# HorizonRobotics/GeoFlowSlam

Measured on AMD Instinct MI355X. Metric: front-end frames/sec (ORB+match+GICP) on 640x480 RGBD, higher is better.
Workload: dtype u8/int32 (ORB, match) + f64 (GICP); 1 GPU; BASELINE.json configs[1]: 640x480 RGBD frame pair, ORB extract (1000 feats, 8 levels) + BF Hamming match + GMS filter + GICP on ~19k-pt clouds (stride-4 depth grid); batch_pairs_per_gpu=512, lanes_per_gpu=4, passes=K passes per lane chain, joined once, distinct_scenes_per_gpu=512, scene_seeds=1000..1511 (rank 0), global_batch_pairs=512, parallelism=frames sharded x1, no collective

## Files before the change

### geoflowslam_amd/api.py

```python
import ctypes as C
import os

import numpy as np

_HERE = os.path.dirname(os.path.abspath(__file__))
_LIB_PATH = os.path.join(_HERE, "libgfs_hip.so")
_lib = None

KP_DTYPE = np.dtype(
    [("x", "<f4"), ("y", "<f4"), ("size", "<f4"), ("angle", "<f4"), ("response", "<f4"), ("octave", "<i4"),
     ("class_id", "<i4")]
)


class GfsError(RuntimeError):
    pass


class OrbConfig(C.Structure):
    _fields_ = [("nfeatures", C.c_int32), ("scale_factor", C.c_float), ("nlevels", C.c_int32),
                ("ini_th_fast", C.c_int32), ("min_th_fast", C.c_int32), ("max_rows", C.c_int32),
                ("max_cols", C.c_int32), ("max_batch", C.c_int32), ("device", C.c_int32),
                ("blur_taps_variant", C.c_int32)]


def _i32_fields(names):
    return [(n, C.c_int32) for n in names.split()]


class OrbGeometryInfo(C.Structure):
    _fields_ = _i32_fields("supported pyr_strips pyr_strips_fine pyr_in_lds xtab_in_lds xtab_in_lds_fine kp_cap octree_on_device "
                           "oct_node_cap n_cells n_blur_tiles fast_lds_wave")


class OrbLevelInfo(C.Structure):
    _fields_ = _i32_fields("rows cols n_cell_cols n_cell_rows w_cell h_cell n_cells max_cell_w max_cell_h quota n_ini kp_cap "
                           "octree_on_device")


class OrbPaths(C.Structure):
    _fields_ = _i32_fields("octree_on_device pyr_kernel pyr_fine_cut geometry_builds last_batch rows cols")


ORB_PYR_NONE, ORB_PYR_LDS, ORB_PYR_HBM = 0, 1, 2


class GicpConfig(C.Structure):
    _fields_ = [("num_threads", C.c_int32), ("downsampling_resolution", C.c_double),
                ("max_correspondence_distance", C.c_double), ("rotation_eps", C.c_double),
                ("translation_eps", C.c_double), ("max_iterations", C.c_int32), ("num_neighbors", C.c_int32)]


class GicpResult(C.Structure):
    _fields_ = [("T", C.c_double * 16), ("converged", C.c_int32), ("iterations", C.c_uint64),
                ("num_inliers", C.c_uint64), ("H", C.c_double * 36), ("b", C.c_double * 6), ("error", C.c_double),
                ("n_target_ds", C.c_int32), ("n_source_ds", C.c_int32), ("n_linearize", C.c_int32),
                ("n_error_evals", C.c_int32)]


class LbaProblem(C.Structure):
    _fields_ = [("n_poses", C.c_int32), ("n_points", C.c_int32), ("n_edges", C.c_int32), ("pose_q", C.c_void_p),
                ("pose_t", C.c_void_p), ("pose_fixed", C.c_void_p), ("points", C.c_void_p), ("edge_pose", C.c_void_p),
                ("edge_point", C.c_void_p), ("edge_obs", C.c_void_p), ("edge_inv_sigma2", C.c_void_p),
                ("edge_stereo", C.c_void_p), ("fx", C.c_double), ("fy", C.c_double), ("cx", C.c_double),
                ("cy", C.c_double), ("bf", C.c_double), ("huber_mono", C.c_double), ("huber_stereo", C.c_double),
                ("iterations", C.c_int32)]


class LbaSolution(C.Structure):
    _fields_ = [("pose_q", C.c_void_p), ("pose_t", C.c_void_p), ("points", C.c_void_p), ("edge_chi2", C.c_void_p),
                ("edge_depth_positive", C.c_void_p), ("iterations_run", C.c_int32), ("final_chi2", C.c_double),
                ("final_lambda", C.c_double)]


class LbaTrial(C.Structure):
    _fields_ = [("Dinv", C.c_void_p), ("Hs", C.c_void_p), ("bs", C.c_void_p), ("xp", C.c_void_p), ("xl", C.c_void_p),
                ("lambda_", C.c_double), ("scale", C.c_double), ("solve_ok", C.c_int32)]


class GbaInfo(C.Structure):
    _fields_ = [("n_free", C.c_int32), ("panel_rows", C.c_int32), ("panels", C.c_int32), ("block_pairs", C.c_int64),
                ("contributions", C.c_int64), ("system_bytes", C.c_int64), ("trials", C.c_int32), ("launches", C.c_int32)]


class EssentialGraphProblem(C.Structure):
    _fields_ = [("n_vertices", C.c_int32), ("n_edges", C.c_int32), ("n_points", C.c_int32), ("vertex_q", C.c_void_p),
                ("vertex_t", C.c_void_p), ("vertex_s", C.c_void_p), ("vertex_fixed", C.c_void_p), ("edge_i", C.c_void_p),
                ("edge_j", C.c_void_p), ("edge_q", C.c_void_p), ("edge_t", C.c_void_p), ("edge_s", C.c_void_p), ("edge_w", C.c_void_p),
                ("fix_scale", C.c_int32), ("iterations", C.c_int32), ("lambda_init", C.c_double), ("points", C.c_void_p),
                ("point_ref", C.c_void_p)]


class EssentialGraphSolution(C.Structure):
    _fields_ = [("vertex_q", C.c_void_p), ("vertex_t", C.c_void_p), ("vertex_s", C.c_void_p), ("points", C.c_void_p),
                ("edge_chi2", C.c_void_p), ("iterations_run", C.c_int32), ("final_chi2", C.c_double), ("final_lambda", C.c_double)]


class EssentialGraphInfo(C.Structure):
    _fields_ = [("n_free", C.c_int32), ("dimension", C.c_int32), ("panels", C.c_int32), ("blocks", C.c_int64), ("trials", C.c_int32),
                ("launches", C.c_int32), ("system_bytes", C.c_int64)]


class EssentialGraphTrial(C.Structure):
    _fields_ = [("H", C.c_void_p), ("b", C.c_void_p), ("x", C.c_void_p), ("chi2", C.c_double), ("trial_chi2", C.c_double),
                ("scale", C.c_double), ("n_free", C.c_int32), ("dimension", C.c_int32), ("solve_ok", C.c_int32)]


class LbaLidar(C.Structure):
    _fields_ = [("map", C.c_void_p), ("pose_local", C.c_void_p), ("matches_inliers", C.c_void_p), ("cloud_begin", C.c_void_p),
                ("cloud", C.c_void_p), ("two_camera", C.c_int32)]


def lba_lidar_struct(prob, map_handle=None):
    L = LbaLidar()
    keep = dict(pose_local=np.ascontiguousarray(prob["pose_local"], np.uint8),
                matches_inliers=np.ascontiguousarray(prob["matches_inliers"], np.int32),
                cloud_begin=np.ascontiguousarray(prob["cloud_begin"], np.int32),
                cloud=np.ascontiguousarray(prob["cloud"], np.float32).reshape(-1, 3))
    for k, v in keep.items():
        setattr(L, k, v.ctypes.data)
    L.map = map_handle
    L.two_camera = int(prob.get("two_camera", 0))
    return L, keep


class PoseProblem(C.Structure):
    _fields_ = [("q", C.c_double * 4), ("t", C.c_double * 3), ("n_obs", C.c_int32), ("xw", C.c_void_p), ("obs", C.c_void_p),
                ("inv_sigma2", C.c_void_p), ("stereo", C.c_void_p), ("fx", C.c_double), ("fy", C.c_double),
                ("cx", C.c_double), ("cy", C.c_double), ("bf", C.c_double), ("n_rounds", C.c_int32), ("its", C.c_int32)]


class PoseSolution(C.Structure):
    _fields_ = [("outlier", C.c_void_p), ("chi2", C.c_void_p), ("q", C.c_double * 4), ("t", C.c_double * 3),
                ("avg_reproj_error", C.c_float), ("n_inliers", C.c_int32), ("rounds_run", C.c_int32),
                ("iterations_run", C.c_int32)]


def pose_structs(prob):
    P, S = PoseProblem(), PoseSolution()
    n = int(prob["n_obs"]) if "n_obs" in prob else len(prob["xw"])
    keep = dict(xw=np.ascontiguousarray(prob["xw"], np.float64).reshape(-1, 3), obs=np.ascontiguousarray(prob["obs"], np.float64).reshape(-1, 3),
                inv_sigma2=np.ascontiguousarray(prob["inv_sigma2"], np.float32), stereo=np.ascontiguousarray(prob["stereo"], np.uint8),
                outlier=np.zeros(max(n, 1), np.uint8), chi2=np.zeros(max(n, 1), np.float64))
    P.q[:] = [float(v) for v in prob["q"]]
    P.t[:] = [float(v) for v in prob["t"]]
    P.n_obs = n
    for name in ("xw", "obs", "inv_sigma2", "stereo"):
        setattr(P, name, keep[name].ctypes.data)
    for name in ("fx", "fy", "cx", "cy", "bf"):
        setattr(P, name, float(prob[name]))
    P.n_rounds = int(prob.get("n_rounds", 4))
    P.its = int(prob.get("its", 10))
    S.outlier = keep["outlier"].ctypes.data
    S.chi2 = keep["chi2"].ctypes.data
    return P, S, keep, n


def pose_result(S, keep, n):
    return dict(outlier=keep["outlier"][:n].astype(bool), chi2=keep["chi2"][:n].copy(), q=np.array(S.q[:]), t=np.array(S.t[:]),
                avg_reproj_error=float(S.avg_reproj_error), n_inliers=int(S.n_inliers), rounds_run=int(S.rounds_run),
                iterations_run=int(S.iterations_run))


class Sim3OptProblem(C.Structure):
    _fields_ = [("s12", C.c_double * 8), ("cam1", C.c_double * 4), ("cam2", C.c_double * 4), ("th2", C.c_float),
                ("fix_scale", C.c_int32), ("n_pairs", C.c_int32), ("x1c", C.c_void_p), ("x2c", C.c_void_p), ("obs1", C.c_void_p),
                ("obs2", C.c_void_p), ("inv_sigma2_1", C.c_void_p), ("inv_sigma2_2", C.c_void_p)]


class Sim3OptSolution(C.Structure):
    _fields_ = [("s12", C.c_double * 8), ("n_in", C.c_int32), ("n_bad", C.c_int32), ("status", C.c_int32),
                ("iterations_run", C.c_int32 * 2), ("pair_state", C.c_void_p), ("chi2", C.c_void_p)]


SIM3_OPT_EARLY_RETURN, SIM3_OPT_BOTH_PHASES = 0, 1
SIM3_PAIR_INLIER, SIM3_PAIR_REMOVED_FIRST, SIM3_PAIR_REMOVED_FINAL = 0, 1, 2


def sim3_opt_structs(prob):
    P, S = Sim3OptProblem(), Sim3OptSolution()
    n = int(prob["n_pairs"]) if "n_pairs" in prob else len(prob["x1c"])
    keep = dict(x1c=np.ascontiguousarray(prob["x1c"], np.float64).reshape(-1, 3), x2c=np.ascontiguousarray(prob["x2c"], np.float64).reshape(-1, 3),
                obs1=np.ascontiguousarray(prob["obs1"], np.float64).reshape(-1, 2), obs2=np.ascontiguousarray(prob["obs2"], np.float64).reshape(-1, 2),
                inv_sigma2_1=np.ascontiguousarray(prob["inv_sigma2_1"], np.float32), inv_sigma2_2=np.ascontiguousarray(prob["inv_sigma2_2"], np.float32),
                pair_state=np.zeros(max(n, 1), np.uint8), chi2=np.zeros((max(n, 1), 2), np.float64))
    P.s12[:] = [float(v) for v in prob["s12"]]
    P.cam1[:] = [float(v) for v in prob["cam1"]]
    P.cam2[:] = [float(v) for v in prob["cam2"]]
    P.th2 = float(prob["th2"])
    P.fix_scale = int(bool(prob["fix_scale"]))
    P.n_pairs = n
    for name in ("x1c", "x2c", "obs1", "obs2", "inv_sigma2_1", "inv_sigma2_2"):
        setattr(P, name, keep[name].ctypes.data)
    S.pair_state = keep["pair_state"].ctypes.data
    S.chi2 = keep["chi2"].ctypes.data
    return P, S, keep, n

# ... 483 lines not shown
                 node_start=np.full(cap + 1, -7, np.int32), feat_idx=np.full(cap, -7, np.int32),
                 word_of_feature=np.full(cap, -7, np.int32) if with_words else None)
        for name, a in k.items():
            setattr(VV[b], name, a.ctypes.data if a is not None else None)
        keep.append(k)
    return VV, keep


def bow_vectors_results(VV, keep, counts):
    out = []
    for b, k in enumerate(keep):
        nw, nn = VV[b].n_words, VV[b].n_nodes
        m = int(k["node_start"][nn])
        out.append(dict(word_id=k["word_id"][:nw].copy(), word_value=k["word_value"][:nw].copy(), node_id=k["node_id"][:nn].copy(),
                        node_start=k["node_start"][:nn + 1].copy(), feat_idx=k["feat_idx"][:m].copy(),
                        word_of_feature=None if k["word_of_feature"] is None or counts is None else k["word_of_feature"][:counts[b]].copy()))
    return out


def sbp_map_struct(prob):
    P = SbpMapProblem()
    keep = dict(mp_proj=np.ascontiguousarray(prob["mp_proj"], np.float32).reshape(-1, 3),
                mp_level=np.ascontiguousarray(prob["mp_level"], np.int32),
                mp_view_cos=np.ascontiguousarray(prob["mp_view_cos"], np.float32),
                mp_desc=np.ascontiguousarray(prob["mp_desc"], np.uint8).reshape(-1, 32),
                mp_has_obs=np.ascontiguousarray(prob["mp_has_obs"], np.uint8),
                cur_kps_un=np.ascontiguousarray(prob["cur_kps_un"], KP_DTYPE),
                cur_u_right=np.ascontiguousarray(prob["cur_u_right"], np.float32),
                cur_desc=np.ascontiguousarray(prob["cur_desc"], np.uint8).reshape(-1, 32),
                cur_has_mp_obs=np.ascontiguousarray(prob["cur_has_mp_obs"], np.uint8),
                scale_factors=np.ascontiguousarray(prob["scale_factors"], np.float32))
    P.n_mp, P.n_cur = len(keep["mp_proj"]), len(keep["cur_kps_un"])
    for name, a in keep.items():
        setattr(P, name, a.ctypes.data)
    for name in ("min_x", "min_y", "grid_w_inv", "grid_h_inv", "th", "nn_ratio"):
        setattr(P, name, float(np.float32(prob[name])))
    P.n_levels = len(keep["scale_factors"])
    return P, keep


def sbp_struct(prob):
    P = SbpProblem()
    keep = dict(last_xw=np.ascontiguousarray(prob["last_xw"], np.float32).reshape(-1, 3),
                last_desc=np.ascontiguousarray(prob["last_desc"], np.uint8).reshape(-1, 32),
                last_octave=np.ascontiguousarray(prob["last_octave"], np.int32),
                last_angle=np.ascontiguousarray(prob["last_angle"], np.float32),
                last_mp_has_obs=np.ascontiguousarray(prob["last_mp_has_obs"], np.uint8),
                cur_kps_un=np.ascontiguousarray(prob["cur_kps_un"], KP_DTYPE),
                cur_u_right=np.ascontiguousarray(prob["cur_u_right"], np.float32),
                cur_desc=np.ascontiguousarray(prob["cur_desc"], np.uint8).reshape(-1, 32),
                cur_has_mp_obs=np.ascontiguousarray(prob["cur_has_mp_obs"], np.uint8),
                scale_factors=np.ascontiguousarray(prob["scale_factors"], np.float32))
    P.n_last, P.n_cur = len(keep["last_xw"]), len(keep["cur_kps_un"])
    for name, a in keep.items():
        setattr(P, name, a.ctypes.data)
    for name in ("Tcw_q", "Tcw_t", "Tlw_q", "Tlw_t"):
        getattr(P, name)[:] = [float(np.float32(v)) for v in prob[name]]
    for name in ("fx", "fy", "cx", "cy", "bf", "b", "min_x", "max_x", "min_y", "max_y", "grid_w_inv", "grid_h_inv", "th"):
        setattr(P, name, float(np.float32(prob[name])))
    P.n_levels = len(keep["scale_factors"])
    P.mono = int(prob.get("mono", 0))
    P.check_orientation = int(prob.get("check_orientation", 1))
    return P, keep


class PoseLidarProblem(C.Structure):
    _fields_ = [("q", C.c_float * 4), ("t", C.c_float * 3), ("n_obs", C.c_int32), ("xw", C.c_void_p), ("obs", C.c_void_p),
                ("inv_sigma2", C.c_void_p), ("stereo", C.c_void_p), ("fx", C.c_double), ("fy", C.c_double), ("cx", C.c_double),
                ("cy", C.c_double), ("bf", C.c_double), ("n_cloud", C.c_int32), ("cloud", C.c_void_p), ("map", C.c_void_p),
                ("n_iterations", C.c_int32), ("two_camera", C.c_int32)]


class PoseLidarSolution(C.Structure):
    _fields_ = [("outlier", C.c_void_p), ("chi2", C.c_void_p), ("q", C.c_double * 4), ("t", C.c_double * 3), ("qf", C.c_float * 4),
                ("tf", C.c_float * 3), ("avg_reproj_error", C.c_float), ("n_inliers", C.c_int32), ("n_lidar_inliers", C.c_int32),
                ("residual", C.c_float), ("lidar_rounds", C.c_int32), ("rounds_run", C.c_int32), ("iterations_run", C.c_int32),
                ("round_edges", C.c_int32 * 4), ("round_chi2", C.c_float * 4), ("round_valid", C.c_int32 * 4)]


class LidarMapInput(C.Structure):
    _fields_ = [("n_keyframes", C.c_int32), ("q", C.c_void_p), ("t", C.c_void_p), ("cloud_begin", C.c_void_p), ("cloud", C.c_void_p),
                ("leaf", C.c_float)]


class LidarMapInfo(C.Structure):
    _fields_ = [("n_in", C.c_int32), ("n_out", C.c_int32), ("passthrough", C.c_int32), ("div", C.c_int32 * 3)]


class FrameCloudConfig(C.Structure):
    _fields_ = [("horizontal_angle", C.c_double), ("max_distance", C.c_double), ("local_map_resolution", C.c_double),
                ("downsize_resolution", C.c_float), ("angle_guard_deg", C.c_double)]


class FrameCloudInfo(C.Structure):
    _fields_ = [(k, C.c_int32) for k in ("n_in", "n_scans", "n_edge_raw", "n_surf_raw", "n_edge_voxel", "n_surf_voxel", "n_edge", "n_surf",
                                         "n_down", "host_scan_split")] + [("passthrough", C.c_int32 * 3)]


class FrameCloudStageBuffers(C.Structure):
    _fields_ = [("scans", C.c_void_p), ("cap_scans", C.c_int32)] + \
               [(k, C.c_void_p) for k in ("edge_raw", "surf_raw", "edge_voxel", "surf_voxel", "edge", "surf")] + [("cap_points", C.c_int32)]


def frame_cloud_info(I):
    d = {k: int(getattr(I, k)) for k, _ in FrameCloudInfo._fields_[:10]}
    d["passthrough"] = tuple(int(v) for v in I.passthrough)
    return d


def lidar_map_info(I):
    return dict(n_in=int(I.n_in), n_out=int(I.n_out), passthrough=int(I.passthrough), div=tuple(int(v) for v in I.div))


def pose_lidar_structs(prob, map_handle=None):
    P, S = PoseLidarProblem(), PoseLidarSolution()
    xw = np.ascontiguousarray(prob["xw"], np.float64).reshape(-1, 3)
    n = len(xw)
    cloud = np.ascontiguousarray(prob["cloud"], np.float32).reshape(-1, 3)
    keep = dict(xw=xw, obs=np.ascontiguousarray(prob["obs"], np.float64).reshape(-1, 3),
                inv_sigma2=np.ascontiguousarray(prob["inv_sigma2"], np.float32), stereo=np.ascontiguousarray(prob["stereo"], np.uint8),
                cloud=cloud, outlier=np.zeros(max(n, 1), np.uint8), chi2=np.zeros(max(n, 1), np.float64))
    P.q[:] = [float(v) for v in np.asarray(prob["q"], np.float32)]
    P.t[:] = [float(v) for v in np.asarray(prob["t"], np.float32)]
    P.n_obs = n
    for name in ("xw", "obs", "inv_sigma2", "stereo", "cloud"):
        setattr(P, name, keep[name].ctypes.data)
    for name in ("fx", "fy", "cx", "cy", "bf"):
        setattr(P, name, float(prob[name]))
    P.n_cloud = len(cloud)
    P.map = map_handle
    P.n_iterations = int(prob.get("n_iterations", 3))
    P.two_camera = int(prob.get("two_camera", 0))
    S.outlier = keep["outlier"].ctypes.data
    S.chi2 = keep["chi2"].ctypes.data
    S.n_lidar_inliers = int(prob.get("n_lidar_inliers", 0))
    S.residual = float(prob.get("residual", 0.0))
    return P, S, keep, n


def pose_lidar_result(S, keep, n):
    return dict(outlier=keep["outlier"][:n].astype(bool), chi2=keep["chi2"][:n].copy(), q=np.array(S.q[:]), t=np.array(S.t[:]),
                qf=np.array(S.qf[:], np.float32), tf=np.array(S.tf[:], np.float32), avg_reproj_error=np.float32(S.avg_reproj_error),
                n_inliers=int(S.n_inliers), n_lidar_inliers=int(S.n_lidar_inliers), residual=np.float32(S.residual),
                lidar_rounds=int(S.lidar_rounds), rounds_run=int(S.rounds_run), iterations_run=int(S.iterations_run),
                round_edges=list(S.round_edges), round_chi2=np.array(S.round_chi2[:], np.float32), round_valid=list(S.round_valid))


ABI_SYMBOLS = [
    "gfs_abi_version", "gfs_last_error", "gfs_device_count",
    "gfs_orb_default_config", "gfs_orb_create", "gfs_orb_destroy", "gfs_orb_get_tables", "gfs_orb_max_keypoints",
    "gfs_orb_extract", "gfs_orb_extract_batch", "gfs_orb_extract_batch_device", "gfs_orb_device_results",
    "gfs_orb_fetch", "gfs_orb_level_size", "gfs_orb_fetch_level", "gfs_orb_fetch_candidates", "gfs_orb_octree_host",
    "gfs_orb_octree_device", "gfs_test_sort_replica", "gfs_test_heap_sort_replica", "gfs_test_glibc_math", "gfs_test_traffic",
    "gfs_test_orb_blur_tiles", "gfs_test_orb_geometry", "gfs_test_orb_last_paths",
    "gfs_hamming256", "gfs_matcher_create", "gfs_matcher_destroy", "gfs_bf_match_hamming",
    "gfs_bf_match_hamming_batch_device",
    "gfs_gicp_default_config", "gfs_gicp_create", "gfs_gicp_destroy", "gfs_gicp_align", "gfs_gicp_align_batch_device",
    "gfs_gicp_fetch_preprocessed", "gfs_gicp_tile_stats", "gfs_gicp_knn_stats", "gfs_gicp_coop_stats", "gfs_test_gicp_coop_hold", "gfs_test_gicp_coop_release", "gfs_test_gicp_coop_in_use", "gfs_frame_rgbd", "gfs_gicp_align_next", "gfs_gicp_align_next_batch_device", "gfs_test_voxel_sort", "gfs_test_voxel_sort_paths", "gfs_test_wave_std_sort",
    "gfs_lba_create", "gfs_lba_destroy", "gfs_lba_solve", "gfs_lba_solve_bool", "gfs_lba_linearize", "gfs_lba_batch_create", "gfs_lba_batch_destroy",
    "gfs_lba_solve_batch", "gfs_lba_lidar_reserve", "gfs_lba_solve_lidar", "gfs_lba_solve_lidar_bool", "gfs_lba_linearize_lidar",
    "gfs_lba_fetch_lidar_edges", "gfs_test_lba_stop_at_look", "gfs_test_lba_last_looks", "gfs_test_lba_first_trial",
    "gfs_gba_create", "gfs_gba_destroy", "gfs_gba_solve", "gfs_gba_solve_bool", "gfs_gba_last_info", "gfs_test_gba_first_trial",
    "gfs_test_gba_panel_rows", "gfs_test_gba_lists", "gfs_test_gba_tile_layout",
    "gfs_essential_graph_create", "gfs_essential_graph_destroy", "gfs_essential_graph_optimize", "gfs_essential_graph_correct_points",
    "gfs_essential_graph_last_info", "gfs_test_essential_graph_first_trial", "gfs_test_essential_graph_lists",
    "gfs_sim3_opt_create", "gfs_sim3_opt_destroy", "gfs_sim3_optimize", "gfs_test_glibc_exp",
    "gfs_sim3_ransac_iterations", "gfs_sim3_ransac_create", "gfs_sim3_ransac_solve", "gfs_sim3_ransac_destroy",
    "gfs_frame_create", "gfs_frame_destroy", "gfs_depth_to_cloud", "gfs_depth_to_cloud_batch_device", "gfs_depth_convert_u16_batch_device", "gfs_stereo_from_rgbd",
    "gfs_stereo_from_rgbd_batch_device",
    "gfs_pose_create", "gfs_pose_destroy", "gfs_pose_optimize", "gfs_pose_set_sum_order",
    "gfs_lidar_mapper_create", "gfs_lidar_mapper_destroy", "gfs_lidar_map_build", "gfs_lidar_map_fetch", "gfs_voxel_grid_filter",
    "gfs_test_lidar_map_grid",
    "gfs_frame_cloud_default_config", "gfs_frame_cloud_create", "gfs_frame_cloud_destroy", "gfs_frame_cloud_extract",
    "gfs_frame_cloud_extract_device", "gfs_test_frame_cloud_stages", "gfs_test_frame_cloud_radius",
    "gfs_lidar_map_create", "gfs_lidar_map_set", "gfs_lidar_map_destroy", "gfs_pose_lidar_create", "gfs_pose_lidar_destroy",
    "gfs_pose_lidar_set_sum_order", "gfs_pose_lidar_optimize", "gfs_pose_lidar_fetch_edges",
    "gfs_gms_create", "gfs_gms_destroy", "gfs_gms_inlier_mask", "gfs_gms_inlier_mask_batch_device",
    "gfs_sbp_create", "gfs_sbp_destroy", "gfs_search_by_projection", "gfs_search_by_projection_map",
    "gfs_sbp_reserve_local", "gfs_search_local_points", "gfs_sbp_reserve_fuse", "gfs_fuse_search", "gfs_test_glibc_logf",
    "gfs_sbp_reserve_sim3_search", "gfs_sim3_search", "gfs_test_sim3_search_groups",
    "gfs_sbp_reserve_triangulation", "gfs_create_new_map_points", "gfs_sbp_reserve_bow", "gfs_search_by_bow",
    "gfs_map_points_create", "gfs_map_points_destroy", "gfs_map_points_update",
    "gfs_bow_create", "gfs_bow_destroy", "gfs_bow_transform", "gfs_bow_transform_device",
    "gfs_bow_db_create", "gfs_bow_db_destroy", "gfs_bow_db_add", "gfs_bow_db_erase", "gfs_bow_db_query",
    "gfs_klt_create", "gfs_klt_destroy", "gfs_klt_layout", "gfs_klt_pyramid_create", "gfs_klt_pyramid_destroy",
    "gfs_klt_build_pyramid", "gfs_klt_build_pyramid_device", "gfs_klt_pyramid_download", "gfs_klt_track", "gfs_klt_fb_track",
    "gfs_klt_fb_track_device",
    "gfs_fmat_create", "gfs_fmat_destroy", "gfs_find_fundamental_ransac", "gfs_find_fundamental_ransac_device",
    "gfs_klt_compact_tracks_device", "gfs_klt_apply_mask_device",
    "gfs_clahe_default_config", "gfs_clahe_create", "gfs_clahe_destroy", "gfs_clahe_apply", "gfs_clahe_apply_device",
    "gfs_clahe_download_luts", "gfs_klt_build_pyramid_clahe", "gfs_klt_build_pyramid_clahe_device",
    "gfs_timer_create", "gfs_timer_destroy", "gfs_timer_start", "gfs_timer_stop", "gfs_timer_elapsed_ms",
    "gfs_profile_enable", "gfs_profile_report", "gfs_profile_reset",
]


def lib():
    global _lib
    if _lib is None:
        if not os.path.exists(_LIB_PATH):
            raise GfsError(f"{_LIB_PATH} not built: run `python -c 'import __graft_entry__ as g; g.build()'` "
                           "(there is no CPU fallback)")
        L = C.CDLL(_LIB_PATH)
        L.gfs_last_error.restype = C.c_char_p
        vp, ip, i = C.c_void_p, C.POINTER(C.c_int), C.c_int
        L.gfs_orb_default_config.argtypes = [C.POINTER(OrbConfig)]
        L.gfs_orb_create.argtypes = [C.POINTER(OrbConfig), C.POINTER(vp)]
        L.gfs_orb_destroy.argtypes = [vp]
        L.gfs_orb_get_tables.argtypes = [vp] * 7
        L.gfs_orb_max_keypoints.argtypes = [vp]
        L.gfs_orb_extract.argtypes = [vp, vp, i, i, i, i, i, vp, vp, i, ip]
        L.gfs_orb_extract_batch.argtypes = [vp, vp, i, i, i, i, i, i, vp, vp, i, vp, vp]
        L.gfs_orb_extract_batch_device.argtypes = [vp, vp, i, i, i, i, i, vp]
        L.gfs_orb_device_results.argtypes = [vp, C.POINTER(vp), C.POINTER(vp), C.POINTER(vp), C.POINTER(vp), ip]
        L.gfs_orb_fetch.argtypes = [vp, i, vp, vp, i, ip, ip]
        L.gfs_orb_level_size.argtypes = [vp, i, ip, ip]
        L.gfs_orb_fetch_level.argtypes = [vp, i, i, i, vp]
        L.gfs_orb_fetch_candidates.argtypes = [vp, i, i, vp, vp, vp, i]
        L.gfs_test_orb_geometry.argtypes = [i, i, i, i, C.c_float, C.POINTER(OrbGeometryInfo), vp, i]
        L.gfs_test_orb_last_paths.argtypes = [vp, C.POINTER(OrbPaths)]
        L.gfs_orb_octree_host.argtypes = [vp, vp, vp, i, i, i, i, i, i, vp, i]
        L.gfs_orb_octree_device.argtypes = [i, vp, vp, vp, i, i, i, i, i, i, vp, vp, vp, i]
        L.gfs_test_glibc_math.argtypes = [i, vp, i, vp, vp, vp]
        L.gfs_test_glibc_logf.argtypes = [i, vp, i, vp]
        L.gfs_sbp_reserve_local.argtypes = [vp, i]
        L.gfs_search_local_points.argtypes = [vp, C.POINTER(LocalPointsProblem), i, C.POINTER(LocalPointsResult)]
        L.gfs_sbp_reserve_fuse.argtypes = [vp, i, i, i]
        L.gfs_fuse_search.argtypes = [vp, C.POINTER(FusePoints), i, C.POINTER(FuseKeyframe), i, C.POINTER(FuseResult)]
        L.gfs_sbp_reserve_sim3_search.argtypes = [vp, i, i, i]
        L.gfs_sim3_search.argtypes = [vp, C.POINTER(FusePoints), i, C.POINTER(Sim3SearchProblem), i, C.POINTER(Sim3SearchResult)]
        L.gfs_test_sim3_search_groups.argtypes = [vp, i]
        L.gfs_sbp_reserve_triangulation.argtypes = [vp, i, C.c_int64]
        L.gfs_create_new_map_points.argtypes = [vp, C.POINTER(TriProblem), i, C.POINTER(C.POINTER(TriResult))]
        L.gfs_sbp_reserve_bow.argtypes = [vp, i, i]
        L.gfs_search_by_bow.argtypes = [vp, C.POINTER(BowProblem), i, C.POINTER(C.POINTER(BowResult))]
        L.gfs_map_points_create.argtypes = [i, i, i, C.POINTER(vp)]
        L.gfs_map_points_destroy.argtypes = [vp]
        L.gfs_map_points_update.argtypes = [vp, C.POINTER(MapPointsProblem), C.POINTER(MapPointsResult)]
        L.gfs_test_traffic.argtypes = [i, i, C.c_longlong, C.c_longlong, i, C.POINTER(C.c_longlong)]
        L.gfs_hamming256.argtypes = [vp, vp]
        L.gfs_matcher_create.argtypes = [i, i, i, i, C.POINTER(vp)]
        L.gfs_matcher_destroy.argtypes = [vp]
        L.gfs_bf_match_hamming.argtypes = [vp, vp, i, vp, i, vp, vp]
        L.gfs_bf_match_hamming_batch_device.argtypes = [vp, vp, vp, vp, vp, i, i, vp, vp, vp]
        if hasattr(L, "gfs_gicp_create"):
            L.gfs_gicp_default_config.argtypes = [C.POINTER(GicpConfig)]
            L.gfs_gicp_create.argtypes = [i, i, i, C.POINTER(vp)]
            L.gfs_gicp_destroy.argtypes = [vp]
            L.gfs_gicp_align.argtypes = [vp, vp, i, vp, i, vp, C.POINTER(GicpConfig), C.POINTER(GicpResult)]
            L.gfs_gicp_align_batch_device.argtypes = [vp, vp, vp, vp, vp, i, i, vp, C.POINTER(GicpConfig), vp, vp]
            L.gfs_gicp_fetch_preprocessed.argtypes = [vp, i, i, vp, vp, i, ip]
            L.gfs_gicp_tile_stats.argtypes = [vp, vp, i]
            L.gfs_gicp_knn_stats.argtypes = [vp, i, i, vp, vp, i]
            L.gfs_gicp_coop_stats.argtypes = [vp, vp]
            L.gfs_test_gicp_coop_hold.argtypes = [vp, i]
            L.gfs_test_gicp_coop_release.argtypes = [vp, i]
            L.gfs_test_gicp_coop_in_use.argtypes = [i]
            L.gfs_test_voxel_sort.argtypes = [vp, vp, i, vp]
            L.gfs_test_voxel_sort_paths.argtypes = [vp, vp]
            L.gfs_test_wave_std_sort.argtypes = [i, vp, i, vp]
            L.gfs_gicp_align_next.argtypes = [vp, vp, i, vp, C.POINTER(GicpConfig), C.POINTER(GicpResult)]
            L.gfs_gicp_align_next_batch_device.argtypes = [vp, vp, vp, i, i, vp, C.POINTER(GicpConfig), vp, vp]
        if hasattr(L, "gfs_lba_create"):
            L.gfs_lba_create.argtypes = [i, i, i, i, C.POINTER(vp)]
            L.gfs_lba_destroy.argtypes = [vp]
            L.gfs_lba_solve.argtypes = [vp, C.POINTER(LbaProblem), C.POINTER(LbaSolution), vp]
            L.gfs_lba_solve_bool.argtypes = [vp, C.POINTER(LbaProblem), C.POINTER(LbaSolution), vp]
            L.gfs_lba_linearize.argtypes = [vp, C.POINTER(LbaProblem), vp, vp, vp, vp, vp, vp, C.POINTER(C.c_double)]
            L.gfs_lba_batch_create.argtypes = [i, i, i, i, i, C.POINTER(vp)]
            L.gfs_lba_batch_destroy.argtypes = [vp]
            L.gfs_lba_solve_batch.argtypes = [vp, vp, vp, i, vp]
            L.gfs_test_lba_stop_at_look.argtypes = [i]
            L.gfs_test_lba_last_looks.argtypes = [C.POINTER(C.c_int32)] * 4
            L.gfs_test_lba_first_trial.argtypes = [vp, C.POINTER(LbaProblem), C.POINTER(LbaTrial)]
        if hasattr(L, "gfs_gba_create"):
            L.gfs_gba_create.argtypes = [i, i, i, i, C.POINTER(vp)]
            L.gfs_gba_destroy.argtypes = [vp]
            L.gfs_gba_solve.argtypes = [vp, C.POINTER(LbaProblem), C.POINTER(LbaSolution), vp]
            L.gfs_gba_solve_bool.argtypes = [vp, C.POINTER(LbaProblem), C.POINTER(LbaSolution), vp]
            L.gfs_gba_last_info.argtypes = [vp, C.POINTER(GbaInfo)]
            L.gfs_test_gba_first_trial.argtypes = [vp, C.POINTER(LbaProblem), C.POINTER(LbaTrial)]
            L.gfs_test_gba_panel_rows.argtypes = []
            L.gfs_test_gba_lists.argtypes = [i, i, i, vp, vp, vp, vp, vp, vp, vp, C.c_int64, vp, C.c_int64, vp, vp]
            L.gfs_test_gba_tile_layout.argtypes = [C.c_int64, C.c_int64, C.c_int64, vp]
        if hasattr(L, "gfs_essential_graph_create"):
            L.gfs_essential_graph_create.argtypes = [i, i, i, i, C.POINTER(vp)]
            L.gfs_essential_graph_destroy.argtypes = [vp]
            L.gfs_essential_graph_optimize.argtypes = [vp, C.POINTER(EssentialGraphProblem), C.POINTER(EssentialGraphSolution)]
            L.gfs_essential_graph_correct_points.argtypes = [vp, i, vp, vp, i, vp, vp, vp]
            L.gfs_essential_graph_last_info.argtypes = [vp, C.POINTER(EssentialGraphInfo)]
            L.gfs_test_essential_graph_first_trial.argtypes = [vp, C.POINTER(EssentialGraphProblem), C.POINTER(EssentialGraphTrial)]
            L.gfs_test_essential_graph_lists.argtypes = [i, i, vp, vp, vp, vp, vp, vp, vp, C.c_int64, vp, C.c_int64]
        if hasattr(L, "gfs_sim3_opt_create"):
            L.gfs_sim3_opt_create.argtypes = [i, i, i, C.POINTER(vp)]
            L.gfs_sim3_opt_destroy.argtypes = [vp]
            L.gfs_sim3_optimize.argtypes = [vp, vp, i, vp]
            L.gfs_test_glibc_exp.argtypes = [i, vp, i, vp]
        if hasattr(L, "gfs_sim3_ransac_create"):
            L.gfs_sim3_ransac_iterations.argtypes = [i, C.c_double, i, i]
            L.gfs_sim3_ransac_create.argtypes = [i, i, i, i, C.POINTER(vp)]
            L.gfs_sim3_ransac_destroy.argtypes = [vp]
            L.gfs_sim3_ransac_solve.argtypes = [vp, vp, i, vp]
        L.gfs_bow_create.argtypes = [i, C.POINTER(BowVocabularyStruct), i, i, C.POINTER(vp)]
        L.gfs_bow_destroy.argtypes = [vp]
        L.gfs_bow_destroy.restype = None
        L.gfs_bow_transform.argtypes = [vp, C.POINTER(vp), vp, i, i, C.POINTER(BowVectors)]
        L.gfs_bow_transform_device.argtypes = [vp, vp, vp, i, i, i, C.POINTER(BowVectors)]
        L.gfs_bow_db_create.argtypes = [i, i, i, C.POINTER(vp)]
        L.gfs_bow_db_destroy.argtypes = [vp]
        L.gfs_bow_db_destroy.restype = None
        L.gfs_bow_db_add.argtypes = [vp, i, i, vp, vp]
        L.gfs_bow_db_erase.argtypes = [vp, i]
        L.gfs_bow_db_query.argtypes = [vp, i, vp, vp, vp, vp, vp]
        if hasattr(L, "gfs_lba_solve_lidar"):
            L.gfs_lba_lidar_reserve.argtypes = [vp, i]
            L.gfs_lba_solve_lidar.argtypes = [vp, C.POINTER(LbaProblem), C.POINTER(LbaLidar), C.POINTER(LbaSolution), vp, vp]
            L.gfs_lba_solve_lidar_bool.argtypes = [vp, C.POINTER(LbaProblem), C.POINTER(LbaLidar), C.POINTER(LbaSolution), vp, vp]
            L.gfs_lba_linearize_lidar.argtypes = [vp, C.POINTER(LbaProblem), C.POINTER(LbaLidar), vp, vp, vp, vp, vp, vp,
                                                  C.POINTER(C.c_double), vp, i, vp]
            L.gfs_lba_fetch_lidar_edges.argtypes = [vp, i, vp, vp, vp, i, vp]
        if hasattr(L, "gfs_lidar_map_build"):
            L.gfs_lidar_mapper_create.argtypes = [i, i, i, C.POINTER(vp)]
            L.gfs_lidar_mapper_destroy.argtypes = [vp]
            L.gfs_lidar_map_build.argtypes = [vp, C.POINTER(LidarMapInput), vp, C.POINTER(LidarMapInfo)]
            L.gfs_lidar_map_fetch.argtypes = [vp, vp, i, C.POINTER(C.c_int32)]
            L.gfs_voxel_grid_filter.argtypes = [vp, vp, i, C.c_float, vp, i, C.POINTER(LidarMapInfo)]
            L.gfs_test_lidar_map_grid.argtypes = [vp, vp, i, vp, vp, i, C.POINTER(C.c_int32), C.POINTER(C.c_int32)]
        L.gfs_frame_cloud_default_config.argtypes = [C.POINTER(FrameCloudConfig)]
        L.gfs_frame_cloud_default_config.restype = None
        L.gfs_frame_cloud_create.argtypes = [i, i, C.POINTER(FrameCloudConfig), C.POINTER(vp)]
        L.gfs_frame_cloud_destroy.argtypes = [vp]
        L.gfs_frame_cloud_extract.argtypes = [vp, vp, i, vp, i, vp, i, C.POINTER(FrameCloudInfo)]
        L.gfs_frame_cloud_extract_device.argtypes = [vp, vp, vp, vp, i, vp, i, C.POINTER(FrameCloudInfo)]
        L.gfs_test_frame_cloud_stages.argtypes = [vp, C.POINTER(FrameCloudStageBuffers)]
        L.gfs_test_frame_cloud_radius.argtypes = [vp, vp, i, i, vp, i, C.POINTER(C.c_int32)]
        if hasattr(L, "gfs_frame_create"):
            f = C.c_float
            L.gfs_frame_create.argtypes = [i, i, i, i, C.POINTER(vp)]
            L.gfs_frame_destroy.argtypes = [vp]
            L.gfs_depth_to_cloud.argtypes = [vp, vp, i, i, i, i, f, f, f, f, vp, i, ip]
            L.gfs_depth_to_cloud_batch_device.argtypes = [vp, vp, i, i, i, i, f, f, f, f, vp, i, vp, vp]
            L.gfs_depth_convert_u16_batch_device.argtypes = [vp, vp, i, i, i, f, vp, vp]
            L.gfs_stereo_from_rgbd.argtypes = [vp, vp, vp, i, vp, i, i, i, f, vp, vp]
            L.gfs_frame_rgbd.argtypes = [vp, vp, vp, i, vp, i, i, i, f, i, f, f, f, f, vp, vp, vp, i, ip, vp, vp, ip]
            L.gfs_stereo_from_rgbd_batch_device.argtypes = [vp, vp, vp, vp, i, i, vp, i, i, f, vp, vp, vp]
        if hasattr(L, "gfs_klt_create"):
            f, d = C.c_float, C.c_double
            L.gfs_klt_create.argtypes = [i, i, i, i, i, i, i, C.POINTER(vp)]
            L.gfs_klt_destroy.argtypes = [vp]
            L.gfs_klt_layout.argtypes = [vp, vp, vp, vp]
            L.gfs_klt_pyramid_create.argtypes = [vp, C.POINTER(vp)]
            L.gfs_klt_pyramid_destroy.argtypes = [vp]
            L.gfs_klt_build_pyramid.argtypes = [vp, vp, vp, i, i]
            L.gfs_klt_build_pyramid_device.argtypes = [vp, vp, vp, i, i, vp]
            L.gfs_klt_pyramid_download.argtypes = [vp, vp, i, vp, vp]
            L.gfs_klt_track.argtypes = [vp, vp, vp, i, vp, vp, vp, vp, vp, i, i, d, i, d]
            L.gfs_klt_fb_track.argtypes = [vp, vp, vp, i, vp, vp, vp, vp, vp, i, f, f]
            L.gfs_klt_fb_track_device.argtypes = [vp, vp, vp, i, i, vp, vp, vp, vp, vp, i, f, f, vp]
            L.gfs_klt_compact_tracks_device.argtypes = [vp, i, i, vp, vp, vp, vp, vp, vp, vp, vp, vp]
            L.gfs_klt_apply_mask_device.argtypes = [vp, i, i, vp, vp, vp, vp, vp]
        L.gfs_clahe_default_config.argtypes = [C.POINTER(ClaheConfig)]
        L.gfs_clahe_default_config.restype = None
        L.gfs_clahe_create.argtypes = [i, i, i, i, C.POINTER(ClaheConfig), C.POINTER(vp)]
        L.gfs_clahe_destroy.argtypes = [vp]
        L.gfs_clahe_apply.argtypes = [vp, vp, i, i, i, i, vp, i]
        L.gfs_clahe_apply_device.argtypes = [vp, vp, i, i, i, i, vp, i, vp]
        L.gfs_clahe_download_luts.argtypes = [vp, i, vp]
        L.gfs_klt_build_pyramid_clahe.argtypes = [vp, vp, vp, vp, i, i, vp, i]
        L.gfs_klt_build_pyramid_clahe_device.argtypes = [vp, vp, vp, vp, i, i, vp, i, vp]
        if hasattr(L, "gfs_fmat_create"):
            L.gfs_fmat_create.argtypes = [i, i, i, C.POINTER(vp)]
            L.gfs_fmat_destroy.argtypes = [vp]
            L.gfs_find_fundamental_ransac.argtypes = [vp, i, vp, vp, vp, C.c_double, C.c_double, i, vp, vp, vp]
            L.gfs_find_fundamental_ransac_device.argtypes = [vp, i, i, vp, vp, vp, C.c_double, C.c_double, i, vp, vp, vp]
        L.gfs_timer_create.argtypes = [i, C.POINTER(vp)]
        L.gfs_timer_destroy.argtypes = [vp]
        L.gfs_timer_start.argtypes = [vp, vp]
        L.gfs_timer_stop.argtypes = [vp, vp]
        L.gfs_timer_elapsed_ms.argtypes = [vp, C.POINTER(C.c_float)]
        L.gfs_profile_report.argtypes = [vp, vp, vp, i]
        _lib = L
    return _lib


def _p(a):
    return a.ctypes.data_as(C.c_void_p) if a is not None else None


def _check(rc, what):
    if rc < 0:
        err = GfsError(f"{what} failed ({rc}): {lib().gfs_last_error().decode()}")
        err.code = rc
        raise err
    return rc


def device_count():
    return lib().gfs_device_count()


class ORBextractor:

    def __init__(self, nfeatures=1000, scaleFactor=1.2, nlevels=8, iniThFAST=20, minThFAST=7, max_rows=480,
                 max_cols=640, max_batch=1, device=0, blur_taps_variant=0):
        L = lib()
        cfg = OrbConfig()
        L.gfs_orb_default_config(C.byref(cfg))
        cfg.nfeatures, cfg.scale_factor, cfg.nlevels = nfeatures, scaleFactor, nlevels
        cfg.ini_th_fast, cfg.min_th_fast = iniThFAST, minThFAST
        cfg.max_rows, cfg.max_cols, cfg.max_batch, cfg.device = max_rows, max_cols, max_batch, device
        cfg.blur_taps_variant = blur_taps_variant
        self.nlevels = nlevels
        self.h = C.c_void_p()
        _check(L.gfs_orb_create(C.byref(cfg), C.byref(self.h)), "gfs_orb_create")
        self.cap = L.gfs_orb_max_keypoints(self.h)

    def close(self):
        if getattr(self, "h", None) and _lib is not None:
            _lib.gfs_orb_destroy(self.h)
        self.h = None

    __del__ = close

    def GetLevels(self):
        return self.nlevels

    def tables(self):
        n = self.nlevels
        sc, inv, s2, is2 = (np.zeros(n, np.float32) for _ in range(4))
        feats = np.zeros(n, np.int32)
        umax = np.zeros(16, np.int32)
        _check(lib().gfs_orb_get_tables(self.h, _p(sc), _p(inv), _p(s2), _p(is2), _p(feats), _p(umax)), "get_tables")
        return dict(scale=sc, inv_scale=inv, sigma2=s2, inv_sigma2=is2, feats=feats, umax=umax)

    def GetScaleFactors(self):
        return self.tables()["scale"]

    def GetInverseScaleFactors(self):
        return self.tables()["inv_scale"]

    def GetScaleSigmaSquares(self):
        return self.tables()["sigma2"]

    def GetInverseScaleSigmaSquares(self):
        return self.tables()["inv_sigma2"]

    def __call__(self, image, vLappingArea=(0, 0)):
        if image is None or image.size == 0:
            return -1, np.zeros(0, KP_DTYPE), np.zeros((0, 32), np.uint8)
        assert image.dtype == np.uint8 and image.ndim == 2, "CV_8UC1 expected (src/ORBextractor.cc:1153)"
        stride = image.strides[0]
        assert image.strides[1] == 1
        kps = np.zeros(self.cap, KP_DTYPE)
        desc = np.zeros((self.cap, 32), np.uint8)
        n = C.c_int(0)
        r = lib().gfs_orb_extract(self.h, C.c_void_p(image.ctypes.data), image.shape[0], image.shape[1], stride,
                                  vLappingArea[0], vLappingArea[1], _p(kps), _p(desc), self.cap, C.byref(n))
        if r < -1:
            err = GfsError(f"gfs_orb_extract failed ({r + 100}): {lib().gfs_last_error().decode()}")
            err.code = r + 100
            raise err
        return r, kps[:n.value].copy(), desc[:n.value].copy()

    def extract_batch(self, images, vLappingArea=(0, 0)):
        imgs = [np.ascontiguousarray(im, np.uint8) for im in images]
        B = len(imgs)
        rows, cols = imgs[0].shape
        ptrs = (C.c_void_p * B)(*[im.ctypes.data for im in imgs])
        kps = np.zeros((B, self.cap), KP_DTYPE)
        desc = np.zeros((B, self.cap, 32), np.uint8)
        n = np.zeros(B, np.int32)
        mono = np.zeros(B, np.int32)
        _check(lib().gfs_orb_extract_batch(self.h, ptrs, B, rows, cols, cols, vLappingArea[0], vLappingArea[1], _p(kps),
                                           _p(desc), self.cap, _p(n), _p(mono)), "gfs_orb_extract_batch")
        return [(int(mono[b]), kps[b, :n[b]].copy(), desc[b, :n[b]].copy()) for b in range(B)]

    def extract_batch_device(self, dev_ptr, B, rows, cols, vLappingArea=(0, 0), stream=None):
        _check(lib().gfs_orb_extract_batch_device(self.h, C.c_void_p(dev_ptr), B, rows, cols, vLappingArea[0],
                                                  vLappingArea[1], C.c_void_p(stream) if stream else None),
               "gfs_orb_extract_batch_device")

    def device_results(self):
        k, d, c, m = C.c_void_p(), C.c_void_p(), C.c_void_p(), C.c_void_p()
        cap = C.c_int()
        _check(lib().gfs_orb_device_results(self.h, C.byref(k), C.byref(d), C.byref(c), C.byref(m), C.byref(cap)),
               "gfs_orb_device_results")
        return dict(kps=k.value, desc=d.value, counts=c.value, mono=m.value, cap=cap.value)

    def fetch(self, b):
        kps = np.zeros(self.cap, KP_DTYPE)
        desc = np.zeros((self.cap, 32), np.uint8)
        n, mono = C.c_int(), C.c_int()
        _check(lib().gfs_orb_fetch(self.h, b, _p(kps), _p(desc), self.cap, C.byref(n), C.byref(mono)), "gfs_orb_fetch")
        return mono.value, kps[:n.value].copy(), desc[:n.value].copy()

    def level_size(self, l):
        r, c = C.c_int(), C.c_int()
        _check(lib().gfs_orb_level_size(self.h, l, C.byref(r), C.byref(c)), "gfs_orb_level_size")
        return r.value, c.value

    def level(self, l, b=0, blurred=False):
        r, c = self.level_size(l)
        a = np.zeros((r, c), np.uint8)
        _check(lib().gfs_orb_fetch_level(self.h, b, l, int(blurred), _p(a)), "gfs_orb_fetch_level")
        return a

    def candidates(self, l, b=0):
        n = _check(lib().gfs_orb_fetch_candidates(self.h, b, l, None, None, None, 0), "gfs_orb_fetch_candidates")
        x, y, s = (np.zeros(max(n, 1), np.int32) for _ in range(3))
        lib().gfs_orb_fetch_candidates(self.h, b, l, _p(x), _p(y), _p(s), n)
        return x[:n], y[:n], s[:n]


    def last_paths(self):
        P = OrbPaths()
        _check(lib().gfs_test_orb_last_paths(self.h, C.byref(P)), "gfs_test_orb_last_paths")
        return {n: int(getattr(P, n)) for n, _ in OrbPaths._fields_}


def orb_geometry(rows, cols, nfeatures=1000, nlevels=8, scale_factor=1.2):
    I = OrbGeometryInfo()
    Lv = (OrbLevelInfo * nlevels)()
    rc = lib().gfs_test_orb_geometry(rows, cols, nfeatures, nlevels, scale_factor, C.byref(I), C.cast(Lv, C.c_void_p), nlevels)
    out = {n: int(getattr(I, n)) for n, _ in OrbGeometryInfo._fields_}
    out["supported"] = bool(out["supported"])
    if rc == -5:
        return dict(out, levels=[])
    _check(rc, "gfs_test_orb_geometry")
    return dict(out, levels=[{n: int(getattr(Lv[l], n)) for n, _ in OrbLevelInfo._fields_} for l in range(nlevels)])


def wave_std_sort_perm(keys, device=0):
    k = np.ascontiguousarray(keys, np.uint32)
    perm = np.zeros(max(len(k), 1), np.uint16)
    _check(lib().gfs_test_wave_std_sort(device, _p(k), len(k), _p(perm)), "gfs_test_wave_std_sort")
    return perm[:len(k)].astype(np.int64)


def octree_host(x, y, score, min_x, max_x, min_y, max_y, n_features):
    x = np.ascontiguousarray(x, np.int32)
    y = np.ascontiguousarray(y, np.int32)
    score = np.ascontiguousarray(score, np.int32)
    out = np.zeros(max(len(x), 1), np.int32)
    n = lib().gfs_orb_octree_host(_p(x), _p(y), _p(score), len(x), min_x, max_x, min_y, max_y, n_features, _p(out),
                                  len(out))
    return out[:n]


def octree_device(x, y, score, min_x, max_x, min_y, max_y, n_features, device=0):
    x = np.ascontiguousarray(x, np.int32)
    y = np.ascontiguousarray(y, np.int32)
    score = np.ascontiguousarray(score, np.int32)
    cap = n_features + 64
    ox, oy, os_ = (np.zeros(cap, np.int32) for _ in range(3))
    n = _check(lib().gfs_orb_octree_device(device, _p(x), _p(y), _p(score), len(x), min_x, max_x, min_y, max_y, n_features,
                                           _p(ox), _p(oy), _p(os_), cap), "gfs_orb_octree_device")
    return ox[:n], oy[:n], os_[:n]


class ORBmatcher:

    def __init__(self, max_query=4096, max_train=4096, max_batch=1, device=0):
        self.h = C.c_void_p()
        _check(lib().gfs_matcher_create(device, max_query, max_train, max_batch, C.byref(self.h)), "gfs_matcher_create")

    def close(self):
        if getattr(self, "h", None) and _lib is not None:
            _lib.gfs_matcher_destroy(self.h)
        self.h = None

    __del__ = close

    @staticmethod
    def DescriptorDistance(a, b):
        a = np.ascontiguousarray(a, np.uint8)
        b = np.ascontiguousarray(b, np.uint8)
        return int(lib().gfs_hamming256(_p(a), _p(b)))

    def match(self, query, train):
        q = np.ascontiguousarray(query, np.uint8).reshape(-1, 32)
        t = np.ascontiguousarray(train, np.uint8).reshape(-1, 32)
        ti = np.zeros(len(q), np.int32)
        di = np.zeros(len(q), np.int32)
        n = _check(lib().gfs_bf_match_hamming(self.h, _p(q), len(q), _p(t), len(t), _p(ti), _p(di)),
                   "gfs_bf_match_hamming")
        return ti[:n], di[:n]

    def match_batch_device(self, d_query, d_nq, d_train, d_nt, B, stride_rows, d_idx, d_dist, stream=None):
        _check(lib().gfs_bf_match_hamming_batch_device(self.h, C.c_void_p(d_query), C.c_void_p(d_nq), C.c_void_p(d_train),
                                                       C.c_void_p(d_nt), B, stride_rows, C.c_void_p(d_idx),
                                                       C.c_void_p(d_dist), C.c_void_p(stream) if stream else None),
               "gfs_bf_match_hamming_batch_device")


def gicp_default_config():
    c = GicpConfig()
    lib().gfs_gicp_default_config(C.byref(c))
    return c


def _result_dict(res):
    return dict(
        T=np.array(res.T).reshape(4, 4).T.copy(), converged=bool(res.converged), iterations=int(res.iterations),
        num_inliers=int(res.num_inliers), H=np.array(res.H).reshape(6, 6).T.copy(), b=np.array(res.b),
        error=float(res.error), n_target_ds=res.n_target_ds, n_source_ds=res.n_source_ds,
        n_linearize=res.n_linearize, n_error_evals=res.n_error_evals)


class RegistrationGICP:

    def __init__(self, max_points=40960, max_batch=1, device=0):
        self.h = C.c_void_p()
        self.max_points = max_points
        _check(lib().gfs_gicp_create(device, max_points, max_batch, C.byref(self.h)), "gfs_gicp_create")

    def close(self):
        if getattr(self, "h", None) and _lib is not None:
            _lib.gfs_gicp_destroy(self.h)
        self.h = None

    __del__ = close

    def RegisterPointClouds(self, target_points, source_points, init_T_target_source=None, cfg=None):
        t = np.ascontiguousarray(target_points, np.float32).reshape(-1, 4)
        s = np.ascontiguousarray(source_points, np.float32).reshape(-1, 4)
        T0 = np.eye(4) if init_T_target_source is None else np.asarray(init_T_target_source, np.float64)
        T0c = np.ascontiguousarray(T0.T.reshape(-1))
        cfg = cfg or gicp_default_config()
        res = GicpResult()
        _check(lib().gfs_gicp_align(self.h, _p(t), len(t), _p(s), len(s), _p(T0c), C.byref(cfg), C.byref(res)),
               "gfs_gicp_align")
        return _result_dict(res)

    def voxel_sort_perm(self, keys):
        k = np.ascontiguousarray(keys, np.uint64)
        perm = np.zeros(max(len(k), 1), np.uint32)
        _check(lib().gfs_test_voxel_sort(self.h, _p(k), len(k), _p(perm)), "gfs_test_voxel_sort")
        return perm[:len(k)].astype(np.int64)

    def voxel_sort_paths(self):
        out = np.zeros(3, np.int32)
        _check(lib().gfs_test_voxel_sort_paths(self.h, _p(out)), "gfs_test_voxel_sort_paths")
        return dict(tie_free=int(out[0]), harmless=int(out[1]), replica=int(out[2]))

    def RegisterNext(self, source_points, init_T_target_source=None, cfg=None):
        s = np.ascontiguousarray(source_points, np.float32).reshape(-1, 4)
        T0 = np.eye(4) if init_T_target_source is None else np.asarray(init_T_target_source, np.float64)
        T0c = np.ascontiguousarray(T0.T.reshape(-1))
        cfg = cfg or gicp_default_config()
        res = GicpResult()
        _check(lib().gfs_gicp_align_next(self.h, _p(s), len(s), _p(T0c), C.byref(cfg), C.byref(res)), "gfs_gicp_align_next")
        return _result_dict(res)

    def align_next_batch_device(self, d_source, d_ns, B, stride_pts, init_T=None, cfg=None, stream=None, raw=False):
        cfg = cfg or gicp_default_config()
        out = (GicpResult * B)()
        T0 = None
        if init_T is not None:
            T0 = np.ascontiguousarray(np.asarray(init_T, np.float64).transpose(0, 2, 1).reshape(B, 16))
        _check(lib().gfs_gicp_align_next_batch_device(self.h, C.c_void_p(d_source), C.c_void_p(d_ns), B, stride_pts, _p(T0),
                                                      C.byref(cfg), out, C.c_void_p(stream) if stream else None),
               "gfs_gicp_align_next_batch_device")
        return out if raw else [_result_dict(r) for r in out]

    def align_batch_device(self, d_target, d_nt, d_source, d_ns, B, stride_pts, init_T=None, cfg=None, stream=None,
                           raw=False):
        cfg = cfg or gicp_default_config()
        out = (GicpResult * B)()
        T0 = None
        if init_T is not None:
            T0 = np.ascontiguousarray(np.asarray(init_T, np.float64).transpose(0, 2, 1).reshape(B, 16))
# ... 1229 lines not shown
```

### geoflowslam_amd/csrc/orb.hip

```cpp
#include <algorithm>
#include <atomic>
#include <cmath>
#include <condition_variable>
#include <functional>
#include <memory>
#include <thread>

#include "gfs_common.hpp"
#include "orb_host.hpp"
#include "std_sort_replica.hpp"
#include "wave_std_sort.hpp"

using gfs::BlurTileDev;
using gfs::CellDev;
using gfs::LevelDev;

namespace {

struct KpIn {
  float x, y;
  int level;
  float response;
  int slot;
};

struct Lvl0 {
  const uint8_t* base;
  size_t frame_stride;
  int pitch;
};

__device__ __forceinline__ const uint8_t* level_ptr(const LevelDev& L, int level, int b, Lvl0 l0, const uint8_t* pyr,
                                                    size_t pyr_frame, int* pitch) {
  if (level == 0) {
    *pitch = l0.pitch;
    return l0.base + (size_t)b * l0.frame_stride;
  }
  *pitch = L.pitch;
  return pyr + (size_t)b * pyr_frame + L.plane_off;
}

constexpr int kPyrThreads = 1024, kPyrWaves = kPyrThreads / 64;
constexpr int kPyrTabRows = gfs::OrbGeometry::kPyrTabRows, kPyrProgRows = gfs::OrbGeometry::kPyrProgRows;
typedef float pyr_f2 __attribute__((ext_vector_type(2)));

__global__ __launch_bounds__(kPyrThreads) void k_pyr_area_lds(const LevelDev* __restrict__ levels, int nlevels, Lvl0 l0,
                                                              uint8_t* __restrict__ pyr, size_t pyr_frame,
                                                              const int* __restrict__ strip_rows, unsigned lds_a,
                                                              unsigned lds_x, int xt_total,
                                                              const int* __restrict__ xt_start, const int* __restrict__ xt_n,
                                                              const float* __restrict__ xt_alpha, const int* __restrict__ yt_start,
                                                              const int* __restrict__ yt_n, const float* __restrict__ yt_alpha) {
  extern __shared__ __align__(16) uint8_t smem[];
  __shared__ float4 s_prog[kPyrProgRows + 1];
  __shared__ int s_first[kPyrTabRows];
  const int k = blockIdx.x, b = blockIdx.y, tid = threadIdx.x;
  const int wave = __builtin_amdgcn_readfirstlane(tid >> 6), lane = tid & 63;
  const int* rng = strip_rows + 2 * k * nlevels;
#ifdef GFS_PYR_TIMING
  __shared__ long long pyr_t[12];
  { const long long _n = clock64(); if (tid == 0) pyr_t[0] = _n; }
#endif
  for (int i = tid; i < kPyrProgRows + 1; i += kPyrThreads) s_prog[i] = make_float4(0.f, 0.f, 0.f, 0.f);
  bool my_row = false;
  int my_first = 0, my_ny = 0, my_prev_last = -1, my_slot = 0, my_prog = 0;
  float4 my_ay = make_float4(0.f, 0.f, 0.f, 0.f);
  {
    int off = 0, pb = 0;
    for (int level = 1; level < nlevels; level++) {
      const int r0 = rng[2 * level], n = rng[2 * level + 1] - r0, yo = levels[level].ytab_off;
      const int srow0 = rng[2 * (level - 1)];
      const int i = tid - off;
      if (i >= 0 && i < n) {
        const int d = r0 + i;
        my_row = true;
        my_first = yt_start[yo + d];
        my_ny = yt_n[yo + d];
        my_ay = *reinterpret_cast<const float4*>(yt_alpha + 4 * (size_t)(yo + d));
        if (d > 0) my_prev_last = yt_start[yo + d - 1] + yt_n[yo + d - 1] - 1;
        my_slot = off + i;
        my_prog = pb - srow0;
      }
      off += n;
      pb += rng[2 * (level - 1) + 1] - srow0;
    }
  }
  float4* s_xt = reinterpret_cast<float4*>(smem + lds_x);
  if (lds_x)
    for (int i0 = tid; i0 < xt_total; i0 += 4 * kPyrThreads) {
      float4 a[4];
      int st[4];
#pragma unroll
      for (int q = 0; q < 4; q++) {
        const int i = i0 + q * kPyrThreads;
        if (i < xt_total) {
          a[q] = *reinterpret_cast<const float4*>(xt_alpha + 4 * (size_t)i);
          st[q] = xt_start[i];
        }
      }
#pragma unroll
      for (int q = 0; q < 4; q++) {
        const int i = i0 + q * kPyrThreads;
        if (i < xt_total) s_xt[i] = make_float4(a[q].x, a[q].y, a[q].z, __int_as_float(st[q]));
      }
    }
  {
    const LevelDev S0 = levels[0];
    int gp;
    const uint8_t* src = level_ptr(S0, 0, b, l0, pyr, pyr_frame, &gp);
    const int s0 = rng[0], s1 = rng[1], cols = S0.cols, sp = gfs::OrbGeometry::kPyrLdsPitch(cols);
    if (((cols | gp) & 15) == 0 && ((uintptr_t)src & 15) == 0) {
      const int qpr = cols >> 4, total = (s1 - s0) * qpr;
      for (int i0 = tid; i0 < total; i0 += 4 * kPyrThreads) {
        uint4 v[4];
#pragma unroll
        for (int q = 0; q < 4; q++) {
          const int i = i0 + q * kPyrThreads;
          if (i < total) {
            const int y = i / qpr, x = i - y * qpr;
            v[q] = *reinterpret_cast<const uint4*>(src + (size_t)(s0 + y) * gp + 16 * x);
          }
        }
#pragma unroll
        for (int q = 0; q < 4; q++) {
          const int i = i0 + q * kPyrThreads;
          if (i < total) reinterpret_cast<uint4*>(smem)[i] = v[q];
        }
      }
    } else if (((cols | gp) & 3) == 0 && ((uintptr_t)src & 3) == 0) {
      const int wpr = cols >> 2, total = (s1 - s0) * wpr;
      for (int i0 = tid; i0 < total; i0 += 4 * kPyrThreads) {
        uint32_t v[4];
#pragma unroll
        for (int q = 0; q < 4; q++) {
          const int i = i0 + q * kPyrThreads;
          if (i < total) {
            const int y = i / wpr, x = i - y * wpr;
            v[q] = *reinterpret_cast<const uint32_t*>(src + (size_t)(s0 + y) * gp + 4 * x);
          }
        }
#pragma unroll
        for (int q = 0; q < 4; q++) {
          const int i = i0 + q * kPyrThreads;
          if (i < total) reinterpret_cast<uint32_t*>(smem)[i] = v[q];
        }
      }
    } else {
      const int total = (s1 - s0) * cols;
      for (int i = tid; i < total; i += kPyrThreads) {
        const int y = i / cols, x = i - y * cols;
        smem[y * sp + x] = src[(size_t)(s0 + y) * gp + x];
      }
    }
  }
  __syncthreads();
  if (my_row) {
    const float ays[4] = {my_ay.x, my_ay.y, my_ay.z, my_ay.w};
    s_first[my_slot] = my_first;
    float* pr = reinterpret_cast<float*>(s_prog + my_prog + my_first);
#pragma unroll
    for (int j = 0; j < 4; j++)
      if (j < my_ny) {
        if (j == 0 && my_first == my_prev_last) {
          pr[1] = ays[0];
          pr[3] = __int_as_float(1);
        } else {
          pr[4 * j] = ays[j];
        }
        if (j == my_ny - 1) pr[4 * j + 2] = __int_as_float(1);
      }
  }
  __syncthreads();
#ifdef GFS_PYR_TIMING
  { const long long _n = clock64(); if (tid == 0) pyr_t[8] = _n; }
#endif
  int tab0 = 0, pb = 0;
  for (int level = 1; level < nlevels; level++) {
    const LevelDev L = levels[level];
    const int scols = levels[level - 1].cols;
    const int r0 = rng[2 * level], nrow = rng[2 * level + 1] - r0, srow0 = rng[2 * (level - 1)], nsrc = rng[2 * (level - 1) + 1] - srow0;
    const int sp = gfs::OrbGeometry::kPyrLdsPitch(scols), kp = gfs::OrbGeometry::kPyrLdsPitch(L.cols);
    const unsigned src_off = (level - 1) & 1 ? lds_a : 0u, keep_off = level & 1 ? lds_a : 0u;
    const bool has_keep = level + 1 < nlevels;
    uint8_t* dst = pyr + (size_t)b * pyr_frame + L.plane_off;
    const bool dst_even = (((uintptr_t)dst | (unsigned)L.pitch) & 1) == 0;
    const int nchunk = (L.cols + 127) >> 7, cw = (((L.cols + nchunk - 1) / nchunk) + 1) & ~1;
    const int units = nchunk * nrow;
    const int u1 = (int)((long long)(wave + 1) * units / kPyrWaves);
    int u = (int)((long long)wave * units / kPyrWaves);
    while (u < u1) {
      const int chunk = u / nrow, row_a = u - chunk * nrow, row_b = min(nrow, row_a + (u1 - u));
      const int dx0 = chunk * cw + 2 * lane;
      const bool on0 = 2 * lane < cw && dx0 < L.cols, on1 = on0 && dx0 + 1 < L.cols;
      const int xa = L.xtab_off + min(dx0, L.cols - 1), xb = L.xtab_off + min(dx0 + 1, L.cols - 1);
      int sxa, sxb;
      float4 axa, axb;
      bool x4 = false;
      if (lds_x) {
        axa = s_xt[xa];
        axb = s_xt[xb];
        sxa = __float_as_int(axa.w);
        sxb = __float_as_int(axb.w);
      } else {
        sxa = xt_start[xa];
        sxb = xt_start[xb];
        x4 = __ballot(xt_n[xa] > 3 || xt_n[xb] > 3) != 0ull;
        axa = *reinterpret_cast<const float4*>(xt_alpha + 4 * (size_t)xa);
        axb = *reinterpret_cast<const float4*>(xt_alpha + 4 * (size_t)xb);
      }
      const pyr_f2 a0 = {axa.x, axb.x}, a1 = {axa.y, axb.y}, a2 = {axa.z, axb.z}, a3 = {axa.w, axb.w};
      const uint32_t* wa = reinterpret_cast<const uint32_t*>(smem + src_off + (sxa & ~3));
      const uint32_t* wb = reinterpret_cast<const uint32_t*>(smem + src_off + (sxb & ~3));
      const int sha = (sxa & 3) * 8, shb = (sxb & 3) * 8, spw = sp >> 2;
      uint8_t* drow = dst + (size_t)(r0 + row_a) * L.pitch + dx0;
      uint8_t* krow = smem + keep_off + (size_t)row_a * kp + dx0;
      auto walk = [&](auto X4) {
        constexpr bool kX4 = decltype(X4)::value;
        auto words = [&](int si, uint32_t(&w)[4]) {
          const int o = si * spw;
          w[0] = wa[o];
          w[1] = wa[o + 1];
          w[2] = wb[o];
          w[3] = wb[o + 1];
        };
        auto hsum = [&](const uint32_t(&w)[4]) {
          const uint32_t va = __builtin_amdgcn_alignbit(w[1], w[0], sha), vb = __builtin_amdgcn_alignbit(w[3], w[2], shb);
          const pyr_f2 c0 = {(float)(va & 0xffu), (float)(vb & 0xffu)}, c1 = {(float)((va >> 8) & 0xffu), (float)((vb >> 8) & 0xffu)},
                       c2 = {(float)((va >> 16) & 0xffu), (float)((vb >> 16) & 0xffu)};
          pyr_f2 buf = c0 * a0;
          buf = buf + c1 * a1;
          buf = buf + c2 * a2;
          if constexpr (kX4) {
            const pyr_f2 c3 = {(float)(va >> 24), (float)(vb >> 24)};
            buf = buf + c3 * a3;
          }
          return buf;
        };
        auto emit = [&](pyr_f2 sum) {
          const unsigned v = __builtin_amdgcn_cvt_pk_u8_f32(sum.y, 1u, __builtin_amdgcn_cvt_pk_u8_f32(sum.x, 0u, 0u));
          if (on0) {
            if (on1 && dst_even) {
              *reinterpret_cast<uint16_t*>(drow) = (uint16_t)v;
            } else {
              drow[0] = (uint8_t)v;
              if (on1) drow[1] = (uint8_t)(v >> 8);
            }
            if (has_keep) *reinterpret_cast<uint16_t*>(krow) = (uint16_t)v;
          }
          drow += L.pitch;
          krow += kp;
        };
        int si = __builtin_amdgcn_readfirstlane(s_first[tab0 + row_a]) - srow0, left = row_b - row_a;
        uint32_t w[4];
        words(si, w);
        float4 P = s_prog[pb + si];
        pyr_f2 sum;
        {
          const pyr_f2 h = hsum(w);
          words(min(si + 1, nsrc - 1), w);
          const float4 Pn = s_prog[pb + si + 1];
          const bool opens = __builtin_amdgcn_readfirstlane(__float_as_int(P.w)) != 0;
          sum = h * (opens ? P.y : P.x);
          if (!opens && __builtin_amdgcn_readfirstlane(__float_as_int(P.z)) != 0) {
            emit(sum);
            sum = h * P.y;
            left--;
          }
          P = Pn;
          si++;
        }
        while (left > 0) {
          const pyr_f2 h = hsum(w);
          words(min(si + 1, nsrc - 1), w);
          const float4 Pn = s_prog[pb + si + 1];
          sum = sum + h * P.x;
          if (__builtin_amdgcn_readfirstlane(__float_as_int(P.z)) != 0) {
            emit(sum);
            sum = h * P.y;
            left--;
          }
          P = Pn;
          si++;
        }
      };
      if (x4) walk(std::true_type{});
      else walk(std::false_type{});
      u += row_b - row_a;
    }
    pb += nsrc;
    tab0 += nrow;
    __syncthreads();
#ifdef GFS_PYR_TIMING
    { const long long _n = clock64(); if (tid == 0) pyr_t[level] = _n; }
#endif
  }
#ifdef GFS_PYR_TIMING
  if (tid == 0 && b == 7 && (k == 0 || k == 3))
    printf("PYRT k=%d stage=%lld l1=%lld l2=%lld l3=%lld l4=%lld l5=%lld l6=%lld l7=%lld total=%lld\n", k, pyr_t[8] - pyr_t[0],
           pyr_t[1] - pyr_t[8], pyr_t[2] - pyr_t[1], pyr_t[3] - pyr_t[2], pyr_t[4] - pyr_t[3], pyr_t[5] - pyr_t[4], pyr_t[6] - pyr_t[5],
           pyr_t[7] - pyr_t[6], pyr_t[7] - pyr_t[0]);
#endif
}

__global__ __launch_bounds__(kPyrThreads) void k_pyr_area_hbm(const LevelDev* __restrict__ levels, int nlevels, Lvl0 l0,
                                                              uint8_t* __restrict__ pyr, size_t pyr_frame,
                                                              const int* __restrict__ strip_rows,
                                                              const int* __restrict__ xt_start, const int* __restrict__ xt_n,
                                                              const float* __restrict__ xt_alpha, const int* __restrict__ yt_start,
                                                              const int* __restrict__ yt_n, const float* __restrict__ yt_alpha) {
  const int k = blockIdx.x, b = blockIdx.y, tid = threadIdx.x;
  const int* rng = strip_rows + 2 * k * nlevels;
  for (int level = 1; level < nlevels; level++) {
    const LevelDev L = levels[level];
    const LevelDev S = levels[level - 1];
    const int r0 = rng[2 * level], r1 = rng[2 * level + 1];
    int sp;
    const uint8_t* src = level_ptr(S, level - 1, b, l0, pyr, pyr_frame, &sp);
    uint8_t* dst = pyr + (size_t)b * pyr_frame + L.plane_off;
    int ncolt = min(L.cols, kPyrThreads), rows_par = kPyrThreads / ncolt;
    {
      int best = rows_par * L.cols;
      for (int q = 2; q <= 8; q++) {
        const int c = (L.cols + q - 1) / q, r = kPyrThreads / c;
        if (c >= 64 && r * L.cols > best * q) {
          best = r * L.cols / q;
          ncolt = c;
          rows_par = r;
        }
      }
    }
    const int cxi = tid % ncolt, ry = tid / ncolt;
    if (ry < rows_par) {
      for (int dx = cxi; dx < L.cols; dx += ncolt) {
        const int xi = L.xtab_off + dx;
        const int sx0 = xt_start[xi], nx = xt_n[xi];
        const float4 ax = *reinterpret_cast<const float4*>(xt_alpha + 4 * (size_t)xi);
        for (int dy = r0 + ry; dy < r1; dy += rows_par) {
          const int yi = L.ytab_off + dy;
          const int sy0 = yt_start[yi], ny = yt_n[yi];
          const float4 ay = *reinterpret_cast<const float4*>(yt_alpha + 4 * (size_t)yi);
          const float ays[4] = {ay.x, ay.y, ay.z, ay.w};
          float sum = 0.f;
#pragma unroll
          for (int j = 0; j < 4; j++) {
            if (j < ny) {
              const uint8_t* row = src + (size_t)(sy0 + j) * sp + sx0;
              float buf = __fadd_rn(0.f, __fmul_rn((float)row[0], ax.x));
              if (nx > 1) buf = __fadd_rn(buf, __fmul_rn((float)row[1], ax.y));
              if (nx > 2) buf = __fadd_rn(buf, __fmul_rn((float)row[2], ax.z));
              if (nx > 3) buf = __fadd_rn(buf, __fmul_rn((float)row[3], ax.w));
              const float t = __fmul_rn(ays[j], buf);
              sum = (j == 0) ? t : __fadd_rn(sum, t);
            }
          }
          const int r = __float2int_rn(sum);
          dst[(size_t)dy * L.pitch + dx] = (uint8_t)min(max(r, 0), 255);
        }
      }
    }
    __threadfence_block();
    __syncthreads();
  }
}

__device__ __forceinline__ unsigned has9(unsigned m) {
  const unsigned m32 = m | (m << 16);
  unsigned r = m32 & (m32 >> 1);
  r &= r >> 2;
  r &= r >> 4;
  r &= m32 >> 8;
  return r & 0xffffu;
}

#define GFS_RING16_(F)                                                                                                     \
  F(rp3[0]) F(rp3[1]) F(rp2[2]) F(rp1[3]) F(c[3]) F(rm1[3]) F(rm2[2]) F(rm3[1]) F(rm3[0]) F(rm3[-1]) F(rm2[-2]) F(rm1[-3]) \
  F(c[-3]) F(rp1[-3]) F(rp2[-2]) F(rp3[-1])
__device__ __forceinline__ bool arc_is_corner_pol(const uint8_t* __restrict__ c, int p, int th, int pol) {
  const int v = c[0];
  const int sgn = pol ? -1 : 1, off = pol ? v + th : th - v;
  const uint8_t *rm3 = c - 3 * p, *rm2 = c - 2 * p, *rm1 = c - p, *rp1 = c + p, *rp2 = c + 2 * p, *rp3 = c + 3 * p;
  unsigned m = 0;
#define GFS_RING_(px) m = __builtin_amdgcn_alignbit(m, (unsigned)((int)(px) * sgn + off), 31);
  GFS_RING16_(GFS_RING_)
#undef GFS_RING_
  return has9(m & 0xffffu) != 0;
}
__device__ __forceinline__ int arc_score_pol(const uint8_t* __restrict__ c, int p, int pol) {
  const int v = c[0];
  const int sgn = pol ? 1 : -1, off = pol ? -v : v;
  const uint8_t *rm3 = c - 3 * p, *rm2 = c - 2 * p, *rm1 = c - p, *rp1 = c + p, *rp2 = c + 2 * p, *rp3 = c + 3 * p;
  int d[16];
  {
    int k = 0;
#define GFS_RING_(px) d[k++] = (int)(px) * sgn + off;
    GFS_RING16_(GFS_RING_)
#undef GFS_RING_
  }
  int lo[16], lo4[16];
#pragma unroll
  for (int k = 0; k < 16; k++) lo[k] = min(d[k], d[(k + 1) & 15]);
#pragma unroll
  for (int k = 0; k < 16; k++) lo4[k] = min(lo[k], lo[(k + 2) & 15]);
  int A = -256;
#pragma unroll
  for (int k = 0; k < 16; k++) A = max(A, min(min(lo4[k], lo4[(k + 4) & 15]), d[(k + 8) & 15]));
  return A;
}
#undef GFS_RING16_

#ifndef GFS_FC_WAVES
#define GFS_FC_WAVES 4
#endif
constexpr int kFcWaves = GFS_FC_WAVES;
#ifdef GFS_FAST_TIMING
#define FC_T_INIT long long fc_acc[8] = {0, 0, 0, 0, 0, 0, 0, 0}, fc_last = clock64();
#define FC_T(k) { const long long _n = clock64(); fc_acc[k] += _n - fc_last; fc_last = _n; }
#define FC_T_END(nq_, nc_, nk_) if (lane == 0 && (blockIdx.x % 257) == 0 && wave == 0) printf("FASTT lvl=%d stage=%lld p0=%lld compact=%lld arc=%lld score=%lld nms=%lld emit=%lld nq=%d nc=%d nk=%d\n", (int)C.level, fc_acc[0], fc_acc[1], fc_acc[2], fc_acc[3], fc_acc[4], fc_acc[5], fc_acc[6], nq_, nc_, nk_);
#else
#define FC_T_INIT
#define FC_T(k)
#define FC_T_END(a, b, c)
#endif

typedef unsigned short fc_us2 __attribute__((ext_vector_type(2)));
typedef short fc_s2 __attribute__((ext_vector_type(2)));
__device__ __forceinline__ unsigned fc_min(unsigned a, unsigned b) {
  return __builtin_bit_cast(unsigned, __builtin_elementwise_min(__builtin_bit_cast(fc_us2, a), __builtin_bit_cast(fc_us2, b)));
}
__device__ __forceinline__ unsigned fc_max(unsigned a, unsigned b) {
  return __builtin_bit_cast(unsigned, __builtin_elementwise_max(__builtin_bit_cast(fc_us2, a), __builtin_bit_cast(fc_us2, b)));
}
__device__ __forceinline__ unsigned fc_add(unsigned a, unsigned b) {
  return __builtin_bit_cast(unsigned, (fc_s2)(__builtin_bit_cast(fc_s2, a) + __builtin_bit_cast(fc_s2, b)));
}
__device__ __forceinline__ unsigned fc_sub(unsigned a, unsigned b) {
  return __builtin_bit_cast(unsigned, (fc_s2)(__builtin_bit_cast(fc_s2, a) - __builtin_bit_cast(fc_s2, b)));
}
__device__ __forceinline__ void fc_pair_test(unsigned T, unsigned Bt, unsigned L, unsigned R, unsigned v, unsigned t2, unsigned* dark,
                                             unsigned* bright) {
  const unsigned md = fc_max(fc_min(T, Bt), fc_min(L, R));
  const unsigned mb = fc_min(fc_max(T, Bt), fc_max(L, R));
  *dark = fc_sub(fc_add(md, t2), v);
  *bright = fc_sub(fc_add(v, t2), mb);
}
__device__ __forceinline__ unsigned fc_nibble(unsigned fe, unsigned fo) {
  const unsigned tt = ((fe >> 15) & 0x00010001u) | ((fo >> 14) & 0x00020002u);
  return (tt | (tt >> 14)) & 0xfu;
}
// ... 841 lines not shown
          const int j = V - 1 - k;
          const int ni = vs[j].node;
          const ONode nd = nodes[ni];
          s_proc[ni] = 1;
          const unsigned long long v = s_npre[k];
          const int A = (int)(pbase & 0xfffff), Mx = (int)((pbase >> 20) & 0xfffff);
          pbase += v;
          const int ci = (int)(v & 0xfffff);
          uint32_t* pa = perm(pc);
          uint32_t* pb = perm(pc ^ 1);
          unsigned long long pk = 0;
          if (have) {
#pragma unroll
            for (int u = 0; u < kOctChunk; u++)
              if (nd.kb + u < nd.ke) pk += 1ull << (16 * oct_quadrant(nd, nkey[u]));
          } else {
            for_keys(pa, nd.kb, nd.ke, [&](int, uint32_t key) { pk += 1ull << (16 * oct_quadrant(nd, key)); });
          }
          const int cnt[4] = {(int)(pk & 0xffff), (int)((pk >> 16) & 0xffff), (int)((pk >> 32) & 0xffff), (int)(pk >> 48)};
          unsigned long long pos = (unsigned long long)cnt[0] << 16 | (unsigned long long)(cnt[0] + cnt[1]) << 32 |
                                   (unsigned long long)(cnt[0] + cnt[1] + cnt[2]) << 48;
          if (have) {
#pragma unroll
            for (int u = 0; u < kOctChunk; u++)
              if (nd.kb + u < nd.ke) {
                const int sh = 16 * oct_quadrant(nd, nkey[u]);
                pa[nd.kb + (int)((pos >> sh) & 0xffff)] = nkey[u];
                pos += 1ull << sh;
              }
          } else {
            for_keys(pa, nd.kb, nd.ke, [&](int, uint32_t key) {
              const int sh = 16 * oct_quadrant(nd, key);
              pb[nd.kb + (int)((pos >> sh) & 0xffff)] = key;
              pos += 1ull << sh;
            });
            for_keys(pb, nd.kb, nd.ke, [&](int p, uint32_t key) { pa[p] = key; });
          }
          int kb = nd.kb, before = 0, mrank = 0;
          for (int q = 0; q < 4; q++) {
            if (cnt[q] == 0) continue;
            const int posn = T - A - ci + (ci - 1 - before);
            ONode ch = oct_child(nd, q);
            ch.kb = kb;
            ch.ke = kb + cnt[q];
            nxt[posn] = ch;
            if (cnt[q] > 1) {
              vnew[Mx + mrank] = OVs{cnt[q], ch.x0, (short)posn};
              mrank++;
            }
            kb += cnt[q];
            before++;
          }
        }
        __syncthreads();
        const int nchunk = (nn + kOctThreads - 1) / kOctThreads;
        const int i0 = min(tid * nchunk, nn), i1 = min(i0 + nchunk, nn);
        unsigned long long ls = 0;
        for (int i = i0; i < i1; i++) ls += s_proc[i] ? 0 : 1;
        unsigned long long stot;
        unsigned long long sbase = oct_scan_u64(ls, s_w64, &stot);
        for (int i = i0; i < i1; i++) {
          if (s_proc[i]) continue;
          nxt[T + (int)sbase] = nodes[i];
          sbase++;
        }
        __syncthreads();
        cur ^= 1;
        vcur ^= 1;
        nn = T + (int)stot;
        nvs = Mtot;
        OCT_T(4)
        if (nn >= N || nn == prev2) finish = true;
      }
    }
  }
  const ONode* nodes = s_nodes(cur);
  uint32_t* out = kept + (size_t)b * kp_cap + kept_off[l];
  for (int i = tid; i < nn; i += kOctThreads) {
    const ONode nd = nodes[i];
    uint32_t best = perm(pc)[nd.kb];
    for (int pb_ = nd.kb + 1; pb_ < nd.ke; pb_ += 8) {
      uint32_t t[8];
#pragma unroll
      for (int u = 0; u < 8; u++) t[u] = pb_ + u < nd.ke ? perm(pc)[pb_ + u] : 0u;
#pragma unroll
      for (int u = 0; u < 8; u++)
        if (pb_ + u < nd.ke && (t[u] >> 24) > (best >> 24)) best = t[u];
    }
    out[i] = best;
  }
  OCT_T(5)
  OCT_T_END
  if (tid == 0) kept_cnt[(size_t)b * nlevels + l] = nn;
}

__global__ __launch_bounds__(256) void k_kp_finalize(const LevelDev* __restrict__ levels, int nlevels,
                                                     const uint32_t* __restrict__ kept, const int* __restrict__ kept_cnt,
                                                     const int* __restrict__ kept_off, int kp_cap, int lap0, int lap1,
                                                     KpIn* __restrict__ kpin, int* __restrict__ kp_count,
                                                     int* __restrict__ mono_out) {
  __shared__ unsigned long long s_w64[4];
  __shared__ int s_base[2];
  const int b = blockIdx.x, tid = threadIdx.x;
  const uint32_t* kp = kept + (size_t)b * kp_cap;
  const int* cnt = kept_cnt + (size_t)b * nlevels;
  int total = 0;
  for (int l = 0; l < nlevels; l++) total += cnt[l];
  KpIn* out = kpin + (size_t)b * kp_cap;
  if (tid == 0) {
    s_base[0] = 0;
    s_base[1] = 0;
  }
  __syncthreads();
  int rec = 0;
  for (int l = 0; l < nlevels; l++) {
    const float scale = levels[l].scale;
    const int nl_ = cnt[l];
    for (int i0 = 0; i0 < nl_; i0 += 256) {
      const int i = i0 + tid;
      const bool valid = i < nl_;
      KpIn k;
      bool stereo = false;
      if (valid) {
        const uint32_t v = kp[kept_off[l] + i];
        k.x = (float)((int)(v & 0xfff) + 16);
        k.y = (float)((int)((v >> 12) & 0xfff) + 16);
        k.level = l;
        k.response = (float)(v >> 24);
        const float sx = l ? __fmul_rn(k.x, scale) : k.x;
        stereo = sx >= (float)lap0 && sx <= (float)lap1;
      }
      unsigned long long tot;
      const unsigned long long pre = oct_scan_u64(valid ? (stereo ? (1ull << 32) : 1ull) : 0ull, s_w64, &tot);
      if (valid) {
        const int mono_rank = s_base[0] + (int)(pre & 0xffffffffull), st_rank = s_base[1] + (int)(pre >> 32);
        k.slot = stereo ? (total - 1 - st_rank) : mono_rank;
        out[rec + i] = k;
      }
      __syncthreads();
      if (tid == 0) {
        s_base[0] += (int)(tot & 0xffffffffull);
        s_base[1] += (int)(tot >> 32);
      }
      __syncthreads();
    }
    rec += nl_;
  }
  if (tid == 0) {
    kp_count[b] = total;
    mono_out[b] = s_base[0];
  }
}

__device__ __forceinline__ int reflect101(int p, int n) {
  if (p < 0) p = -p;
  if (p >= n) p = 2 * (n - 1) - p;
  return p;
}

constexpr int kBlurTW = 64, kBlurTH = 32;
__global__ __launch_bounds__(256) void k_blur7(const LevelDev* __restrict__ levels,
                                               const BlurTileDev* __restrict__ tiles, Lvl0 l0,
                                               const uint8_t* __restrict__ pyr, size_t pyr_frame,
                                               uint8_t* __restrict__ blur, size_t blur_frame, int t0, int t1, int t2,
                                               int t3) {
  __shared__ __align__(16) uint32_t raw[kBlurTH + 6][18];
  __shared__ __align__(16) uint16_t hb[kBlurTH + 6][kBlurTW];
  const BlurTileDev T = tiles[blockIdx.x];
  const int b = blockIdx.y;
  struct {
    int rows, cols, pitch;
    unsigned blur_off;
  } L = {T.rows, T.cols, T.pitch, T.blur_off};
  const int sp = T.level == 0 ? l0.pitch : T.pitch;
  const uint8_t* src = T.level == 0 ? l0.base + (size_t)b * l0.frame_stride : pyr + (size_t)b * pyr_frame + T.plane_off;
  const int x0 = T.tx * kBlurTW, y0 = T.ty * kBlurTH;
  const int tid = threadIdx.x;
  const bool word_ok = ((sp & 3) == 0) && ((reinterpret_cast<size_t>(src) & 3) == 0);
  constexpr int kWords = (kBlurTH + 6) * 18, kIt = (kWords + 255) / 256;
  uint32_t v[kIt];
#pragma unroll
  for (int it = 0; it < kIt; it++) {
    const int i = tid + it * 256;
    v[it] = 0;
    if (i < kWords) {
      const int r = i / 18, w = i - r * 18;
      const int sy = reflect101(y0 + r - 3, L.rows);
      const int xb = x0 - 4 + 4 * w;
      if (word_ok && xb >= 0 && xb + 3 < L.cols) {
        v[it] = *reinterpret_cast<const uint32_t*>(src + (size_t)sy * sp + xb);
      } else {
#pragma unroll
        for (int k = 0; k < 4; k++) {
          const int sx = reflect101(xb + k, L.cols);
          const int sxc = min(max(sx, 0), L.cols - 1);
          v[it] |= (uint32_t)src[(size_t)sy * sp + sxc] << (8 * k);
        }
      }
    }
  }
#pragma unroll
  for (int it = 0; it < kIt; it++) {
    const int i = tid + it * 256;
    if (i < kWords) (&raw[0][0])[i] = v[it];
  }
  __syncthreads();
  for (int i = tid; i < (kBlurTH + 6) * (kBlurTW / 4); i += 256) {
    const int r = i >> 4, g = i & 15;
    const uint32_t w0 = raw[r][g], w1 = raw[r][g + 1], w2 = raw[r][g + 2];
    typedef unsigned short us2 __attribute__((ext_vector_type(2)));
    auto pair = [&](int i) -> us2 {
      const uint32_t hi = i + 1 <= 7 ? w1 : w2, lo = i + 1 <= 7 ? w0 : w1;
      const uint32_t j = i + 1 <= 7 ? i : i - 4;
      const uint32_t v = __builtin_amdgcn_perm(hi, lo, j | (0x0cu << 8) | ((j + 1) << 16) | (0x0cu << 24));
      return __builtin_bit_cast(us2, v);
    };
    const us2 T0 = {(unsigned short)t0, (unsigned short)t0}, T1 = {(unsigned short)t1, (unsigned short)t1},
              T2 = {(unsigned short)t2, (unsigned short)t2}, T3 = {(unsigned short)t3, (unsigned short)t3};
    uint32_t o2[2];
#pragma unroll
    for (int h2 = 0; h2 < 2; h2++) {
      const int b0 = 1 + 2 * h2;
      const us2 v = (pair(b0) + pair(b0 + 6)) * T0 + (pair(b0 + 1) + pair(b0 + 5)) * T1 + (pair(b0 + 2) + pair(b0 + 4)) * T2 + pair(b0 + 3) * T3;
      o2[h2] = __builtin_bit_cast(uint32_t, v);
    }
    *reinterpret_cast<uint2*>(&hb[r][4 * g]) = make_uint2(o2[0], o2[1]);
  }
  __syncthreads();
  uint8_t* dst = blur + (size_t)b * blur_frame + L.blur_off;
  for (int i = tid; i < kBlurTH * (kBlurTW / 4); i += 256) {
    const int r = i >> 4, g = i & 15;
    const int y = y0 + r, x = x0 + 4 * g;
    if (y >= L.rows || x >= L.cols) continue;
    unsigned acc[4] = {0, 0, 0, 0};
    const int taps[7] = {t0, t1, t2, t3, t2, t1, t0};
#pragma unroll
    for (int j = 0; j < 7; j++) {
      const uint2 h = *reinterpret_cast<const uint2*>(&hb[r + j][4 * g]);
      typedef unsigned short us2 __attribute__((ext_vector_type(2)));
      const us2 hx = __builtin_bit_cast(us2, h.x), hy = __builtin_bit_cast(us2, h.y);
      const unsigned short tj = (unsigned short)taps[j];
      acc[0] += (unsigned)hx.x * (unsigned)tj;
      acc[1] += (unsigned)hx.y * (unsigned)tj;
      acc[2] += (unsigned)hy.x * (unsigned)tj;
      acc[3] += (unsigned)hy.y * (unsigned)tj;
    }
    uint32_t pk = 0;
#pragma unroll
    for (int k = 0; k < 4; k++) pk |= min((acc[k] + 32768u) >> 16, 255u) << (8 * k);
    uint8_t* d = dst + (size_t)y * L.pitch + x;
    if (x + 3 < L.cols) {
      *reinterpret_cast<uint32_t*>(d) = pk;
    } else {
      for (int k = 0; k < 4 && x + k < L.cols; k++) d[k] = (uint8_t)(pk >> (8 * k));
    }
  }
}

__device__ __forceinline__ float fast_atan2_deg(float y, float x) {
  const float p1 = 0.9997878412794807f * (float)(180 / 3.14159265358979323846);
  const float p3 = -0.3258083974640975f * (float)(180 / 3.14159265358979323846);
  const float p5 = 0.1555786518463281f * (float)(180 / 3.14159265358979323846);
  const float p7 = -0.04432655554792128f * (float)(180 / 3.14159265358979323846);
  const float eps = (float)2.2204460492503131e-16;
  const float ax = fabsf(x), ay = fabsf(y);
  float a, c, c2;
  if (ax >= ay) {
    c = __fdiv_rn(ay, __fadd_rn(ax, eps));
    c2 = __fmul_rn(c, c);
    a = __fmul_rn(__fadd_rn(__fmul_rn(__fadd_rn(__fmul_rn(__fadd_rn(__fmul_rn(p7, c2), p5), c2), p3), c2), p1), c);
  } else {
    c = __fdiv_rn(ax, __fadd_rn(ay, eps));
    c2 = __fmul_rn(c, c);
    a = __fsub_rn(90.f, __fmul_rn(__fadd_rn(__fmul_rn(__fadd_rn(__fmul_rn(__fadd_rn(__fmul_rn(p7, c2), p5), c2), p3), c2), p1), c));
  }
  if (x < 0) a = __fsub_rn(180.f, a);
  if (y < 0) a = __fsub_rn(360.f, a);
  return a;
}

__device__ __forceinline__ float sincos_poly(double x, double x2, int n, bool flip) {
  const double C0 = 0x1p0, C1 = -0x1.ffffffd0c621cp-2, C2 = 0x1.55553e1068f19p-5, C3 = -0x1.6c087e89a359dp-10,
               C4 = 0x1.99343027bf8c3p-16;
  const double S1 = -0x1.555545995a603p-3, S2 = 0x1.1107605230bc4p-7, S3 = -0x1.994eb3774cf24p-13;
  if ((n & 1) == 0) {
    const double x3 = __dmul_rn(x, x2);
    const double s1 = __fma_rn(x2, S3, S2);
    const double x7 = __dmul_rn(x3, x2);
    const double s = __fma_rn(x3, S1, x);
    return (float)__fma_rn(x7, s1, s);
  }
  const double sg = flip ? -1.0 : 1.0;
  const double x4 = __dmul_rn(x2, x2);
  const double c2 = __fma_rn(x2, sg * C4, sg * C3);
  const double c1 = __fma_rn(x2, sg * C1, sg * C0);
  const double x6 = __dmul_rn(x4, x2);
  const double c = __fma_rn(x4, sg * C2, c1);
  return (float)__fma_rn(x6, c2, c);
}
__device__ __forceinline__ unsigned abstop12(float x) { return (__float_as_uint(x) >> 20) & 0x7ff; }
__device__ __forceinline__ void glibc_sincosf(float y, float* sn, float* cs) {
  double x = (double)y;
  if (abstop12(y) < abstop12(0x1.921FB6p-1f)) {
    if (abstop12(y) < abstop12(0x1p-12f)) {
      *sn = y;
      *cs = 1.0f;
      return;
    }
    const double x2 = __dmul_rn(x, x);
    *sn = sincos_poly(x, x2, 0, false);
    *cs = sincos_poly(x, x2, 1, false);
    return;
  }
  const double r = __dmul_rn(x, 0x1.45F306DC9C883p+23);
  const int n = ((int)r + 0x800000) >> 24;
  x = __fma_rn(-(double)n, 0x1.921FB54442D18p0, x);
  const double sgn = ((n & 3) == 1 || (n & 3) == 2) ? -1.0 : 1.0;
  const bool flip = (n & 2) != 0;
  const double x2 = __dmul_rn(x, x);
  const double xs = __dmul_rn(x, sgn);
  *sn = sincos_poly(xs, x2, n, flip);
  *cs = sincos_poly(xs, x2, n ^ 1, flip);
}

__device__ __forceinline__ int round_half_away(float x) {
  float r = truncf(x);
  const float diff = __fsub_rn(x, r);
  if (fabsf(diff) >= 0.5f) r = __fadd_rn(r, copysignf(1.f, x));
  return (int)r;
}

constexpr int kObGroup = 16;
constexpr int kObPerWg = 256 / kObGroup;
constexpr int kObHalf = 18, kObRows = 2 * kObHalf + 1, kObRowWords = 10;
__global__ __launch_bounds__(256) void k_orient_brief(const LevelDev* __restrict__ levels, Lvl0 l0,
                                                      const uint8_t* __restrict__ pyr, size_t pyr_frame,
                                                      const uint8_t* __restrict__ blur, size_t blur_frame,
                                                      const KpIn* __restrict__ kpin, const int* __restrict__ kp_count,
                                                      int kp_cap, const int* __restrict__ umax,
                                                      const int8_t* __restrict__ pattern, gfs_keypoint* __restrict__ kps,
                                                      uint8_t* __restrict__ desc, int xcd_frames, int nchunks) {
  int wg_chunk = blockIdx.x, wg_frame = blockIdx.y;
  if (xcd_frames > 0) {
    const int id = blockIdx.x, slot = id >> 3;
    wg_frame = (slot / nchunks) * 8 + (id & 7);
    wg_chunk = slot % nchunks;
    if (wg_frame >= xcd_frames) return;
  }
  __shared__ uint2 s_w[31 * 8];
  __shared__ uint32_t s_patch[kObPerWg][kObRows * kObRowWords];
  if (threadIdx.x < 31 * 8) {
    const int r = threadIdx.x >> 3, j = threadIdx.x & 7, v = r - 15, um = umax[v < 0 ? -v : v];
    unsigned W = 0, M = 0;
#pragma unroll
    for (int q = 0; q < 4; q++) {
      const int u = -16 + 4 * j + q;
      if (u >= -um && u <= um) {
        W |= (unsigned)(u + 16) << (8 * q);
        M |= 1u << (8 * q);
      }
    }
    s_w[threadIdx.x] = make_uint2(W, M);
  }
  __syncthreads();
  const int sl = threadIdx.x & (kObGroup - 1);
  const int b = wg_frame, n_kp = kp_count[b];
  const int k_raw = wg_chunk * kObPerWg + (threadIdx.x / kObGroup);
  if ((int)(wg_chunk * kObPerWg + (threadIdx.x >> 6) * (64 / kObGroup)) >= n_kp) return;
  const bool live = k_raw < n_kp;
  const int k = live ? k_raw : n_kp - 1;
  const KpIn in = kpin[(size_t)b * kp_cap + k];
  const LevelDev L = levels[in.level];
  int sp;
  const uint8_t* src = level_ptr(L, in.level, b, l0, pyr, pyr_frame, &sp);
  const int cx = __float2int_rn(in.x), cy = __float2int_rn(in.y);
  const uint8_t* bl = blur + (size_t)b * blur_frame + L.blur_off;
  const int bx = round_half_away(in.x), by = round_half_away(in.y);
  const uint8_t* bc = bl + (size_t)by * L.pitch + bx;
  const uint8_t* wcorner = bc - (size_t)kObHalf * L.pitch - kObHalf;
// ... 30 lines not shown
        sW = __builtin_amdgcn_udot4(w, wm.x, sW, false);
        sM += dm;
        m01 += (r - 15) * dm;
      }
    }
    m10 = (int)sW - 16 * sM;
  }
#pragma unroll
  for (int ofs = kObGroup / 2; ofs > 0; ofs >>= 1) {
    m10 += __shfl_xor(m10, ofs, kObGroup);
    m01 += __shfl_xor(m01, ofs, kObGroup);
  }
  const float angle = fast_atan2_deg((float)m01, (float)m10);
  const float factorPI = (float)(3.14159265358979323846 / 180.f);
  float a, bb;
  glibc_sincosf(__fmul_rn(angle, factorPI), &bb, &a);
  __builtin_amdgcn_fence(__ATOMIC_RELEASE, "wavefront");
  __builtin_amdgcn_wave_barrier();
  __builtin_amdgcn_fence(__ATOMIC_ACQUIRE, "wavefront");
  const uint8_t* win = reinterpret_cast<const uint8_t*>(mp) + kObHalf * (4 * kObRowWords) + kObHalf + ax;
  unsigned bits = 0;
#pragma unroll
  for (int q = 0; q < 4; q++) {
    const int4 pw = *reinterpret_cast<const int4*>(pattern + 64 * sl + 16 * q);
    const int words[4] = {pw.x, pw.y, pw.z, pw.w};
#pragma unroll
    for (int t = 0; t < 4; t++) {
      const int wv = words[t];
      const float x0 = (float)(int8_t)(wv & 0xff), y0 = (float)(int8_t)((wv >> 8) & 0xff);
      const float x1 = (float)(int8_t)((wv >> 16) & 0xff), y1 = (float)(int8_t)((wv >> 24) & 0xff);
      const int r0 = round_half_away(__fadd_rn(__fmul_rn(x0, bb), __fmul_rn(y0, a)));
      const int c0 = round_half_away(__fsub_rn(__fmul_rn(x0, a), __fmul_rn(y0, bb)));
      const int r1 = round_half_away(__fadd_rn(__fmul_rn(x1, bb), __fmul_rn(y1, a)));
      const int c1 = round_half_away(__fsub_rn(__fmul_rn(x1, a), __fmul_rn(y1, bb)));
      const int v0 = win[r0 * (4 * kObRowWords) + c0], v1 = win[r1 * (4 * kObRowWords) + c1];
      bits |= (unsigned)(v0 < v1) << (4 * q + t);
    }
  }
  if (!live) return;
  const size_t o = (size_t)b * kp_cap + in.slot;
  *reinterpret_cast<unsigned short*>(desc + o * 32 + 2 * sl) = (unsigned short)bits;
  if (sl == 0) {
    gfs_keypoint kp;
    kp.x = in.level ? __fmul_rn(in.x, L.scale) : in.x;
    kp.y = in.level ? __fmul_rn(in.y, L.scale) : in.y;
    kp.size = L.patch_size;
    kp.angle = angle;
    kp.response = in.response;
    kp.octave = in.level;
    kp.class_id = -1;
    kps[o] = kp;
  }
}

const int8_t kPattern[256 * 4] = {
#include "brief_pattern.inc"
};
const int kBlurTaps[2][4] = {{18, 34, 48, 56}, {18, 34, 49, 55}};

class WorkerPool {
 public:
  explicit WorkerPool(int n) : n_(std::max(1, n)) {
    for (int t = 1; t < n_; t++) th_.emplace_back([this, t]() { loop(t); });
  }
  ~WorkerPool() {
    {
      std::lock_guard<std::mutex> lk(mu_);
      quit_ = true;
      gen_++;
    }
    cv_.notify_all();
    for (auto& x : th_) x.join();
  }
  int size() const { return n_; }
  void run(int n, const std::function<void(int, int)>& f) {
    if (n <= 0) return;
    {
      std::lock_guard<std::mutex> lk(mu_);
      fn_ = &f;
      total_ = n;
      next_.store(0);
      pending_ = n_ - 1;
      gen_++;
    }
    cv_.notify_all();
    work(0);
    std::unique_lock<std::mutex> lk(mu_);
    done_cv_.wait(lk, [this]() { return pending_ == 0; });
    fn_ = nullptr;
  }

 private:
  void work(int t) {
    for (;;) {
      const int i = next_.fetch_add(1);
      if (i >= total_) break;
      (*fn_)(i, t);
    }
  }
  void loop(int t) {
    unsigned long seen = 0;
    for (;;) {
      {
        std::unique_lock<std::mutex> lk(mu_);
        cv_.wait(lk, [&]() { return gen_ != seen; });
        seen = gen_;
        if (quit_) return;
      }
      work(t);
      {
        std::lock_guard<std::mutex> lk(mu_);
        if (--pending_ == 0) done_cv_.notify_one();
      }
    }
  }
  int n_;
  std::vector<std::thread> th_;
  std::mutex mu_;
  std::condition_variable cv_, done_cv_;
  const std::function<void(int, int)>* fn_ = nullptr;
  std::atomic<int> next_{0};
  int total_ = 0, pending_ = 0;
  unsigned long gen_ = 0;
  bool quit_ = false;
};

}

struct gfs_orb {
  gfs_orb_config cfg;
  gfs::OrbParams P;
  gfs::OrbGeometry G;
  int geom_rows = 0, geom_cols = 0;
  size_t cap_pyr = 0, cap_blur = 0, cap_slab = 0, cap_cells = 0;
  int cap_kp = 0;
  hipStream_t stream = nullptr;
  hipEvent_t ev_copy = nullptr;
  std::mutex mu;
  int host_threads = 1;
  std::unique_ptr<WorkerPool> pool;
  gfs::DevBuf<uint8_t> d_stage, d_pyr, d_blur;
  gfs::DevBuf<LevelDev> d_levels;
  gfs::DevBuf<CellDev> d_cells;
  gfs::DevBuf<BlurTileDev> d_tiles;
  gfs::DevBuf<int> d_strip_rows, d_strip_rows_fine, d_xt_start, d_xt_n, d_yt_start, d_yt_n, d_cell_cnt, d_cand_off, d_kp_count, d_mono;
  gfs::DevBuf<float> d_xt_alpha, d_yt_alpha;
  gfs::DevBuf<uint32_t> d_slab, d_cand, d_perm0, d_perm1, d_kept;
  gfs::DevBuf<unsigned short> d_seg0, d_seg1;
  gfs::DevBuf<int> d_kept_cnt, d_kept_off;
  int oct_node_cap = kOctMaxNodes;
  bool cands_packed = false;
  bool device_octree = true;
  bool pyr_in_hbm = false;
  bool octree_supported = true;
  bool host_counts_valid = false, host_cands_valid = false;
  gfs::DevBuf<KpIn> d_kpin;
  gfs::DevBuf<gfs_keypoint> d_kps;
  gfs::DevBuf<uint8_t> d_desc;
  gfs::DevBuf<int8_t> d_pattern;
  gfs::DevBuf<int> d_umax;
  gfs::PinBuf<int> h_cand_off, h_kp_count, h_mono;
  gfs::PinBuf<uint32_t> h_cand;
  gfs::PinBuf<KpIn> h_kpin;
  int geometry_builds = 0;
  int last_B = 0;
  Lvl0 last_l0{};
  std::vector<gfs::OctreeScratch> scratch;
  std::vector<std::vector<int>> kept;
};

namespace {

enum PyrKernel { kPyrNone = 0, kPyrLds = 1, kPyrHbm = 2 };
struct PyrPath {
  PyrKernel kernel;
  bool fine;
};
inline PyrPath pyr_path(const gfs_orb* h, int B) {
  const gfs::OrbGeometry& G = h->G;
  if (G.pyr_strips <= 0) return {kPyrNone, false};
  if (G.pyr_lds_a + G.pyr_lds_b > 0 && !h->pyr_in_hbm) return {kPyrLds, G.pyr_strips_fine > 0 && B * G.pyr_strips < 128};
  return {kPyrHbm, false};
}
inline bool octree_on_device(const gfs_orb* h) { return h->device_octree && h->octree_supported; }

int ensure_geometry(gfs_orb* h, int rows, int cols) {
  if (h->geom_rows == rows && h->geom_cols == cols) return GFS_OK;
  GFS_REQUIRE(rows <= h->cfg.max_rows && cols <= h->cfg.max_cols, GFS_ERR_CAPACITY,
              "image %dx%d exceeds the handle's max %dx%d", cols, rows, h->cfg.max_cols, h->cfg.max_rows);
  gfs::OrbGeometry G;
  G.build(h->P, rows, cols);
  GFS_REQUIRE(G.supported, GFS_ERR_UNSUPPORTED, "ORB geometry for %dx%d unsupported: %s", cols, rows, G.why);
  GFS_REQUIRE(kFcWaves * G.fast_lds_wave <= 160 * 1024 && G.max_tile_w + 6 <= 256 && (G.max_tile_w + 6) * G.max_tile_h < 16384,
              GFS_ERR_UNSUPPORTED, "FAST cell tile of %dx%d too large for LDS", cols, rows);
  GFS_REQUIRE(G.pyr_bytes <= h->cap_pyr && G.blur_bytes <= h->cap_blur && G.slab_entries <= h->cap_slab &&
                  G.cells.size() <= h->cap_cells && G.kp_cap <= h->cap_kp,
              GFS_ERR_CAPACITY, "image %dx%d needs more workspace than the handle reserved", cols, rows);
  hipStream_t s = h->stream;
  if (h->geom_rows != 0) GFS_HIP(hipDeviceSynchronize());
  GFS_HIP(hipMemcpyAsync(h->d_levels.p, G.levels.data(), G.levels.size() * sizeof(LevelDev), hipMemcpyHostToDevice, s));
  GFS_HIP(hipMemcpyAsync(h->d_cells.p, G.cells.data(), G.cells.size() * sizeof(CellDev), hipMemcpyHostToDevice, s));
  GFS_HIP(hipMemcpyAsync(h->d_tiles.p, G.blur_tiles.data(), G.blur_tiles.size() * sizeof(BlurTileDev), hipMemcpyHostToDevice, s));
  if (G.pyr_strips > 0) {
    GFS_HIP(hipMemcpyAsync(h->d_strip_rows.p, G.strip_rows.data(), G.strip_rows.size() * 4, hipMemcpyHostToDevice, s));
    if (G.pyr_strips_fine > 0)
      GFS_HIP(hipMemcpyAsync(h->d_strip_rows_fine.p, G.strip_rows_fine.data(), G.strip_rows_fine.size() * 4, hipMemcpyHostToDevice, s));
    GFS_HIP(hipMemcpyAsync(h->d_xt_start.p, G.xt_start.data(), G.xt_start.size() * 4, hipMemcpyHostToDevice, s));
    GFS_HIP(hipMemcpyAsync(h->d_xt_n.p, G.xt_n.data(), G.xt_n.size() * 4, hipMemcpyHostToDevice, s));
    GFS_HIP(hipMemcpyAsync(h->d_xt_alpha.p, G.xt_alpha.data(), G.xt_alpha.size() * 4, hipMemcpyHostToDevice, s));
    GFS_HIP(hipMemcpyAsync(h->d_yt_start.p, G.yt_start.data(), G.yt_start.size() * 4, hipMemcpyHostToDevice, s));
    GFS_HIP(hipMemcpyAsync(h->d_yt_n.p, G.yt_n.data(), G.yt_n.size() * 4, hipMemcpyHostToDevice, s));
    GFS_HIP(hipMemcpyAsync(h->d_yt_alpha.p, G.yt_alpha.data(), G.yt_alpha.size() * 4, hipMemcpyHostToDevice, s));
  }
  std::vector<int> kept_off(G.levels.size());
  {
    int o = 0;
    for (size_t l = 0; l < G.levels.size(); l++) {
      kept_off[l] = o;
      o += G.levels[l].kp_cap;
    }
  }
  GFS_HIP(hipMemcpyAsync(h->d_kept_off.p, kept_off.data(), kept_off.size() * sizeof(int), hipMemcpyHostToDevice, s));
  GFS_HIP(hipStreamSynchronize(s));
  h->octree_supported = G.oct_on_device;
  h->oct_node_cap = G.oct_node_cap;
  h->G = std::move(G);
  h->geom_rows = rows;
  h->geom_cols = cols;
  h->geometry_builds++;
  return GFS_OK;
}

int run_batch(gfs_orb* h, Lvl0 l0, int B, int rows, int cols, int lap0, int lap1, hipStream_t s) {
  const gfs::OrbGeometry& G = h->G;
  const int nl = h->P.nlevels;
  const int n_cells = (int)G.cells.size();
  const size_t cap_pyr = h->cap_pyr, cap_blur = h->cap_blur, cap_slab = h->cap_slab;
  const PyrPath pp = pyr_path(h, B);
  if (pp.kernel == kPyrLds) {
    const bool fine = pp.fine;
    const int S = fine ? G.pyr_strips_fine : G.pyr_strips;
    const size_t la = fine ? G.pyr_lds_a_fine : G.pyr_lds_a, lb = fine ? G.pyr_lds_b_fine : G.pyr_lds_b;
    const size_t lx = fine ? G.pyr_lds_x_fine : G.pyr_lds_x;
    GFS_LAUNCH("k_pyr_area_lds", k_pyr_area_lds, dim3(S, B), dim3(kPyrThreads), la + lb + lx, s, h->d_levels.p, nl, l0, h->d_pyr.p, cap_pyr,
               fine ? h->d_strip_rows_fine.p : h->d_strip_rows.p, (unsigned)la, lx ? (unsigned)(la + lb) : 0u, (int)G.xt_start.size(),
               h->d_xt_start.p, h->d_xt_n.p, h->d_xt_alpha.p,
               h->d_yt_start.p, h->d_yt_n.p, h->d_yt_alpha.p);
  } else if (pp.kernel == kPyrHbm) {
    GFS_LAUNCH("k_pyr_area_hbm", k_pyr_area_hbm, dim3(G.pyr_strips, B), dim3(kPyrThreads), 0, s, h->d_levels.p, nl, l0, h->d_pyr.p,
               cap_pyr, h->d_strip_rows.p, h->d_xt_start.p, h->d_xt_n.p, h->d_xt_alpha.p, h->d_yt_start.p, h->d_yt_n.p,
               h->d_yt_alpha.p);
  }
  const FastMap fm = fast_map(B, n_cells);
  GFS_LAUNCH("k_fast_cells", k_fast_cells, dim3(fm.grid), dim3(64 * kFcWaves), (size_t)kFcWaves * G.fast_lds_wave, s, h->d_cells.p, l0,
             h->d_pyr.p, cap_pyr, h->P.ini_th, h->P.min_th, n_cells, fm, (int)G.fast_lds_wave, cap_slab, h->d_slab.p, h->d_cell_cnt.p);
  const int* tp = kBlurTaps[h->P.blur_variant ? 1 : 0];
  if (octree_on_device(h)) {
    GFS_LAUNCH("k_octree", k_octree, dim3(B * nl), dim3(kOctThreads), oct_lds_bytes(h->oct_node_cap), s, h->d_levels.p, nl, nullptr,
               nullptr, cap_slab, h->d_perm0.p, h->d_perm1.p, h->d_seg0.p, h->d_seg1.p, h->d_kept_off.p, h->cap_kp, h->d_kept.p,
               h->d_kept_cnt.p, h->oct_node_cap, h->d_cells.p, h->d_cell_cnt.p, n_cells, h->d_slab.p);
    h->cands_packed = false;
    GFS_LAUNCH("k_kp_finalize", k_kp_finalize, dim3(B), dim3(256), 0, s, h->d_levels.p, nl, h->d_kept.p, h->d_kept_cnt.p,
               h->d_kept_off.p, h->cap_kp, lap0, lap1, h->d_kpin.p, h->d_kp_count.p, h->d_mono.p);
    GFS_LAUNCH("k_blur7", k_blur7, dim3((unsigned)G.blur_tiles.size(), B), dim3(256), 0, s, h->d_levels.p, h->d_tiles.p, l0,
               h->d_pyr.p, cap_pyr, h->d_blur.p, cap_blur, tp[0], tp[1], tp[2], tp[3]);
    {
      static const bool ob_xcd = !(getenv("GFS_ORB_OB_XCD") && atoi(getenv("GFS_ORB_OB_XCD")) == 0);
      const int nch = gfs::div_up(h->cap_kp, kObPerWg);
      const bool by_xcd = ob_xcd && B >= 8;
      GFS_LAUNCH("k_orient_brief", k_orient_brief, by_xcd ? dim3((unsigned)(gfs::div_up(B, 8) * 8 * nch)) : dim3(nch, B), dim3(256), 0, s,
                 h->d_levels.p, l0, h->d_pyr.p, cap_pyr, h->d_blur.p, cap_blur, h->d_kpin.p, h->d_kp_count.p, h->cap_kp, h->d_umax.p,
                 h->d_pattern.p, h->d_kps.p, h->d_desc.p, by_xcd ? B : 0, nch);
    }
    h->last_B = B;
    h->last_l0 = l0;
    h->host_counts_valid = false;
    h->host_cands_valid = false;
    return GFS_OK;
  }
  GFS_LAUNCH("k_cand_pack", k_cand_pack, dim3(B), dim3(256), 0, s, h->d_levels.p, h->d_cells.p, nl, n_cells, cap_slab, h->d_slab.p,
             h->d_cell_cnt.p, cap_slab, h->d_cand.p, h->d_cand_off.p);
  GFS_HIP(hipMemcpyAsync(h->h_cand_off.p, h->d_cand_off.p, (size_t)B * (nl + 1) * sizeof(int), hipMemcpyDeviceToHost, s));
  GFS_HIP(hipStreamSynchronize(s));
  int max_total = 0;
  for (int b = 0; b < B; b++) max_total = std::max(max_total, h->h_cand_off.p[(size_t)b * (nl + 1) + nl]);
  if (max_total > 0)
    GFS_HIP(hipMemcpy2DAsync(h->h_cand.p, cap_slab * 4, h->d_cand.p, cap_slab * 4, (size_t)max_total * 4, B,
                             hipMemcpyDeviceToHost, s));
  GFS_HIP(hipEventRecord(h->ev_copy, s));
  GFS_LAUNCH("k_blur7", k_blur7, dim3((unsigned)G.blur_tiles.size(), B), dim3(256), 0, s, h->d_levels.p, h->d_tiles.p, l0,
             h->d_pyr.p, cap_pyr, h->d_blur.p, cap_blur, tp[0], tp[1], tp[2], tp[3]);
  GFS_HIP(hipEventSynchronize(h->ev_copy));
  const int ntask = B * nl;
  if ((int)h->kept.size() < ntask) h->kept.resize(ntask);
  if ((int)h->scratch.size() < h->host_threads) h->scratch.resize(h->host_threads);
  h->pool->run(ntask, [&](int t, int tid) {
    const int b = t / nl, l = t % nl;
    const int* off = h->h_cand_off.p + (size_t)b * (nl + 1);
    const LevelDev& L = G.levels[l];
    std::vector<int>& out = h->kept[t];
    out.clear();
    gfs::distribute_octree(h->h_cand.p + (size_t)b * cap_slab + off[l], off[l + 1] - off[l], 16, L.max_bx, 16, L.max_by,
                           L.quota, h->scratch[tid], out);
  });
  int max_n = 0;
  for (int b = 0; b < B; b++) {
    int n = 0;
    for (int l = 0; l < nl; l++) n += (int)h->kept[(size_t)b * nl + l].size();
    GFS_REQUIRE(n <= h->cap_kp, GFS_ERR_CAPACITY, "internal: %d keypoints exceed capacity %d", n, h->cap_kp);
    h->h_kp_count.p[b] = n;
    max_n = std::max(max_n, n);
    int mono = 0, stereo = n - 1, i = 0;
    const int* off = h->h_cand_off.p + (size_t)b * (nl + 1);
    KpIn* rec = h->h_kpin.p + (size_t)b * h->cap_kp;
    for (int l = 0; l < nl; l++) {
      const uint32_t* c = h->h_cand.p + (size_t)b * cap_slab + off[l];
      const float scale = h->P.scale[l];
      for (int idx : h->kept[(size_t)b * nl + l]) {
        KpIn k;
        k.x = (float)(gfs::cand_x(c[idx]) + 16);
        k.y = (float)(gfs::cand_y(c[idx]) + 16);
        k.level = l;
        k.response = (float)gfs::cand_score(c[idx]);
        const float sx = l ? k.x * scale : k.x;
        if (sx >= lap0 && sx <= lap1)
          k.slot = stereo--;
        else
          k.slot = mono++;
        rec[i++] = k;
      }
    }
    h->h_mono.p[b] = mono;
  }
  GFS_HIP(hipMemcpyAsync(h->d_kp_count.p, h->h_kp_count.p, (size_t)B * sizeof(int), hipMemcpyHostToDevice, s));
  GFS_HIP(hipMemcpyAsync(h->d_mono.p, h->h_mono.p, (size_t)B * sizeof(int), hipMemcpyHostToDevice, s));
  if (max_n > 0) {
    GFS_HIP(hipMemcpy2DAsync(h->d_kpin.p, (size_t)h->cap_kp * sizeof(KpIn), h->h_kpin.p, (size_t)h->cap_kp * sizeof(KpIn),
                             (size_t)max_n * sizeof(KpIn), B, hipMemcpyHostToDevice, s));
    GFS_LAUNCH("k_orient_brief", k_orient_brief, dim3(gfs::div_up(max_n, kObPerWg), B), dim3(256), 0, s, h->d_levels.p, l0,
               h->d_pyr.p, cap_pyr, h->d_blur.p, cap_blur, h->d_kpin.p, h->d_kp_count.p, h->cap_kp, h->d_umax.p,
               h->d_pattern.p, h->d_kps.p, h->d_desc.p, 0, 0);
  }
  h->last_B = B;
  h->last_l0 = l0;
  h->host_counts_valid = true;
  h->host_cands_valid = true;
  h->cands_packed = true;
  return GFS_OK;
}

int sync_host_view(gfs_orb* h, bool want_candidates) {
  if (h->host_counts_valid && (!want_candidates || h->host_cands_valid)) return GFS_OK;
  const int B = h->last_B, nl = h->P.nlevels;
  GFS_HIP(hipDeviceSynchronize());
  GFS_HIP(hipMemcpy(h->h_kp_count.p, h->d_kp_count.p, (size_t)B * sizeof(int), hipMemcpyDeviceToHost));
  GFS_HIP(hipMemcpy(h->h_mono.p, h->d_mono.p, (size_t)B * sizeof(int), hipMemcpyDeviceToHost));
  h->host_counts_valid = true;
  if (want_candidates) {
    if (!h->cands_packed) {
      const int n_cells = (int)h->G.cells.size();
      GFS_LAUNCH("k_cand_pack", k_cand_pack, dim3(B), dim3(256), 0, h->stream, h->d_levels.p, h->d_cells.p, nl, n_cells, h->cap_slab,
                 h->d_slab.p, h->d_cell_cnt.p, h->cap_slab, h->d_cand.p, h->d_cand_off.p);
      GFS_HIP(hipDeviceSynchronize());
      h->cands_packed = true;
    }
    GFS_HIP(hipMemcpy(h->h_cand_off.p, h->d_cand_off.p, (size_t)B * (nl + 1) * sizeof(int), hipMemcpyDeviceToHost));
    GFS_HIP(hipMemcpy(h->h_cand.p, h->d_cand.p, (size_t)B * h->cap_slab * sizeof(uint32_t), hipMemcpyDeviceToHost));
    h->host_cands_valid = true;
  }
  return GFS_OK;
}

}

extern "C" {

void gfs_orb_default_config(gfs_orb_config* c) {
  if (!c) return;
  c->nfeatures = 1000;
  c->scale_factor = 1.2f;
  c->nlevels = 8;
  c->ini_th_fast = 20;
  c->min_th_fast = 7;
  c->max_rows = 480;
  c->max_cols = 640;
  c->max_batch = 1;
  c->device = 0;
  c->blur_taps_variant = 0;
}

int gfs_orb_create(const gfs_orb_config* cfg, gfs_orb** out) {
  GFS_REQUIRE(cfg && out, GFS_ERR_INVALID_ARG, "gfs_orb_create: NULL argument");
  GFS_REQUIRE(cfg->nfeatures > 0 && cfg->nlevels > 0 && cfg->nlevels <= 16 && cfg->scale_factor > 1.f &&
                  cfg->max_rows > 0 && cfg->max_cols > 0 && cfg->max_batch > 0,
              GFS_ERR_INVALID_ARG, "gfs_orb_create: invalid configuration");
  if (!gfs::device_ok(cfg->device)) return GFS_ERR_NO_DEVICE;
  GFS_HIP(hipSetDevice(cfg->device));
  std::unique_ptr<gfs_orb> h(new gfs_orb);
  h->cfg = *cfg;
  h->P.init(cfg->nfeatures, cfg->scale_factor, cfg->nlevels, cfg->ini_th_fast, cfg->min_th_fast, cfg->blur_taps_variant);
  gfs::OrbGeometry G;
  G.build(h->P, cfg->max_rows, cfg->max_cols);
  GFS_REQUIRE(G.supported, GFS_ERR_UNSUPPORTED, "ORB geometry for max size %dx%d unsupported: %s", cfg->max_cols,
              cfg->max_rows, G.why);
  GFS_REQUIRE(kFcWaves * G.fast_lds_wave <= 160 * 1024 && G.max_tile_w + 6 <= 256 && (G.max_tile_w + 6) * G.max_tile_h < 16384, GFS_ERR_UNSUPPORTED,
              "FAST cell tile too large for LDS");
  const size_t B = cfg->max_batch;
  h->cap_pyr = G.pyr_bytes + 4096;
  h->cap_blur = G.blur_bytes + 4096;
  h->cap_slab = G.slab_entries + 1024;
  h->cap_cells = G.cells.size() + 64;
  h->cap_kp = G.kp_cap + 8;
  const int nl = cfg->nlevels;
  GFS_HIP(hipStreamCreateWithFlags(&h->stream, hipStreamNonBlocking));
  GFS_HIP(hipEventCreateWithFlags(&h->ev_copy, hipEventDisableTiming));
  int rc = 0;
  const size_t tab_x = (size_t)cfg->max_cols * nl + 64, tab_y = (size_t)cfg->max_rows * nl + 64;
#define A(x) if (!rc) rc = (x)
  A(h->d_stage.alloc(B * (size_t)cfg->max_rows * cfg->max_cols));
  A(h->d_pyr.alloc(B * h->cap_pyr));
  A(h->d_blur.alloc(B * h->cap_blur));
  A(h->d_levels.alloc(nl));
  A(h->d_cells.alloc(h->cap_cells));
  A(h->d_tiles.alloc(G.blur_tiles.size() + 64));
  A(h->d_strip_rows.alloc((size_t)2 * gfs::OrbGeometry::kPyrMaxStrips * 16));
  A(h->d_strip_rows_fine.alloc((size_t)2 * gfs::OrbGeometry::kPyrMaxStrips * 16));
  GFS_HIP(hipFuncSetAttribute(reinterpret_cast<const void*>(&k_pyr_area_lds), hipFuncAttributeMaxDynamicSharedMemorySize,
                              (int)gfs::OrbGeometry::kPyrLdsBudget));
  GFS_HIP(hipFuncSetAttribute((const void*)k_octree, hipFuncAttributeMaxDynamicSharedMemorySize, (int)oct_lds_bytes(kOctMaxNodes)));
  GFS_HIP(hipFuncSetAttribute((const void*)k_fast_cells, hipFuncAttributeMaxDynamicSharedMemorySize, 160 * 1024));
  A(h->d_xt_start.alloc(tab_x));
  A(h->d_xt_n.alloc(tab_x));
  A(h->d_xt_alpha.alloc(tab_x * 4));
  A(h->d_yt_start.alloc(tab_y));
  A(h->d_yt_n.alloc(tab_y));
  A(h->d_yt_alpha.alloc(tab_y * 4));
  A(h->d_cell_cnt.alloc(B * h->cap_cells));
  A(h->d_cand_off.alloc(B * (nl + 1)));
  A(h->d_kp_count.alloc(B));
  A(h->d_mono.alloc(B));
  A(h->d_slab.alloc(B * h->cap_slab));
  A(h->d_cand.alloc(B * h->cap_slab));
  A(h->d_kpin.alloc(B * h->cap_kp));
  A(h->d_perm0.alloc(B * h->cap_slab + 64));
  A(h->d_perm1.alloc(B * h->cap_slab + 64));
  A(h->d_seg0.alloc(B * h->cap_slab + 64));
  A(h->d_seg1.alloc(B * h->cap_slab + 64));
  A(h->d_kept.alloc(B * h->cap_kp));
  A(h->d_kept_cnt.alloc(B * nl));
  A(h->d_kept_off.alloc(nl));
  A(h->d_kps.alloc(B * h->cap_kp));
  A(h->d_desc.alloc(B * h->cap_kp * 32));
  A(h->h_cand_off.alloc(B * (nl + 1)));
  A(h->h_kp_count.alloc(B));
  A(h->h_mono.alloc(B));
  A(h->h_cand.alloc(B * h->cap_slab));
  A(h->h_kpin.alloc(B * h->cap_kp));
  A(h->d_umax.alloc(16));
  A(h->d_pattern.alloc(1024));
#undef A
  if (rc) return rc;
  for (int i = 0; i < 512; i++) {
    const double x = (double)(int8_t)kPattern[2 * i], y = (double)(int8_t)kPattern[2 * i + 1];
    GFS_REQUIRE(std::sqrt(x * x + y * y) + 0.5 < (double)(kObHalf + 1), GFS_ERR_UNSUPPORTED,
                "a BRIEF test point lies outside the %d x %d window of k_orient_brief", kObRows, kObRows);
  }
  GFS_HIP(hipMemcpy(h->d_umax.p, h->P.umax, 16 * sizeof(int), hipMemcpyHostToDevice));
  GFS_HIP(hipMemcpy(h->d_pattern.p, kPattern, 1024, hipMemcpyHostToDevice));
  GFS_HIP(hipMemset(h->d_kp_count.p, 0, B * sizeof(int)));
  GFS_HIP(hipStreamSynchronize(nullptr));
  h->host_threads = (int)std::max(1u, std::min(16u, std::thread::hardware_concurrency()));
  if (const char* e = getenv("GFS_ORB_HOST_THREADS")) h->host_threads = std::max(1, atoi(e));
  h->pool.reset(new WorkerPool(h->host_threads));
  if (const char* e = getenv("GFS_ORB_OCTREE")) h->device_octree = strcmp(e, "host") != 0;
  h->pyr_in_hbm = getenv("GFS_ORB_PYR_HBM") != nullptr;
  *out = h.release();
  return GFS_OK;
}

void gfs_orb_destroy(gfs_orb* h) {
  if (!h) return;
  (void)hipSetDevice(h->cfg.device);
  if (h->stream) (void)hipStreamSynchronize(h->stream);
  if (h->ev_copy) (void)hipEventDestroy(h->ev_copy);
  if (h->stream) (void)hipStreamDestroy(h->stream);
  delete h;
}

int gfs_orb_get_tables(const gfs_orb* h, float* scale, float* inv_scale, float* sigma2, float* inv_sigma2,
                       int32_t* feats, int32_t* umax16) {
  GFS_REQUIRE(h, GFS_ERR_INVALID_ARG, "gfs_orb_get_tables: NULL handle");
  for (int i = 0; i < h->P.nlevels; i++) {
    if (scale) scale[i] = h->P.scale[i];
    if (inv_scale) inv_scale[i] = h->P.inv_scale[i];
    if (sigma2) sigma2[i] = h->P.sigma2[i];
    if (inv_sigma2) inv_sigma2[i] = h->P.inv_sigma2[i];
    if (feats) feats[i] = h->P.quota[i];
  }
  if (umax16)
    for (int i = 0; i < 16; i++) umax16[i] = h->P.umax[i];
  return GFS_OK;
}

int gfs_orb_max_keypoints(const gfs_orb* h) { return h ? h->cap_kp : GFS_ERR_INVALID_ARG; }

int gfs_orb_extract_batch_device(gfs_orb* h, const void* dev_imgs, int B, int rows, int cols, int lap0, int lap1,
                                 void* stream) {
  GFS_REQUIRE(h && dev_imgs && B > 0 && rows > 0 && cols > 0, GFS_ERR_INVALID_ARG,
              "gfs_orb_extract_batch_device: invalid argument");
  GFS_REQUIRE(B <= h->cfg.max_batch, GFS_ERR_CAPACITY, "batch %d exceeds handle max_batch %d", B, h->cfg.max_batch);
  std::lock_guard<std::mutex> lk(h->mu);
  GFS_HIP(hipSetDevice(h->cfg.device));
  int rc = ensure_geometry(h, rows, cols);
  if (rc) return rc;
  Lvl0 l0{(const uint8_t*)dev_imgs, (size_t)rows * cols, cols};
  return run_batch(h, l0, B, rows, cols, lap0, lap1, stream ? (hipStream_t)stream : h->stream);
}

int gfs_orb_extract_batch(gfs_orb* h, const uint8_t* const* imgs, int B, int rows, int cols, int stride, int lap0,
                          int lap1, gfs_keypoint* kps, uint8_t* desc, int cap, int* n, int* mono_index) {
  GFS_REQUIRE(h && imgs && B > 0 && rows > 0 && cols > 0 && stride >= cols && n, GFS_ERR_INVALID_ARG,
              "gfs_orb_extract_batch: invalid argument");
  GFS_REQUIRE(B <= h->cfg.max_batch, GFS_ERR_CAPACITY, "batch %d exceeds handle max_batch %d", B, h->cfg.max_batch);
  std::lock_guard<std::mutex> lk(h->mu);
  GFS_HIP(hipSetDevice(h->cfg.device));
  int rc = ensure_geometry(h, rows, cols);
  if (rc) return rc;
  hipStream_t s = h->stream;
  for (int b = 0; b < B; b++)
    GFS_HIP(hipMemcpy2DAsync(h->d_stage.p + (size_t)b * rows * cols, cols, imgs[b], stride, cols, rows,
                             hipMemcpyHostToDevice, s));
  Lvl0 l0{h->d_stage.p, (size_t)rows * cols, cols};
  rc = run_batch(h, l0, B, rows, cols, lap0, lap1, s);
  if (rc) return rc;
  GFS_HIP(hipStreamSynchronize(s));
  if ((rc = sync_host_view(h, false))) return rc;
  for (int b = 0; b < B; b++) {
    const int nb = h->h_kp_count.p[b];
    n[b] = nb;
    if (mono_index) mono_index[b] = h->h_mono.p[b];
    if (nb > cap) {
      gfs::set_error("gfs_orb_extract_batch: %d keypoints exceed caller capacity %d", nb, cap);
      return GFS_ERR_CAPACITY;
    }
    if (nb && kps)
      GFS_HIP(hipMemcpyAsync(kps + (size_t)b * cap, h->d_kps.p + (size_t)b * h->cap_kp, (size_t)nb * sizeof(gfs_keypoint),
                             hipMemcpyDeviceToHost, s));
    if (nb && desc)
      GFS_HIP(hipMemcpyAsync(desc + (size_t)b * cap * 32, h->d_desc.p + (size_t)b * h->cap_kp * 32, (size_t)nb * 32,
                             hipMemcpyDeviceToHost, s));
  }
  GFS_HIP(hipStreamSynchronize(s));
  return GFS_OK;
}

int gfs_orb_extract(gfs_orb* h, const uint8_t* img, int rows, int cols, int stride, int lap0, int lap1,
                    gfs_keypoint* kps, uint8_t* desc, int cap, int* n) {
  if (n) *n = 0;
  if (!img || rows <= 0 || cols <= 0) return -1;
  int nn = 0, mono = 0;
  const uint8_t* imgs[1] = {img};
  int rc = gfs_orb_extract_batch(h, imgs, 1, rows, cols, stride, lap0, lap1, kps, desc, cap, &nn, &mono);
  if (n) *n = nn;
  if (rc) return rc - 100;
  return mono;
}

int gfs_orb_device_results(gfs_orb* h, void** dev_kps, void** dev_desc, void** dev_counts, void** dev_mono, int* cap) {
  GFS_REQUIRE(h, GFS_ERR_INVALID_ARG, "gfs_orb_device_results: NULL handle");
  if (dev_kps) *dev_kps = h->d_kps.p;
  if (dev_desc) *dev_desc = h->d_desc.p;
  if (dev_counts) *dev_counts = h->d_kp_count.p;
  if (dev_mono) *dev_mono = h->d_mono.p;
  if (cap) *cap = h->cap_kp;
  return GFS_OK;
}

int gfs_orb_fetch(gfs_orb* h, int b, gfs_keypoint* kps, uint8_t* desc, int cap, int* n, int* mono_index) {
  GFS_REQUIRE(h && b >= 0 && b < h->last_B, GFS_ERR_INVALID_ARG, "gfs_orb_fetch: invalid frame index");
  std::lock_guard<std::mutex> lk(h->mu);
  GFS_HIP(hipSetDevice(h->cfg.device));
  GFS_HIP(hipDeviceSynchronize());
  {
    const int rc0 = sync_host_view(h, false);
    if (rc0) return rc0;
  }
  const int nb = h->h_kp_count.p[b];
  if (n) *n = nb;
  if (mono_index) *mono_index = h->h_mono.p[b];
  GFS_REQUIRE(nb <= cap, GFS_ERR_CAPACITY, "gfs_orb_fetch: %d keypoints exceed caller capacity %d", nb, cap);
  if (nb && kps) GFS_HIP(hipMemcpy(kps, h->d_kps.p + (size_t)b * h->cap_kp, (size_t)nb * sizeof(gfs_keypoint), hipMemcpyDeviceToHost));
  if (nb && desc) GFS_HIP(hipMemcpy(desc, h->d_desc.p + (size_t)b * h->cap_kp * 32, (size_t)nb * 32, hipMemcpyDeviceToHost));
  return GFS_OK;
}

int gfs_orb_level_size(const gfs_orb* h, int level, int* rows, int* cols) {
  GFS_REQUIRE(h && level >= 0 && level < h->P.nlevels && h->geom_rows > 0, GFS_ERR_INVALID_ARG,
              "gfs_orb_level_size: invalid level or no image processed yet");
  *rows = h->G.levels[level].rows;
  *cols = h->G.levels[level].cols;
  return GFS_OK;
}

int gfs_orb_fetch_level(gfs_orb* h, int b, int level, int blurred, uint8_t* dst) {
  GFS_REQUIRE(h && dst && b >= 0 && b < h->last_B && level >= 0 && level < h->P.nlevels, GFS_ERR_INVALID_ARG,
              "gfs_orb_fetch_level: invalid argument");
  std::lock_guard<std::mutex> lk(h->mu);
  GFS_HIP(hipSetDevice(h->cfg.device));
  GFS_HIP(hipDeviceSynchronize());
  const LevelDev& L = h->G.levels[level];
  const uint8_t* src;
  size_t pitch;
  if (blurred) {
    src = h->d_blur.p + (size_t)b * h->cap_blur + L.blur_off;
    pitch = L.pitch;
  } else if (level == 0) {
    src = h->last_l0.base + (size_t)b * h->last_l0.frame_stride;
    pitch = h->last_l0.pitch;
  } else {
    src = h->d_pyr.p + (size_t)b * h->cap_pyr + L.plane_off;
    pitch = L.pitch;
  }
  GFS_HIP(hipMemcpy2D(dst, L.cols, src, pitch, L.cols, L.rows, hipMemcpyDeviceToHost));
  return GFS_OK;
}

int gfs_orb_fetch_candidates(gfs_orb* h, int b, int level, int32_t* x, int32_t* y, int32_t* score, int cap) {
  GFS_REQUIRE(h && b >= 0 && b < h->last_B && level >= 0 && level < h->P.nlevels, GFS_ERR_INVALID_ARG,
              "gfs_orb_fetch_candidates: invalid argument");
  std::lock_guard<std::mutex> lk(h->mu);
  GFS_HIP(hipSetDevice(h->cfg.device));
  {
    const int rc0 = sync_host_view(h, true);
    if (rc0) return rc0;
  }
  const int nl = h->P.nlevels;
  const int* off = h->h_cand_off.p + (size_t)b * (nl + 1);
  const int cnt = off[level + 1] - off[level];
  const uint32_t* c = h->h_cand.p + (size_t)b * h->cap_slab + off[level];
  for (int i = 0; i < cnt && i < cap; i++) {
    if (x) x[i] = gfs::cand_x(c[i]);
    if (y) y[i] = gfs::cand_y(c[i]);
    if (score) score[i] = gfs::cand_score(c[i]);
  }
  return cnt;
}

int gfs_orb_octree_device(int device, const int32_t* x, const int32_t* y, const int32_t* score, int n, int min_x, int max_x,
                          int min_y, int max_y, int n_features, int32_t* out_x, int32_t* out_y, int32_t* out_score, int cap) {
  if (!gfs::device_ok(device)) return GFS_ERR_NO_DEVICE;
  GFS_HIP(hipSetDevice(device));
  GFS_REQUIRE(min_x == 16 && min_y == 16 && n >= 0, GFS_ERR_INVALID_ARG, "gfs_orb_octree_device: min border must be 16");
  LevelDev L{};
  L.max_bx = max_x;
  L.max_by = max_y;
  L.quota = n_features;
  const gfs::OctLevelFit fit = gfs::oct_level_fit(max_x, max_y, n_features);
  GFS_REQUIRE(fit.on_device, GFS_ERR_UNSUPPORTED, "outside k_octree limits");
  const int kcap = n_features + 3 + 4 * fit.n_ini + 8;
  std::vector<uint32_t> c(std::max(n, 1));
  for (int i = 0; i < n; i++) c[i] = (uint32_t)x[i] | ((uint32_t)y[i] << 12) | ((uint32_t)score[i] << 24);
  gfs::DevBuf<LevelDev> dL;
  gfs::DevBuf<uint32_t> dc, p0, p1, dk;
  gfs::DevBuf<unsigned short> s0, s1;
  gfs::DevBuf<int> doff, dko, dcnt;
  int rc = 0;
  if ((rc = dL.alloc(1)) || (rc = dc.alloc(c.size())) || (rc = p0.alloc(c.size() + 64)) || (rc = p1.alloc(c.size() + 64)) ||
      (rc = s0.alloc(c.size() + 64)) || (rc = s1.alloc(c.size() + 64)) || (rc = dk.alloc(kcap)) || (rc = doff.alloc(2)) ||
      (rc = dko.alloc(1)) || (rc = dcnt.alloc(1)))
    return rc;
  const int off[2] = {0, n}, ko = 0;
  GFS_HIP(hipMemcpy(dL.p, &L, sizeof(L), hipMemcpyHostToDevice));
  GFS_HIP(hipMemcpy(dc.p, c.data(), c.size() * 4, hipMemcpyHostToDevice));
  GFS_HIP(hipMemcpy(doff.p, off, sizeof(off), hipMemcpyHostToDevice));
  GFS_HIP(hipMemcpy(dko.p, &ko, sizeof(ko), hipMemcpyHostToDevice));
  const int node_cap = (fit.nodes + 7) / 8 * 8;
  GFS_HIP(hipFuncSetAttribute((const void*)k_octree, hipFuncAttributeMaxDynamicSharedMemorySize, (int)oct_lds_bytes(kOctMaxNodes)));
  hipLaunchKernelGGL(k_octree, dim3(1), dim3(kOctThreads), oct_lds_bytes(node_cap), 0, dL.p, 1, dc.p, doff.p, c.size(), p0.p, p1.p, s0.p, s1.p,
                     dko.p, kcap, dk.p, dcnt.p, node_cap, (const CellDev*)nullptr, (const int*)nullptr, 0, (const uint32_t*)nullptr);
  GFS_HIP(hipDeviceSynchronize());
  int cnt = 0;
  GFS_HIP(hipMemcpy(&cnt, dcnt.p, sizeof(int), hipMemcpyDeviceToHost));
  std::vector<uint32_t> k(std::max(cnt, 1));
  if (cnt) GFS_HIP(hipMemcpy(k.data(), dk.p, (size_t)cnt * 4, hipMemcpyDeviceToHost));
  for (int i = 0; i < cnt && i < cap; i++) {
    out_x[i] = gfs::cand_x(k[i]);
    out_y[i] = gfs::cand_y(k[i]);
    out_score[i] = gfs::cand_score(k[i]);
  }
  return cnt;
}

int gfs_test_orb_last_paths(gfs_orb* h, gfs_test_orb_paths* out) {
  GFS_REQUIRE(h && out, GFS_ERR_INVALID_ARG, "gfs_test_orb_last_paths: NULL argument");
  std::lock_guard<std::mutex> lk(h->mu);
  const PyrPath pp = pyr_path(h, h->last_B);
  out->octree_on_device = octree_on_device(h) ? 1 : 0;
  out->pyr_kernel = (int)pp.kernel;
  out->pyr_fine_cut = pp.fine ? 1 : 0;
  out->geometry_builds = h->geometry_builds;
  out->last_batch = h->last_B;
  out->rows = h->geom_rows;
  out->cols = h->geom_cols;
  return GFS_OK;
}

int gfs_orb_octree_host(const int32_t* x, const int32_t* y, const int32_t* score, int n, int min_x, int max_x,
                        int min_y, int max_y, int n_features, int32_t* out_idx, int cap) {
  std::vector<uint32_t> c(n);
  for (int i = 0; i < n; i++) c[i] = (uint32_t)x[i] | ((uint32_t)y[i] << 12) | ((uint32_t)score[i] << 24);
  gfs::OctreeScratch S;
  std::vector<int> out;
  gfs::distribute_octree(c.data(), n, min_x, max_x, min_y, max_y, n_features, S, out);
  for (size_t i = 0; i < out.size() && (int)i < cap; i++) out_idx[i] = out[i];
  return (int)out.size();
}

}
```

### geoflowslam_amd/csrc/orb_host.cpp

```cpp
#include "orb_host.hpp"

#include <algorithm>
#include <array>
#include <cfloat>
#include <cmath>
#include <cstdlib>
#include <utility>

namespace gfs {

namespace {
inline int cv_round_f(float v) { return (int)std::lrintf(v); }
inline int cv_round_d(double v) { return (int)std::lrint(v); }
inline int cv_floor_d(double v) {
  int i = (int)v;
  return i - (i > v);
}
inline int cv_ceil_d(double v) {
  int i = (int)v;
  return i + (i < v);
}
}

void OrbParams::init(int nf, float sf, int nl, int ini, int mn, int bv) {
// ... 32 lines not shown
  for (v = 0; v < 16; v++) umax[v] = 0;
  for (v = 0; v <= vmax; ++v) umax[v] = cv_round_d(std::sqrt(hp2 - v * v));
  for (v = kHalfPatch, v0 = 0; v >= vmin; --v) {
    while (umax[v0] == umax[v0 + 1]) ++v0;
    umax[v] = v0;
    ++v0;
  }
}

static bool area_tab(int ssize, int dsize, std::vector<int>& start, std::vector<int>& cnt, std::vector<float>& alpha) {
  const double scale = 1. / ((double)dsize / ssize);
  for (int dx = 0; dx < dsize; dx++) {
    double fsx1 = dx * scale, fsx2 = fsx1 + scale;
    double cellWidth = std::min(scale, ssize - fsx1);
    int sx1 = cv_ceil_d(fsx1), sx2 = cv_floor_d(fsx2);
    sx2 = std::min(sx2, ssize - 1);
    sx1 = std::min(sx1, sx2);
    int s0 = -1, n = 0;
    float a[kMaxAreaTaps + 4];
    auto push = [&](int si, float al) {
      if (n == 0) s0 = si;
      if (n < kMaxAreaTaps + 4) a[n] = al;
      n++;
      return si == s0 + n - 1;
    };
    bool ok = true;
    if (sx1 - fsx1 > 1e-3) ok &= push(sx1 - 1, (float)((sx1 - fsx1) / cellWidth));
    for (int sx = sx1; sx < sx2; sx++) ok &= push(sx, float(1.0 / cellWidth));
    if (fsx2 - sx2 > 1e-3) ok &= push(sx2, (float)(std::min(std::min(fsx2 - sx2, 1.), cellWidth) / cellWidth));
    if (!ok || n == 0 || n > kMaxAreaTaps) return false;
    start.push_back(s0);
    cnt.push_back(n);
    for (int k = 0; k < kMaxAreaTaps; k++) alpha.push_back(k < n ? a[k] : 0.f);
  }
  return true;
}

OctLevelFit oct_level_fit(int max_bx, int max_by, int quota) {
  OctLevelFit f;
  f.n_ini = (int)std::round((float)(max_bx - 16) / (float)(max_by - 16));
  if (f.n_ini == 0) f.n_ini = 1;
  f.nodes = quota + 4 * f.n_ini + 8;
  f.on_device = f.n_ini <= 4 && f.nodes <= kOctMaxNodes;
  return f;
}

void OrbGeometry::build(const OrbParams& p, int rows_, int cols_) {
  rows = rows_;
  cols = cols_;
  levels.assign(p.nlevels, LevelDev{});
  cells.clear();
  blur_tiles.clear();
  xt_start.clear();
  yt_start.clear();
  xt_n.clear();
  yt_n.clear();
  xt_alpha.clear();
  yt_alpha.clear();
  supported = true;
  why = "";
  size_t pyr = 0, blur = 0, slab = 0;
  kp_cap = 0;
  max_tile_w = max_tile_h = 0;
  fast_lds_wave = 0;
  oct_on_device = true;
  oct_node_cap = 8;
  for (int l = 0; l < p.nlevels; l++) {
    LevelDev& L = levels[l];
    L.cols = cv_round_f((float)cols * p.inv_scale[l]);
    L.rows = cv_round_f((float)rows * p.inv_scale[l]);
    L.pitch = (int)((L.cols + 127) / 128 * 128);
    L.plane_off = (unsigned)pyr;
    if (l > 0) pyr += (size_t)L.pitch * L.rows;
    L.blur_off = (unsigned)blur;
    blur += (size_t)L.pitch * L.rows;
    L.scale = p.scale[l];
    L.patch_size = (float)(int)(kPatchSize * p.scale[l]);
    L.quota = p.quota[l];
    if (l > 0) {
      const LevelDev& S = levels[l - 1];
      const double sx = 1. / ((double)L.cols / S.cols), sy = 1. / ((double)L.rows / S.rows);
      const bool int_x = std::abs(sx - (int)std::lrint(sx)) < DBL_EPSILON, int_y = std::abs(sy - (int)std::lrint(sy)) < DBL_EPSILON;
      if (sx < 1 || sy < 1 || (int_x && int_y)) {
        supported = false;
        why = "level ratio must be > 1 and non-integer (cv::resize INTER_AREA general path)";
        return;
      }
      L.xtab_off = (int)xt_start.size();
      L.ytab_off = (int)yt_start.size();
      if (!area_tab(S.cols, L.cols, xt_start, xt_n, xt_alpha) || !area_tab(S.rows, L.rows, yt_start, yt_n, yt_alpha)) {
        supported = false;
        why = "INTER_AREA footprint wider than 4 source pixels (scale factor too large)";
        return;
      }
    }
    const int minBX = kEdgeThreshold - 3, minBY = minBX;
    L.max_bx = L.cols - kEdgeThreshold + 3;
    L.max_by = L.rows - kEdgeThreshold + 3;
    const float W = 35;
    const float width = (float)(L.max_bx - minBX), height = (float)(L.max_by - minBY);
    const int nCols = (int)(width / W), nRows = (int)(height / W);
    if (nCols < 1 || nRows < 1) {
      supported = false;
      why = "pyramid level smaller than one FAST cell (reference divides by zero here)";
      return;
    }
    L.n_cell_cols = nCols;
    L.n_cell_rows = nRows;
    L.w_cell = (int)std::ceil(width / nCols);
    L.h_cell = (int)std::ceil(height / nRows);
    L.cell_base = (int)cells.size();
    for (int i = 0; i < nRows; i++) {
      const float iniY = (float)(minBY + i * L.h_cell);
      float maxY = iniY + L.h_cell + 6;
      if (iniY >= L.max_by - 3) continue;
      if (maxY > L.max_by) maxY = (float)L.max_by;
      for (int j = 0; j < nCols; j++) {
        const float iniX = (float)(minBX + j * L.w_cell);
        float maxX = iniX + L.w_cell + 6;
        if (iniX >= L.max_bx - 6) continue;
        if (maxX > L.max_bx) maxX = (float)L.max_bx;
        CellDev c{};
        c.level = (short)l;
        c.x0 = (short)(int)iniX;
        c.y0 = (short)(int)iniY;
        c.w = (short)((int)maxX - (int)iniX);
        c.h = (short)((int)maxY - (int)iniY);
        const int dw = std::max(c.w - 6, 0), dh = std::max(c.h - 6, 0);
        c.pitch = L.pitch;
        c.plane_off = L.plane_off;
        c.slab_off = (unsigned)slab;
        c.slab_cap = (unsigned)(((dw + 1) / 2) * ((dh + 1) / 2));
        slab += c.slab_cap;
        max_tile_w = std::max(max_tile_w, (int)c.w);
        max_tile_h = std::max(max_tile_h, (int)c.h);
        if (dw > 0 && dh > 0) {
          const size_t wp = (size_t)((c.w + 6) & ~3);
          const size_t ng_min = (size_t)std::max(1, dw / 4), past = wp * (c.h + 64 / ng_min + 3) + 16;
          const size_t need = std::max(2 * (wp * c.h + 16) + 2 * (size_t)dw * dh + 16, past);
          fast_lds_wave = std::max(fast_lds_wave, (need + 15) & ~(size_t)15);
        }
        cells.push_back(c);
      }
    }
    L.n_cells = (int)cells.size() - L.cell_base;
    const OctLevelFit fit = oct_level_fit(L.max_bx, L.max_by, L.quota);
    L.kp_cap = L.quota + 3 + 4 * fit.n_ini;
    kp_cap += L.kp_cap;
    if (!fit.on_device) oct_on_device = false;
    oct_node_cap = std::min(std::max(oct_node_cap, (fit.nodes + 7) / 8 * 8), kOctMaxNodes);
    for (int ty = 0; ty < (L.rows + 31) / 32; ty++)
      for (int tx = 0; tx < (L.cols + 63) / 64; tx++) blur_tiles.push_back(BlurTileDev{(short)l, (short)tx, (short)ty, 0, L.rows, L.cols, L.pitch, L.plane_off, L.blur_off, 0u});
  }
  {
    auto at = [&](int l, int tx, int ty) -> const BlurTileDev* {
      for (const BlurTileDev& t : blur_tiles)
        if (t.level == l && t.tx == tx && t.ty == ty) return &t;
      return nullptr;
    };
    std::vector<std::array<BlurTileDev, 4>> quads;
    std::vector<std::array<BlurTileDev, 2>> pairs;
    std::vector<BlurTileDev> single;
    for (const BlurTileDev& t : blur_tiles) {
      if ((t.tx & 1) || (t.ty & 1)) {
        continue;
      }
      const BlurTileDev *r = at(t.level, t.tx + 1, t.ty), *d = at(t.level, t.tx, t.ty + 1), *rd = at(t.level, t.tx + 1, t.ty + 1);
      if (r && d && rd) {
        quads.push_back({t, *r, *d, *rd});
      } else if (r) {
        pairs.push_back({t, *r});
        if (d) single.push_back(*d);
      } else if (d) {
        pairs.push_back({t, *d});
      } else {
        single.push_back(t);
      }
    }
    std::vector<BlurTileDev> out;
    out.reserve(blur_tiles.size());
    size_t g = 0;
    for (; g + 8 <= quads.size(); g += 8)
      for (int k = 0; k < 4; k++)
        for (size_t i = 0; i < 8; i++) out.push_back(quads[g + i][k]);
    for (; g < quads.size(); g++) {
      pairs.push_back({quads[g][0], quads[g][1]});
      pairs.push_back({quads[g][2], quads[g][3]});
    }
    for (g = 0; g + 8 <= pairs.size(); g += 8)
      for (int k = 0; k < 2; k++)
        for (size_t i = 0; i < 8; i++) out.push_back(pairs[g + i][k]);
    for (; g < pairs.size(); g++) {
      out.push_back(pairs[g][0]);
      out.push_back(pairs[g][1]);
    }
    out.insert(out.end(), single.begin(), single.end());
    if (out.size() == blur_tiles.size()) blur_tiles.swap(out);
  }
  if (cols >= 4096 || rows >= 4096) {
    supported = false;
    why = "images must be smaller than 4096 x 4096 (12-bit packed candidate coordinates)";
    return;
  }
  pyr_bytes = pyr;
  blur_bytes = blur;
  slab_entries = slab;
  cand_cap = slab;
  pyr_strips = pyr_strips_fine = 0;
  pyr_lds_a = pyr_lds_b = pyr_lds_a_fine = pyr_lds_b_fine = pyr_lds_x = pyr_lds_x_fine = 0;
  strip_rows.clear();
  strip_rows_fine.clear();
  const int nl = p.nlevels;
  if (nl >= 2) {
    struct Cut {
      int S = 0;
      std::vector<int> tab;
      size_t la = 0, lb = 0;
      int tab_rows = 0;
      int prog_rows = 0;
    };
    auto cut = [&](int S) {
      Cut c;
      c.S = S;
      c.tab.assign((size_t)2 * S * nl, 0);
      for (int k = 0; k < S; k++) {
        int a = 0, b = 0, rows = 0, srows = 0;
        for (int l = nl - 1; l >= 0; l--) {
          const int R = levels[l].rows;
          int oa = l >= 1 ? (int)((long long)k * R / S) : 0, ob = l >= 1 ? (int)((long long)(k + 1) * R / S) : 0;
          if (l < nl - 1 && b > a) {
            const LevelDev& U = levels[l + 1];
            const int fa = yt_start[U.ytab_off + a], fb = yt_start[U.ytab_off + b - 1] + yt_n[U.ytab_off + b - 1];
            if (ob > oa) {
              oa = std::min(oa, fa);
              ob = std::max(ob, fb);
            } else {
              oa = fa;
              ob = fb;
            }
          }
          a = oa;
          b = ob;
          c.tab[2 * ((size_t)k * nl + l)] = a;
          c.tab[2 * ((size_t)k * nl + l) + 1] = b;
          const size_t bytes = (size_t)(b - a) * kPyrLdsPitch(levels[l].cols);
          if (l % 2 == 0) c.la = std::max(c.la, bytes);
          else c.lb = std::max(c.lb, bytes);
          if (l >= 1) rows += b - a;
          if (l < nl - 1) srows += b - a;
        }
        c.tab_rows = std::max(c.tab_rows, rows);
        c.prog_rows = std::max(c.prog_rows, srows);
      }
      c.la = (c.la + 15) / 16 * 16;
      c.lb = (c.lb + 15) / 16 * 16;
      return c;
    };
    const int cand[] = {4, 5, 6, 7, 8, 10, 12, 16, 24, 32, 48, 64};
    size_t budget = kPyrLdsBudget;
    if (const char* e = getenv("GFS_ORB_PYR_LDS_KB")) budget = std::min(kPyrLdsBudget, (size_t)std::max(8, atoi(e)) * 1024);
    size_t xbytes = 16 * xt_start.size();
    for (int n : xt_n)
      if (n > 3) xbytes = 0;
    if (getenv("GFS_ORB_PYR_XTAB_HBM")) xbytes = 0;
    std::vector<Cut> cuts;
    for (int S : cand) cuts.push_back(cut(S));
    bool streamable = true;
    for (int l = 1; l < nl && streamable; l++)
      for (int r = 0; r + 1 < levels[l].rows; r++) {
        const int i = levels[l].ytab_off + r, last = yt_start[i] + yt_n[i] - 1;
        if (yt_start[i + 1] < last || (yt_start[i + 1] == last && yt_n[i + 1] == 1)) {
          streamable = false;
          break;
        }
      }
    auto first_fit = [&](size_t extra) {
      for (size_t i = 0; i < cuts.size() && streamable; i++)
        if (cuts[i].la + cuts[i].lb + extra <= budget && cuts[i].tab_rows <= kPyrTabRows && cuts[i].prog_rows <= kPyrProgRows)
          return (int)i;
      return -1;
    };
    const int pick0 = first_fit(0), pickx = xbytes ? first_fit(xbytes) : -1;
    int pick = pick0;
    if (pickx >= 0 && 2 * cuts[pickx].S <= 3 * cuts[pick0].S) {
      pick = pickx;
      pyr_lds_x = xbytes;
    }
    if (pick < 0) {
      strip_rows = cuts.back().tab;
      pyr_strips = cuts.back().S;
    } else {
      strip_rows = cuts[pick].tab;
      pyr_strips = cuts[pick].S;
      pyr_lds_a = cuts[pick].la;
      pyr_lds_b = cuts[pick].lb;
      for (size_t i = pick + 1; i < cuts.size(); i++)
        if (cuts[i].S >= 4 * pyr_strips || i + 1 == cuts.size()) {
          strip_rows_fine = cuts[i].tab;
          pyr_strips_fine = cuts[i].S;
          pyr_lds_a_fine = cuts[i].la;
          pyr_lds_b_fine = cuts[i].lb;
          pyr_lds_x_fine = cuts[i].la + cuts[i].lb + xbytes <= budget ? xbytes : 0;
          break;
        }
    }
  }
}

void ic_angle_offsets(const int umax[16], std::vector<int8_t>& du, std::vector<int8_t>& dv) {
  du.clear();
  dv.clear();
  for (int u = -kHalfPatch; u <= kHalfPatch; ++u) {
    du.push_back((int8_t)u);
    dv.push_back(0);
  }
  for (int v = 1; v <= kHalfPatch; ++v) {
    const int d = umax[v];
    for (int u = -d; u <= d; ++u) {
      du.push_back((int8_t)u);
      dv.push_back((int8_t)v);
      du.push_back((int8_t)u);
      dv.push_back((int8_t)-v);
    }
  }
}

void distribute_octree(const uint32_t* c, int n, int min_x, int max_x, int min_y, int max_y, int N,
                       OctreeScratch& S, std::vector<int>& out) {
  if (n <= 0) return;
  int nIni = (int)std::round(static_cast<float>(max_x - min_x) / (max_y - min_y));
  if (nIni == 0) nIni = 1;
  const float hX = static_cast<float>(max_x - min_x) / nIni;
  auto& nodes = S.nodes;
  auto& perm = S.perm;
  auto& tmp = S.tmp;
  nodes.clear();
  perm.resize(n);
  tmp.resize(n);
  int head = -1, tail = -1, size = 0;
  auto push_back = [&](int idx) {
    nodes[idx].prev = tail;
    nodes[idx].next = -1;
    if (tail >= 0)
      nodes[tail].next = idx;
    else
      head = idx;
    tail = idx;
    size++;
  };
  auto push_front = [&](int idx) {
    nodes[idx].prev = -1;
    nodes[idx].next = head;
    if (head >= 0)
      nodes[head].prev = idx;
    else
      tail = idx;
    head = idx;
    size++;
  };
  auto erase = [&](int idx) {
    const int p = nodes[idx].prev, q = nodes[idx].next;
    if (p >= 0)
      nodes[p].next = q;
    else
      head = q;
    if (q >= 0)
      nodes[q].prev = p;
    else
      tail = p;
    size--;
  };
  std::vector<int> rcount(nIni + 1, 0);
  for (int i = 0; i < n; i++) {
    int r = (int)((float)cand_x(c[i]) / hX);
    r = std::min(std::max(r, 0), nIni - 1);
    tmp[i] = r;
    rcount[r + 1]++;
  }
  for (int r = 0; r < nIni; r++) rcount[r + 1] += rcount[r];
  {
    std::vector<int> pos(rcount.begin(), rcount.end() - 1);
    for (int i = 0; i < n; i++) perm[pos[tmp[i]]++] = i;
  }
  for (int r = 0; r < nIni; r++) {
    OctreeScratch::Node nd;
    nd.x0 = (int)(hX * static_cast<float>(r));
    nd.x1 = (int)(hX * static_cast<float>(r + 1));
    nd.y0 = 0;
    nd.y1 = max_y - min_y;
    nd.kb = rcount[r];
    nd.ke = rcount[r + 1];
    nd.no_more = false;
    nd.prev = nd.next = -1;
    nodes.push_back(nd);
    push_back((int)nodes.size() - 1);
  }
  for (int it = head; it >= 0;) {
    const int nx = nodes[it].next, cnt = nodes[it].ke - nodes[it].kb;
    if (cnt == 1)
      nodes[it].no_more = true;
    else if (cnt == 0)
      erase(it);
    it = nx;
  }

  std::vector<std::pair<int, int>> vsize, vprev;
  auto split = [&](int it, int* n_to_expand) {
    const OctreeScratch::Node P = nodes[it];
    const int halfX = (int)std::ceil(static_cast<float>(P.x1 - P.x0) / 2);
    const int halfY = (int)std::ceil(static_cast<float>(P.y1 - P.y0) / 2);
    const int xm = P.x0 + halfX, ym = P.y0 + halfY;
    int cnt[4] = {0, 0, 0, 0};
    for (int k = P.kb; k < P.ke; k++) {
      const uint32_t v = c[perm[k]];
      const int q = (cand_x(v) < xm ? 0 : 1) + (cand_y(v) < ym ? 0 : 2);
      tmp[k] = q;
      cnt[q]++;
    }
    int base[4] = {P.kb, P.kb + cnt[0], P.kb + cnt[0] + cnt[1], P.kb + cnt[0] + cnt[1] + cnt[2]};
    {
      int pos[4] = {base[0], base[1], base[2], base[3]};
      static thread_local std::vector<int> side;
      side.assign(perm.begin() + P.kb, perm.begin() + P.ke);
      for (int k = P.kb; k < P.ke; k++) perm[pos[tmp[k]]++] = side[k - P.kb];
    }
    const int bx0[4] = {P.x0, xm, P.x0, xm}, bx1[4] = {xm, P.x1, xm, P.x1};
    const int by0[4] = {P.y0, P.y0, ym, ym}, by1[4] = {ym, ym, P.y1, P.y1};
    for (int q = 0; q < 4; q++) {
      if (cnt[q] == 0) continue;
      OctreeScratch::Node ch;
      ch.x0 = bx0[q];
      ch.x1 = bx1[q];
      ch.y0 = by0[q];
      ch.y1 = by1[q];
      ch.kb = base[q];
      ch.ke = base[q] + cnt[q];
      ch.no_more = cnt[q] == 1;
      ch.prev = ch.next = -1;
      nodes.push_back(ch);
      const int idx = (int)nodes.size() - 1;
      push_front(idx);
      if (cnt[q] > 1) {
        if (n_to_expand) (*n_to_expand)++;
        vsize.push_back(std::make_pair(cnt[q], idx));
      }
    }
  };
  auto cmp = [&](const std::pair<int, int>& a, const std::pair<int, int>& b) {
    if (a.first < b.first) return true;
    if (a.first > b.first) return false;
    return nodes[a.second].x0 < nodes[b.second].x0;
  };

  bool finish = false;
  while (!finish) {
    int prev_size = size, n_to_expand = 0;
    vsize.clear();
    for (int it = head; it >= 0;) {
      if (nodes[it].no_more) {
        it = nodes[it].next;
        continue;
      }
      const int nx = nodes[it].next;
      split(it, &n_to_expand);
      erase(it);
      it = nx;
    }
    if (size >= N || size == prev_size) {
      finish = true;
    } else if (size + n_to_expand * 3 > N) {
      while (!finish) {
        prev_size = size;
        vprev = vsize;
        vsize.clear();
        std::sort(vprev.begin(), vprev.end(), cmp);
        for (int j = (int)vprev.size() - 1; j >= 0; j--) {
          split(vprev[j].second, nullptr);
          erase(vprev[j].second);
          if (size >= N) break;
        }
        if (size >= N || size == prev_size) finish = true;
      }
    }
  }
  for (int it = head; it >= 0; it = nodes[it].next) {
    int best = perm[nodes[it].kb], best_r = cand_score(c[best]);
    for (int k = nodes[it].kb + 1; k < nodes[it].ke; k++) {
      const int r = cand_score(c[perm[k]]);
      if (r > best_r) {
        best = perm[k];
        best_r = r;
      }
    }
    out.push_back(best);
  }
}

}

extern "C" int gfs_test_orb_blur_tiles(int rows, int cols, int nlevels, float scale_factor, int32_t* level_tx_ty, int cap) {
  gfs::OrbParams P;
  P.init(1000, scale_factor, nlevels, 20, 7, 1);
  gfs::OrbGeometry G;
  G.build(P, rows, cols);
  if (!G.supported) return -1;
  const int n = (int)G.blur_tiles.size();
  for (int i = 0; i < n && i < cap; i++) {
    level_tx_ty[3 * i] = G.blur_tiles[i].level;
    level_tx_ty[3 * i + 1] = G.blur_tiles[i].tx;
    level_tx_ty[3 * i + 2] = G.blur_tiles[i].ty;
  }
  return n;
}

#include "../../include/gfs_abi_test.h"
extern "C" int gfs_test_orb_geometry(int rows, int cols, int nfeatures, int nlevels, float scale_factor, gfs_test_orb_geometry_info* info,
                                     gfs_test_orb_level_info* levels, int cap_levels) {
  if (!info || rows <= 0 || cols <= 0 || nfeatures <= 0 || nlevels <= 0 || nlevels > 16 || !(scale_factor > 1.f)) return GFS_ERR_INVALID_ARG;
  gfs::OrbParams P;
  P.init(nfeatures, scale_factor, nlevels, 20, 7, 0);
  gfs::OrbGeometry G;
  G.build(P, rows, cols);
  *info = gfs_test_orb_geometry_info{};
  info->supported = G.supported ? 1 : 0;
  if (!G.supported) return GFS_ERR_UNSUPPORTED;
  info->pyr_strips = G.pyr_strips;
  info->pyr_strips_fine = G.pyr_strips_fine;
  info->pyr_in_lds = G.pyr_lds_a + G.pyr_lds_b > 0 ? 1 : 0;
  info->xtab_in_lds = G.pyr_lds_x > 0 ? 1 : 0;
  info->xtab_in_lds_fine = G.pyr_lds_x_fine > 0 ? 1 : 0;
  info->kp_cap = G.kp_cap;
  info->octree_on_device = G.oct_on_device ? 1 : 0;
  info->oct_node_cap = G.oct_node_cap;
  info->n_cells = (int)G.cells.size();
  info->n_blur_tiles = (int)G.blur_tiles.size();
  info->fast_lds_wave = (int)G.fast_lds_wave;
  for (int l = 0; l < nlevels && l < cap_levels && levels; l++) {
    const gfs::LevelDev& L = G.levels[l];
    const gfs::OctLevelFit fit = gfs::oct_level_fit(L.max_bx, L.max_by, L.quota);
    gfs_test_orb_level_info& o = levels[l];
    o.rows = L.rows;
    o.cols = L.cols;
    o.n_cell_cols = L.n_cell_cols;
    o.n_cell_rows = L.n_cell_rows;
    o.w_cell = L.w_cell;
    o.h_cell = L.h_cell;
    o.n_cells = L.n_cells;
    o.max_cell_w = o.max_cell_h = 0;
    for (int c = L.cell_base; c < L.cell_base + L.n_cells; c++) {
      o.max_cell_w = std::max(o.max_cell_w, (int)G.cells[c].w);
      o.max_cell_h = std::max(o.max_cell_h, (int)G.cells[c].h);
    }
    o.quota = L.quota;
    o.n_ini = fit.n_ini;
    o.kp_cap = L.kp_cap;
    o.octree_on_device = fit.on_device ? 1 : 0;
  }
  return nlevels;
}

#include "std_sort_replica.hpp"
extern "C" int gfs_test_sort_replica(int32_t* size_key, int32_t* x_key, int32_t* payload, int n) {
  struct E {
    int s, x, p;
  };
  std::vector<E> v(n);
  for (int i = 0; i < n; i++) v[i] = E{size_key[i], x_key[i], payload[i]};
  gfs::replica_std_sort(v.data(), v.data() + n, [](const E& a, const E& b) {
    if (a.s < b.s) return true;
    if (a.s > b.s) return false;
    return a.x < b.x;
  });
  for (int i = 0; i < n; i++) {
    size_key[i] = v[i].s;
    x_key[i] = v[i].x;
    payload[i] = v[i].p;
  }
  return n;
}
extern "C" int gfs_test_heap_sort_replica(int32_t* size_key, int32_t* x_key, int32_t* payload, int n) {
  struct E {
    int s, x, p;
  };
  std::vector<E> v(n);
  for (int i = 0; i < n; i++) v[i] = E{size_key[i], x_key[i], payload[i]};
  gfs::replica_heap_sort(v.data(), v.data() + n, [](const E& a, const E& b) {
    if (a.s < b.s) return true;
    if (a.s > b.s) return false;
    return a.x < b.x;
  });
  for (int i = 0; i < n; i++) {
    size_key[i] = v[i].s;
    x_key[i] = v[i].x;
    payload[i] = v[i].p;
  }
  return n;
}
```

### geoflowslam_amd/csrc/orb_host.hpp

```cpp
#pragma once
#include <cstddef>
#include <cstdint>
#include <vector>

namespace gfs {

constexpr int kPatchSize = 31;
constexpr int kHalfPatch = 15;
constexpr int kEdgeThreshold = 19;
constexpr int kMaxAreaTaps = 4;

constexpr int kOctMaxNodes = 768;
struct OctLevelFit {
  int n_ini;
  int nodes;
  bool on_device;
};
OctLevelFit oct_level_fit(int max_bx, int max_by, int quota);

struct LevelDev {
  int rows, cols, pitch;
  unsigned plane_off;
  unsigned blur_off;
  int xtab_off, ytab_off;
  int w_cell, h_cell, n_cell_cols, n_cell_rows, cell_base, n_cells;
  int max_bx, max_by;
  float scale;
  float patch_size;
  int quota;
  int kp_cap;
};

struct CellDev {
  short level, x0, y0, w, h;
  short pad;
  unsigned slab_off;
  unsigned slab_cap;
  int pitch;
  unsigned plane_off;
  unsigned pad2;
};

struct BlurTileDev {
  short level, tx, ty, pad;
  int rows, cols, pitch;
  unsigned plane_off, blur_off;
  unsigned pad2;
};

struct OrbParams {
  int nfeatures, nlevels, ini_th, min_th, blur_variant;
  float scale_factor;
  std::vector<float> scale, inv_scale, sigma2, inv_sigma2;
  std::vector<int> quota;
  int umax[16];
  void init(int nfeatures, float scale_factor, int nlevels, int ini_th, int min_th, int blur_variant);
};

struct OrbGeometry {
  int rows = 0, cols = 0;
  std::vector<LevelDev> levels;
  std::vector<CellDev> cells;
  std::vector<BlurTileDev> blur_tiles;
  std::vector<int> xt_start, yt_start;
  std::vector<int> xt_n, yt_n;
  std::vector<float> xt_alpha, yt_alpha;
  static constexpr int kPyrTabRows = 384, kPyrProgRows = 512;
  static constexpr size_t kPyrLdsBudget = 150 * 1024;
  static constexpr int kPyrLdsPitch(int cols) { return (cols + 3) & ~3; }
  size_t pyr_lds_x = 0, pyr_lds_x_fine = 0;
  std::vector<int> strip_rows;
  int pyr_strips = 0;
  size_t pyr_lds_a = 0, pyr_lds_b = 0;
  std::vector<int> strip_rows_fine;
  int pyr_strips_fine = 0;
  size_t pyr_lds_a_fine = 0, pyr_lds_b_fine = 0;
  static constexpr int kPyrMaxStrips = 64;
  size_t pyr_bytes = 0, blur_bytes = 0;
  size_t slab_entries = 0;
  size_t cand_cap = 0;
  int kp_cap = 0;
  int max_tile_w = 0, max_tile_h = 0;
  size_t fast_lds_wave = 0;
  bool oct_on_device = true;
  int oct_node_cap = 8;
  bool supported = true;
  const char* why = "";
  void build(const OrbParams& p, int rows, int cols);
};

void ic_angle_offsets(const int umax[16], std::vector<int8_t>& du, std::vector<int8_t>& dv);

struct OctreeScratch {
  std::vector<int> perm, tmp;
  struct Node {
    int x0, x1, y0, y1;
    int kb, ke;
    int prev, next;
    bool no_more;
  };
  std::vector<Node> nodes;
};
void distribute_octree(const uint32_t* packed, int n, int min_x, int max_x, int min_y, int max_y, int N,
                       OctreeScratch& scratch, std::vector<int>& out);

inline int cand_x(uint32_t c) { return (int)(c & 0xfff); }
inline int cand_y(uint32_t c) { return (int)((c >> 12) & 0xfff); }
inline int cand_score(uint32_t c) { return (int)(c >> 24); }

}
```

Before: 46980 frames/s.

## Fuse 7-tap Gaussian blur into LDS pyramid kernel for leading levels

Adds a blur phase inside the LDS-resident pyramid kernel so the first N pyramid levels are blurred straight from shared memory. Strip row ranges are widened by a 3-row halo so each strip holds the rows it needs, and the separate k_blur7 launch now covers only the remaining levels' tiles. The goal is to avoid re-reading pyramid planes from HBM and to cut blur tile work in the separate kernel. In exchange the strips carry extra halo rows and more LDS, and the number of fused levels is limited by an LDS and work-balance check.

```diff
diff --git a/geoflowslam_amd/api.py b/geoflowslam_amd/api.py
--- a/geoflowslam_amd/api.py
+++ b/geoflowslam_amd/api.py
@@ -43,6 +43,10 @@
 
 
 ORB_PYR_NONE, ORB_PYR_LDS, ORB_PYR_HBM = 0, 1, 2
+
+
+class OrbBlurPath(C.Structure):
+    _fields_ = _i32_fields("fused fused_levels strips separate_tiles")
 
 
 class GicpConfig(C.Structure):
@@ -832,7 +836,8 @@
     "gfs_orb_extract", "gfs_orb_extract_batch", "gfs_orb_extract_batch_device", "gfs_orb_device_results",
     "gfs_orb_fetch", "gfs_orb_level_size", "gfs_orb_fetch_level", "gfs_orb_fetch_candidates", "gfs_orb_octree_host",
     "gfs_orb_octree_device", "gfs_test_sort_replica", "gfs_test_heap_sort_replica", "gfs_test_glibc_math", "gfs_test_traffic",
-    "gfs_test_orb_blur_tiles", "gfs_test_orb_geometry", "gfs_test_orb_last_paths",
+    "gfs_test_orb_blur_tiles", "gfs_test_orb_geometry", "gfs_test_orb_last_paths", "gfs_test_orb_last_blur_path",
+    "gfs_test_orb_strip_rows",
     "gfs_hamming256", "gfs_matcher_create", "gfs_matcher_destroy", "gfs_bf_match_hamming",
     "gfs_bf_match_hamming_batch_device",
     "gfs_gicp_default_config", "gfs_gicp_create", "gfs_gicp_destroy", "gfs_gicp_align", "gfs_gicp_align_batch_device",
@@ -899,6 +904,8 @@
         L.gfs_orb_fetch_candidates.argtypes = [vp, i, i, vp, vp, vp, i]
         L.gfs_test_orb_geometry.argtypes = [i, i, i, i, C.c_float, C.POINTER(OrbGeometryInfo), vp, i]
         L.gfs_test_orb_last_paths.argtypes = [vp, C.POINTER(OrbPaths)]
+        L.gfs_test_orb_last_blur_path.argtypes = [vp, C.POINTER(OrbBlurPath)]
+        L.gfs_test_orb_strip_rows.argtypes = [i, i, i, C.c_float, i, i, vp, vp, vp, i]
         L.gfs_orb_octree_host.argtypes = [vp, vp, vp, i, i, i, i, i, i, vp, i]
         L.gfs_orb_octree_device.argtypes = [i, vp, vp, vp, i, i, i, i, i, i, vp, vp, vp, i]
         L.gfs_test_glibc_math.argtypes = [i, vp, i, vp, vp, vp]
@@ -1197,6 +1204,31 @@
         _check(lib().gfs_test_orb_last_paths(self.h, C.byref(P)), "gfs_test_orb_last_paths")
         return {n: int(getattr(P, n)) for n, _ in OrbPaths._fields_}
 
+    def last_blur_path(self):
+        P = OrbBlurPath()
+        _check(lib().gfs_test_orb_last_blur_path(self.h, C.byref(P)), "gfs_test_orb_last_blur_path")
+        return {n: int(getattr(P, n)) for n, _ in OrbBlurPath._fields_}
+
+
+def orb_strip_rows(rows, cols, nlevels=8, scale_factor=1.2, blur_fuse=-1, fine=False):
+    info = np.zeros(4, np.int32)
+    cap = 2 * max(64 * nlevels, 2 * rows * nlevels)
+    tab, yt = np.zeros(cap, np.int32), np.zeros(cap, np.int32)
+    n = lib().gfs_test_orb_strip_rows(rows, cols, nlevels, scale_factor, blur_fuse, int(fine), _p(info), _p(tab), _p(yt), cap)
+    if n == -5:
+        return None
+    _check(n, "gfs_test_orb_strip_rows")
+    S = int(info[0])
+    g = orb_geometry(rows, cols, 1000, nlevels, scale_factor)
+    taps, o = [None], 0
+    for l in range(1, nlevels):
+        r = g["levels"][l]["rows"]
+        taps.append(yt[2 * o:2 * (o + r)].reshape(r, 2).copy())
+        o += r
+    return dict(strips=S, fused_levels=int(info[1]), separate_tiles=int(info[2]), in_lds=bool(info[3]),
+                rows=tab[:n].reshape(S, nlevels, 2).copy() if S else np.zeros((0, nlevels, 2), np.int32), taps=taps,
+                level_rows=[g["levels"][l]["rows"] for l in range(nlevels)])
+
 
 def orb_geometry(rows, cols, nfeatures=1000, nlevels=8, scale_factor=1.2):
     I = OrbGeometryInfo()
diff --git a/geoflowslam_amd/csrc/orb.hip b/geoflowslam_amd/csrc/orb.hip
--- a/geoflowslam_amd/csrc/orb.hip
+++ b/geoflowslam_amd/csrc/orb.hip
@@ -40,6 +40,32 @@
   return pyr + (size_t)b * pyr_frame + L.plane_off;
 }
 
+__device__ __forceinline__ int reflect101(int p, int n) {
+  if (p < 0) p = -p;
+  if (p >= n) p = 2 * (n - 1) - p;
+  return p;
+}
+
+__device__ __forceinline__ uint2 blur_h4(uint32_t w0, uint32_t w1, uint32_t w2, int t0, int t1, int t2, int t3) {
+  typedef unsigned short us2 __attribute__((ext_vector_type(2)));
+  auto pair = [&](int i) -> us2 {
+    const uint32_t hi = i + 1 <= 7 ? w1 : w2, lo = i + 1 <= 7 ? w0 : w1;
+    const uint32_t j = i + 1 <= 7 ? i : i - 4;
+    const uint32_t v = __builtin_amdgcn_perm(hi, lo, j | (0x0cu << 8) | ((j + 1) << 16) | (0x0cu << 24));
+    return __builtin_bit_cast(us2, v);
+  };
+  const us2 T0 = {(unsigned short)t0, (unsigned short)t0}, T1 = {(unsigned short)t1, (unsigned short)t1},
+            T2 = {(unsigned short)t2, (unsigned short)t2}, T3 = {(unsigned short)t3, (unsigned short)t3};
+  uint32_t o2[2];
+#pragma unroll
+  for (int h2 = 0; h2 < 2; h2++) {
+    const int b0 = 1 + 2 * h2;
+    const us2 v = (pair(b0) + pair(b0 + 6)) * T0 + (pair(b0 + 1) + pair(b0 + 5)) * T1 + (pair(b0 + 2) + pair(b0 + 4)) * T2 + pair(b0 + 3) * T3;
+    o2[h2] = __builtin_bit_cast(uint32_t, v);
+  }
+  return make_uint2(o2[0], o2[1]);
+}
+
 constexpr int kPyrThreads = 1024, kPyrWaves = kPyrThreads / 64;
 constexpr int kPyrTabRows = gfs::OrbGeometry::kPyrTabRows, kPyrProgRows = gfs::OrbGeometry::kPyrProgRows;
 typedef float pyr_f2 __attribute__((ext_vector_type(2)));
@@ -50,7 +76,9 @@
                                                               unsigned lds_x, int xt_total,
                                                               const int* __restrict__ xt_start, const int* __restrict__ xt_n,
                                                               const float* __restrict__ xt_alpha, const int* __restrict__ yt_start,
-                                                              const int* __restrict__ yt_n, const float* __restrict__ yt_alpha) {
+                                                              const int* __restrict__ yt_n, const float* __restrict__ yt_alpha,
+                                                              uint8_t* __restrict__ blur, size_t blur_frame, int blur_levels, int t0,
+                                                              int t1, int t2, int t3) {
   extern __shared__ __align__(16) uint8_t smem[];
   __shared__ float4 s_prog[kPyrProgRows + 1];
   __shared__ int s_first[kPyrTabRows];
@@ -174,6 +202,99 @@
 #ifdef GFS_PYR_TIMING
   { const long long _n = clock64(); if (tid == 0) pyr_t[8] = _n; }
 #endif
+  auto blur_phase = [&](int l, unsigned off, int h0, int nheld) {
+    typedef unsigned short us2 __attribute__((ext_vector_type(2)));
+    const LevelDev BL = levels[l];
+    const int R = BL.rows, C = BL.cols;
+    const int ba = gfs::OrbGeometry::blur_share(k, (int)gridDim.x, R), bb = gfs::OrbGeometry::blur_share(k + 1, (int)gridDim.x, R);
+    const int nrow = bb - ba;
+    if (nrow <= 0) return;
+    const int spw = gfs::OrbGeometry::kPyrLdsPitch(C) >> 2;
+    const int ng = (C + 3) >> 2, nchunk = (ng + 61) / 62, cg = (ng + nchunk - 1) / nchunk;
+    const int units = nchunk * nrow;
+    const int u1 = (int)((long long)(wave + 1) * units / kPyrWaves);
+    int u = (int)((long long)wave * units / kPyrWaves);
+    const uint32_t* sw = reinterpret_cast<const uint32_t*>(smem + off);
+    uint8_t* dplane = blur + (size_t)b * blur_frame + BL.blur_off;
+    const us2 T01 = {(unsigned short)t0, (unsigned short)t1}, T23 = {(unsigned short)t2, (unsigned short)t3},
+              T21 = {(unsigned short)t2, (unsigned short)t1}, T0_ = {(unsigned short)t0, 0};
+    const us2 P0 = {(unsigned short)t0, (unsigned short)t0}, P1 = {(unsigned short)t1, (unsigned short)t1},
+              P2 = {(unsigned short)t2, (unsigned short)t2}, P3 = {(unsigned short)t3, (unsigned short)t3};
+    while (u < u1) {
+      const int chunk = u / nrow, row_a = u - chunk * nrow, row_b = min(nrow, row_a + (u1 - u));
+      const int g = chunk * cg + lane - 1, x = 4 * g;
+      const bool on = lane >= 1 && lane <= cg && g < ng;
+      const bool edge = chunk == 0 || chunk == nchunk - 1;
+      int ia = min(max(g - 1, 0), spw - 1);
+      uint32_t sel = 0;
+      if (x + 3 >= C || x < 0) {
+        ia = x < 0 ? 0 : min(max(g - (x >= C ? 2 : 1), 0), spw - 1);
+#pragma unroll
+        for (int i = 0; i < 4; i++) {
+          const int p = reflect101(x + i, C), j = p - 4 * ia;
+          sel |= (uint32_t)(p >= 0 && p < C && j >= 0 && j < 8 ? j : 0x0c) << (8 * i);
+        }
+      } else {
+        sel = g >= 1 ? 0x07060504u : 0x03020100u;
+      }
+      const int ib = min(ia + 1, spw - 1), xi = min(max(g, 0), spw - 1);
+      auto word = [&](int y) {
+        const int o = min(max(reflect101(y, R) - h0, 0), nheld - 1) * spw;
+        return edge ? __builtin_amdgcn_perm(sw[o + ib], sw[o + ia], sel) : sw[o + xi];
+      };
+      auto lo16 = [](uint32_t w) { return __builtin_bit_cast(us2, __builtin_amdgcn_perm(0u, w, 0x0c010c00u)); };
+      auto hi16 = [](uint32_t w) { return __builtin_bit_cast(us2, __builtin_amdgcn_perm(0u, w, 0x0c030c02u)); };
+      const int ya = ba + row_a, yb = ba + row_b;
+      us2 wl[7], wh[7];
+      wl[0] = wh[0] = us2{0, 0};
+#pragma unroll
+      for (int j = 0; j < 6; j++) {
+        const uint32_t w = word(ya - 3 + j);
+        wl[j + 1] = lo16(w);
+        wh[j + 1] = hi16(w);
+      }
+      uint32_t wn = word(ya + 3);
+      uint8_t* d = dplane + (size_t)ya * BL.pitch + x;
+      for (int y = ya; y < yb; y++) {
+#pragma unroll
+        for (int j = 0; j < 6; j++) {
+          wl[j] = wl[j + 1];
+          wh[j] = wh[j + 1];
+        }
+        wl[6] = lo16(wn);
+        wh[6] = hi16(wn);
+        wn = word(y + 4);
+        const us2 vl = (wl[0] + wl[6]) * P0 + (wl[1] + wl[5]) * P1 + (wl[2] + wl[4]) * P2 + wl[3] * P3;
+        const us2 vh = (wh[0] + wh[6]) * P0 + (wh[1] + wh[5]) * P1 + (wh[2] + wh[4]) * P2 + wh[3] * P3;
+        const uint32_t a2 = __builtin_bit_cast(uint32_t, vl), a3 = __builtin_bit_cast(uint32_t, vh);
+        const uint32_t a0 = (uint32_t)__builtin_amdgcn_update_dpp(0, (int)a2, 0x138, 0xf, 0xf, false);
+        const uint32_t a1 = (uint32_t)__builtin_amdgcn_update_dpp(0, (int)a3, 0x138, 0xf, 0xf, false);
+        const uint32_t a4 = (uint32_t)__builtin_amdgcn_update_dpp(0, (int)a2, 0x130, 0xf, 0xf, false);
+        const uint32_t a5 = (uint32_t)__builtin_amdgcn_update_dpp(0, (int)a3, 0x130, 0xf, 0xf, false);
+        auto pr = [](uint32_t hi, uint32_t lo) { return __builtin_bit_cast(us2, __builtin_amdgcn_alignbit(hi, lo, 16)); };
+        const us2 A1 = __builtin_bit_cast(us2, a1), A2 = vl, A3 = vh, A4 = __builtin_bit_cast(us2, a4), A5 = __builtin_bit_cast(us2, a5);
+        const us2 B0 = pr(a1, a0), B1 = pr(a2, a1), B2 = pr(a3, a2), B3 = pr(a4, a3), B4 = pr(a5, a4);
+        auto dot4 = [&](us2 q0, us2 q1, us2 q2, us2 q3) {
+          unsigned v = __builtin_amdgcn_udot2(q0, T01, 32768u, false);
+          v = __builtin_amdgcn_udot2(q1, T23, v, false);
+          v = __builtin_amdgcn_udot2(q2, T21, v, false);
+          v = __builtin_amdgcn_udot2(q3, T0_, v, false);
+          return min(v, 0x00ffffffu);
+        };
+        const unsigned m0 = dot4(B0, B1, B2, B3), m1 = dot4(A1, A2, A3, A4), m2 = dot4(B1, B2, B3, B4), m3 = dot4(A2, A3, A4, A5);
+        const uint32_t pk = __builtin_amdgcn_perm(m1, m0, 0x0c0c0602u) | __builtin_amdgcn_perm(m3, m2, 0x06020c0cu);
+        if (on) {
+          if (x + 3 < C) {
+            *reinterpret_cast<uint32_t*>(d) = pk;
+          } else {
+            for (int q = 0; q < 4 && x + q < C; q++) d[q] = (uint8_t)(pk >> (8 * q));
+          }
+        }
+        d += BL.pitch;
+      }
+      u += row_b - row_a;
+    }
+  };
   int tab0 = 0, pb = 0;
   for (int level = 1; level < nlevels; level++) {
     const LevelDev L = levels[level];
@@ -181,7 +302,7 @@
     const int r0 = rng[2 * level], nrow = rng[2 * level + 1] - r0, srow0 = rng[2 * (level - 1)], nsrc = rng[2 * (level - 1) + 1] - srow0;
     const int sp = gfs::OrbGeometry::kPyrLdsPitch(scols), kp = gfs::OrbGeometry::kPyrLdsPitch(L.cols);
     const unsigned src_off = (level - 1) & 1 ? lds_a : 0u, keep_off = level & 1 ? lds_a : 0u;
-    const bool has_keep = level + 1 < nlevels;
+    const bool has_keep = level + 1 < nlevels || level < blur_levels;
     uint8_t* dst = pyr + (size_t)b * pyr_frame + L.plane_off;
     const bool dst_even = (((uintptr_t)dst | (unsigned)L.pitch) & 1) == 0;
     const int nchunk = (L.cols + 127) >> 7, cw = (((L.cols + nchunk - 1) / nchunk) + 1) & ~1;
@@ -287,6 +408,7 @@
       else walk(std::false_type{});
       u += row_b - row_a;
     }
+    if (level - 1 < blur_levels) blur_phase(level - 1, src_off, srow0, nsrc);
     pb += nsrc;
     tab0 += nrow;
     __syncthreads();
@@ -294,6 +416,8 @@
     { const long long _n = clock64(); if (tid == 0) pyr_t[level] = _n; }
 #endif
   }
+  if (nlevels - 1 < blur_levels)
+    blur_phase(nlevels - 1, (nlevels - 1) & 1 ? lds_a : 0u, rng[2 * (nlevels - 1)], rng[2 * (nlevels - 1) + 1] - rng[2 * (nlevels - 1)]);
 #ifdef GFS_PYR_TIMING
   if (tid == 0 && b == 7 && (k == 0 || k == 3))
     printf("PYRT k=%d stage=%lld l1=%lld l2=%lld l3=%lld l4=%lld l5=%lld l6=%lld l7=%lld total=%lld\n", k, pyr_t[8] - pyr_t[0],
@@ -1441,12 +1565,6 @@
   }
 }
 
-__device__ __forceinline__ int reflect101(int p, int n) {
-  if (p < 0) p = -p;
-  if (p >= n) p = 2 * (n - 1) - p;
-  return p;
-}
-
 constexpr int kBlurTW = 64, kBlurTH = 32;
 __global__ __launch_bounds__(256) void k_blur7(const LevelDev* __restrict__ levels,
                                                const BlurTileDev* __restrict__ tiles, Lvl0 l0,
@@ -1497,23 +1615,8 @@
   for (int i = tid; i < (kBlurTH + 6) * (kBlurTW / 4); i += 256) {
     const int r = i >> 4, g = i & 15;
     const uint32_t w0 = raw[r][g], w1 = raw[r][g + 1], w2 = raw[r][g + 2];
-    typedef unsigned short us2 __attribute__((ext_vector_type(2)));
-    auto pair = [&](int i) -> us2 {
-      const uint32_t hi = i + 1 <= 7 ? w1 : w2, lo = i + 1 <= 7 ? w0 : w1;
-      const uint32_t j = i + 1 <= 7 ? i : i - 4;
-      const uint32_t v = __builtin_amdgcn_perm(hi, lo, j | (0x0cu << 8) | ((j + 1) << 16) | (0x0cu << 24));
-      return __builtin_bit_cast(us2, v);
-    };
-    const us2 T0 = {(unsigned short)t0, (unsigned short)t0}, T1 = {(unsigned short)t1, (unsigned short)t1},
-              T2 = {(unsigned short)t2, (unsigned short)t2}, T3 = {(unsigned short)t3, (unsigned short)t3};
-    uint32_t o2[2];
-#pragma unroll
-    for (int h2 = 0; h2 < 2; h2++) {
-      const int b0 = 1 + 2 * h2;
-      const us2 v = (pair(b0) + pair(b0 + 6)) * T0 + (pair(b0 + 1) + pair(b0 + 5)) * T1 + (pair(b0 + 2) + pair(b0 + 4)) * T2 + pair(b0 + 3) * T3;
-      o2[h2] = __builtin_bit_cast(uint32_t, v);
-    }
-    *reinterpret_cast<uint2*>(&hb[r][4 * g]) = make_uint2(o2[0], o2[1]);
+    const uint2 o2 = blur_h4(w0, w1, w2, t0, t1, t2, t3);
+    *reinterpret_cast<uint2*>(&hb[r][4 * g]) = o2;
   }
   __syncthreads();
   uint8_t* dst = blur + (size_t)b * blur_frame + L.blur_off;
@@ -1850,6 +1953,7 @@
   bool cands_packed = false;
   bool device_octree = true;
   bool pyr_in_hbm = false;
+  int last_blur_levels = 0, last_blur_strips = 0, last_blur_tiles = 0;
   bool octree_supported = true;
   bool host_counts_valid = false, host_cands_valid = false;
   gfs::DevBuf<KpIn> d_kpin;
@@ -1881,6 +1985,16 @@
   return {kPyrHbm, false};
 }
 inline bool octree_on_device(const gfs_orb* h) { return h->device_octree && h->octree_supported; }
+struct BlurPath {
+  int fused_levels;
+  int n_tiles;
+  size_t tile0;
+};
+inline BlurPath blur_path(const gfs_orb* h, PyrPath pp) {
+  const gfs::OrbGeometry& G = h->G;
+  if (pp.kernel == kPyrLds && G.blur_fused_levels > 0) return {G.blur_fused_levels, (int)G.blur_tiles_rest.size(), G.blur_tiles.size()};
+  return {0, (int)G.blur_tiles.size(), 0};
+}
 
 int ensure_geometry(gfs_orb* h, int rows, int cols) {
   if (h->geom_rows == rows && h->geom_cols == cols) return GFS_OK;
@@ -1899,6 +2013,9 @@
   GFS_HIP(hipMemcpyAsync(h->d_levels.p, G.levels.data(), G.levels.size() * sizeof(LevelDev), hipMemcpyHostToDevice, s));
   GFS_HIP(hipMemcpyAsync(h->d_cells.p, G.cells.data(), G.cells.size() * sizeof(CellDev), hipMemcpyHostToDevice, s));
   GFS_HIP(hipMemcpyAsync(h->d_tiles.p, G.blur_tiles.data(), G.blur_tiles.size() * sizeof(BlurTileDev), hipMemcpyHostToDevice, s));
+  if (!G.blur_tiles_rest.empty())
+    GFS_HIP(hipMemcpyAsync(h->d_tiles.p + G.blur_tiles.size(), G.blur_tiles_rest.data(), G.blur_tiles_rest.size() * sizeof(BlurTileDev),
+                           hipMemcpyHostToDevice, s));
   if (G.pyr_strips > 0) {
     GFS_HIP(hipMemcpyAsync(h->d_strip_rows.p, G.strip_rows.data(), G.strip_rows.size() * 4, hipMemcpyHostToDevice, s));
     if (G.pyr_strips_fine > 0)
@@ -1935,6 +2052,8 @@
   const int n_cells = (int)G.cells.size();
   const size_t cap_pyr = h->cap_pyr, cap_blur = h->cap_blur, cap_slab = h->cap_slab;
   const PyrPath pp = pyr_path(h, B);
+  const BlurPath bp = blur_path(h, pp);
+  const int* tp = kBlurTaps[h->P.blur_variant ? 1 : 0];
   if (pp.kernel == kPyrLds) {
     const bool fine = pp.fine;
     const int S = fine ? G.pyr_strips_fine : G.pyr_strips;
@@ -1943,7 +2062,7 @@
     GFS_LAUNCH("k_pyr_area_lds", k_pyr_area_lds, dim3(S, B), dim3(kPyrThreads), la + lb + lx, s, h->d_levels.p, nl, l0, h->d_pyr.p, cap_pyr,
                fine ? h->d_strip_rows_fine.p : h->d_strip_rows.p, (unsigned)la, lx ? (unsigned)(la + lb) : 0u, (int)G.xt_start.size(),
                h->d_xt_start.p, h->d_xt_n.p, h->d_xt_alpha.p,
-               h->d_yt_start.p, h->d_yt_n.p, h->d_yt_alpha.p);
+               h->d_yt_start.p, h->d_yt_n.p, h->d_yt_alpha.p, h->d_blur.p, cap_blur, bp.fused_levels, tp[0], tp[1], tp[2], tp[3]);
   } else if (pp.kernel == kPyrHbm) {
     GFS_LAUNCH("k_pyr_area_hbm", k_pyr_area_hbm, dim3(G.pyr_strips, B), dim3(kPyrThreads), 0, s, h->d_levels.p, nl, l0, h->d_pyr.p,
                cap_pyr, h->d_strip_rows.p, h->d_xt_start.p, h->d_xt_n.p, h->d_xt_alpha.p, h->d_yt_start.p, h->d_yt_n.p,
@@ -1952,7 +2071,9 @@
   const FastMap fm = fast_map(B, n_cells);
   GFS_LAUNCH("k_fast_cells", k_fast_cells, dim3(fm.grid), dim3(64 * kFcWaves), (size_t)kFcWaves * G.fast_lds_wave, s, h->d_cells.p, l0,
              h->d_pyr.p, cap_pyr, h->P.ini_th, h->P.min_th, n_cells, fm, (int)G.fast_lds_wave, cap_slab, h->d_slab.p, h->d_cell_cnt.p);
-  const int* tp = kBlurTaps[h->P.blur_variant ? 1 : 0];
+  h->last_blur_levels = bp.fused_levels;
+  h->last_blur_strips = pp.kernel == kPyrLds ? (pp.fine ? G.pyr_strips_fine : G.pyr_strips) : 0;
+  h->last_blur_tiles = bp.n_tiles;
   if (octree_on_device(h)) {
     GFS_LAUNCH("k_octree", k_octree, dim3(B * nl), dim3(kOctThreads), oct_lds_bytes(h->oct_node_cap), s, h->d_levels.p, nl, nullptr,
                nullptr, cap_slab, h->d_perm0.p, h->d_perm1.p, h->d_seg0.p, h->d_seg1.p, h->d_kept_off.p, h->cap_kp, h->d_kept.p,
@@ -1960,8 +2081,9 @@
     h->cands_packed = false;
     GFS_LAUNCH("k_kp_finalize", k_kp_finalize, dim3(B), dim3(256), 0, s, h->d_levels.p, nl, h->d_kept.p, h->d_kept_cnt.p,
                h->d_kept_off.p, h->cap_kp, lap0, lap1, h->d_kpin.p, h->d_kp_count.p, h->d_mono.p);
-    GFS_LAUNCH("k_blur7", k_blur7, dim3((unsigned)G.blur_tiles.size(), B), dim3(256), 0, s, h->d_levels.p, h->d_tiles.p, l0,
-               h->d_pyr.p, cap_pyr, h->d_blur.p, cap_blur, tp[0], tp[1], tp[2], tp[3]);
+    if (bp.n_tiles > 0)
+      GFS_LAUNCH("k_blur7", k_blur7, dim3((unsigned)bp.n_tiles, B), dim3(256), 0, s, h->d_levels.p, h->d_tiles.p + bp.tile0, l0,
+                 h->d_pyr.p, cap_pyr, h->d_blur.p, cap_blur, tp[0], tp[1], tp[2], tp[3]);
     {
       static const bool ob_xcd = !(getenv("GFS_ORB_OB_XCD") && atoi(getenv("GFS_ORB_OB_XCD")) == 0);
       const int nch = gfs::div_up(h->cap_kp, kObPerWg);
@@ -1986,8 +2108,9 @@
     GFS_HIP(hipMemcpy2DAsync(h->h_cand.p, cap_slab * 4, h->d_cand.p, cap_slab * 4, (size_t)max_total * 4, B,
                              hipMemcpyDeviceToHost, s));
   GFS_HIP(hipEventRecord(h->ev_copy, s));
-  GFS_LAUNCH("k_blur7", k_blur7, dim3((unsigned)G.blur_tiles.size(), B), dim3(256), 0, s, h->d_levels.p, h->d_tiles.p, l0,
-             h->d_pyr.p, cap_pyr, h->d_blur.p, cap_blur, tp[0], tp[1], tp[2], tp[3]);
+  if (bp.n_tiles > 0)
+    GFS_LAUNCH("k_blur7", k_blur7, dim3((unsigned)bp.n_tiles, B), dim3(256), 0, s, h->d_levels.p, h->d_tiles.p + bp.tile0, l0,
+               h->d_pyr.p, cap_pyr, h->d_blur.p, cap_blur, tp[0], tp[1], tp[2], tp[3]);
   GFS_HIP(hipEventSynchronize(h->ev_copy));
   const int ntask = B * nl;
   if ((int)h->kept.size() < ntask) h->kept.resize(ntask);
@@ -2097,6 +2220,7 @@
   std::unique_ptr<gfs_orb> h(new gfs_orb);
   h->cfg = *cfg;
   h->P.init(cfg->nfeatures, cfg->scale_factor, cfg->nlevels, cfg->ini_th_fast, cfg->min_th_fast, cfg->blur_taps_variant);
+  if (const char* e = getenv("GFS_ORB_BLUR_FUSED")) h->P.blur_fuse = std::max(0, atoi(e));
   gfs::OrbGeometry G;
   G.build(h->P, cfg->max_rows, cfg->max_cols);
   GFS_REQUIRE(G.supported, GFS_ERR_UNSUPPORTED, "ORB geometry for max size %dx%d unsupported: %s", cfg->max_cols,
@@ -2120,7 +2244,7 @@
   A(h->d_blur.alloc(B * h->cap_blur));
   A(h->d_levels.alloc(nl));
   A(h->d_cells.alloc(h->cap_cells));
-  A(h->d_tiles.alloc(G.blur_tiles.size() + 64));
+  A(h->d_tiles.alloc(2 * G.blur_tiles.size() + 64));
   A(h->d_strip_rows.alloc((size_t)2 * gfs::OrbGeometry::kPyrMaxStrips * 16));
   A(h->d_strip_rows_fine.alloc((size_t)2 * gfs::OrbGeometry::kPyrMaxStrips * 16));
   GFS_HIP(hipFuncSetAttribute(reinterpret_cast<const void*>(&k_pyr_area_lds), hipFuncAttributeMaxDynamicSharedMemorySize,
@@ -2403,6 +2527,16 @@
   return GFS_OK;
 }
 
+int gfs_test_orb_last_blur_path(gfs_orb* h, gfs_test_orb_blur_path* out) {
+  GFS_REQUIRE(h && out, GFS_ERR_INVALID_ARG, "gfs_test_orb_last_blur_path: NULL argument");
+  std::lock_guard<std::mutex> lk(h->mu);
+  out->fused = h->last_blur_levels > 0 ? 1 : 0;
+  out->fused_levels = h->last_blur_levels;
+  out->strips = h->last_blur_strips;
+  out->separate_tiles = h->last_blur_tiles;
+  return GFS_OK;
+}
+
 int gfs_orb_octree_host(const int32_t* x, const int32_t* y, const int32_t* score, int n, int min_x, int max_x,
                         int min_y, int max_y, int n_features, int32_t* out_idx, int cap) {
   std::vector<uint32_t> c(n);
diff --git a/geoflowslam_amd/csrc/orb_host.cpp b/geoflowslam_amd/csrc/orb_host.cpp
--- a/geoflowslam_amd/csrc/orb_host.cpp
+++ b/geoflowslam_amd/csrc/orb_host.cpp
@@ -208,7 +208,7 @@
     for (int ty = 0; ty < (L.rows + 31) / 32; ty++)
       for (int tx = 0; tx < (L.cols + 63) / 64; tx++) blur_tiles.push_back(BlurTileDev{(short)l, (short)tx, (short)ty, 0, L.rows, L.cols, L.pitch, L.plane_off, L.blur_off, 0u});
   }
-  {
+  auto xcd_order = [](std::vector<BlurTileDev>& blur_tiles) {
     auto at = [&](int l, int tx, int ty) -> const BlurTileDev* {
       for (const BlurTileDev& t : blur_tiles)
         if (t.level == l && t.tx == tx && t.ty == ty) return &t;
@@ -252,7 +252,9 @@
     }
     out.insert(out.end(), single.begin(), single.end());
     if (out.size() == blur_tiles.size()) blur_tiles.swap(out);
-  }
+  };
+  const std::vector<BlurTileDev> tiles_natural = blur_tiles;
+  xcd_order(blur_tiles);
   if (cols >= 4096 || rows >= 4096) {
     supported = false;
     why = "images must be smaller than 4096 x 4096 (12-bit packed candidate coordinates)";
@@ -263,6 +265,7 @@
   slab_entries = slab;
   cand_cap = slab;
   pyr_strips = pyr_strips_fine = 0;
+  blur_fused_levels = 0;
   pyr_lds_a = pyr_lds_b = pyr_lds_a_fine = pyr_lds_b_fine = pyr_lds_x = pyr_lds_x_fine = 0;
   strip_rows.clear();
   strip_rows_fine.clear();
@@ -274,8 +277,9 @@
       size_t la = 0, lb = 0;
       int tab_rows = 0;
       int prog_rows = 0;
+      size_t work = 0;
     };
-    auto cut = [&](int S) {
+    auto cut = [&](int S, int fused = 0) {
       Cut c;
       c.S = S;
       c.tab.assign((size_t)2 * S * nl, 0);
@@ -283,7 +287,12 @@
         int a = 0, b = 0, rows = 0, srows = 0;
         for (int l = nl - 1; l >= 0; l--) {
           const int R = levels[l].rows;
-          int oa = l >= 1 ? (int)((long long)k * R / S) : 0, ob = l >= 1 ? (int)((long long)(k + 1) * R / S) : 0;
+          int oa = 0, ob = 0;
+          if (l >= 1 || l < fused) oa = blur_share(k, S, R), ob = blur_share(k + 1, S, R);
+          if (l < fused && ob > oa) {
+            oa = std::max(oa - kBlurHalo, 0);
+            ob = std::min(ob + kBlurHalo, R);
+          }
           if (l < nl - 1 && b > a) {
             const LevelDev& U = levels[l + 1];
             const int fa = yt_start[U.ytab_off + a], fb = yt_start[U.ytab_off + b - 1] + yt_n[U.ytab_off + b - 1];
@@ -303,6 +312,7 @@
           if (l % 2 == 0) c.la = std::max(c.la, bytes);
           else c.lb = std::max(c.lb, bytes);
           if (l >= 1) rows += b - a;
+          if (l >= 1) c.work += (size_t)(b - a) * levels[l].cols;
           if (l < nl - 1) srows += b - a;
         }
         c.tab_rows = std::max(c.tab_rows, rows);
@@ -359,8 +369,31 @@
           pyr_lds_x_fine = cuts[i].la + cuts[i].lb + xbytes <= budget ? xbytes : 0;
           break;
         }
-    }
-  }
+      const Cut base = cuts[pick], base_fine = pyr_strips_fine ? cut(pyr_strips_fine) : Cut{};
+      auto fits = [&](const Cut& c, const Cut& b, size_t lx, size_t share) {
+        return c.la + c.lb + lx <= budget && c.tab_rows <= kPyrTabRows && c.prog_rows <= kPyrProgRows &&
+               (p.blur_fuse > 0 || (c.work - b.work) * share <= b.work);
+      };
+      for (int n = p.blur_fuse < 0 ? nl : std::min(p.blur_fuse, nl); n >= 1; n--) {
+        const Cut c = cut(pyr_strips, n), cf = pyr_strips_fine ? cut(pyr_strips_fine, n) : Cut{};
+        if (!fits(c, base, pyr_lds_x, 16) || (pyr_strips_fine && !fits(cf, base_fine, pyr_lds_x_fine, 8))) continue;
+        blur_fused_levels = n;
+        strip_rows = c.tab;
+        pyr_lds_a = c.la;
+        pyr_lds_b = c.lb;
+        if (pyr_strips_fine) {
+          strip_rows_fine = cf.tab;
+          pyr_lds_a_fine = cf.la;
+          pyr_lds_b_fine = cf.lb;
+        }
+        break;
+      }
+    }
+  }
+  blur_tiles_rest.clear();
+  for (const BlurTileDev& t : tiles_natural)
+    if (t.level >= blur_fused_levels) blur_tiles_rest.push_back(t);
+  xcd_order(blur_tiles_rest);
 }
 
 void ic_angle_offsets(const int umax[16], std::vector<int8_t>& du, std::vector<int8_t>& dv) {
@@ -615,6 +648,28 @@
   return nlevels;
 }
 
+extern "C" int gfs_test_orb_strip_rows(int rows, int cols, int nlevels, float scale_factor, int blur_fuse, int fine, int32_t* info4,
+                                       int32_t* strip_rows, int32_t* ytab, int cap) {
+  if (!info4 || rows <= 0 || cols <= 0 || nlevels <= 0 || nlevels > 16 || !(scale_factor > 1.f)) return GFS_ERR_INVALID_ARG;
+  gfs::OrbParams P;
+  P.init(1000, scale_factor, nlevels, 20, 7, 0);
+  P.blur_fuse = blur_fuse;
+  gfs::OrbGeometry G;
+  G.build(P, rows, cols);
+  if (!G.supported) return GFS_ERR_UNSUPPORTED;
+  const std::vector<int>& tab = fine ? G.strip_rows_fine : G.strip_rows;
+  info4[0] = fine ? G.pyr_strips_fine : G.pyr_strips;
+  info4[1] = G.blur_fused_levels;
+  info4[2] = (int)G.blur_tiles_rest.size();
+  info4[3] = (fine ? G.pyr_lds_a_fine + G.pyr_lds_b_fine : G.pyr_lds_a + G.pyr_lds_b) > 0 ? 1 : 0;
+  for (size_t i = 0; i < tab.size() && (int)i < cap && strip_rows; i++) strip_rows[i] = tab[i];
+  for (size_t i = 0; i < G.yt_start.size() && (int)(2 * i + 1) < cap && ytab; i++) {
+    ytab[2 * i] = G.yt_start[i];
+    ytab[2 * i + 1] = G.yt_start[i] + G.yt_n[i] - 1;
+  }
+  return (int)tab.size();
+}
+
 #include "std_sort_replica.hpp"
 extern "C" int gfs_test_sort_replica(int32_t* size_key, int32_t* x_key, int32_t* payload, int n) {
   struct E {
diff --git a/geoflowslam_amd/csrc/orb_host.hpp b/geoflowslam_amd/csrc/orb_host.hpp
--- a/geoflowslam_amd/csrc/orb_host.hpp
+++ b/geoflowslam_amd/csrc/orb_host.hpp
@@ -54,6 +54,7 @@
   std::vector<float> scale, inv_scale, sigma2, inv_sigma2;
   std::vector<int> quota;
   int umax[16];
+  int blur_fuse = -1;
   void init(int nfeatures, float scale_factor, int nlevels, int ini_th, int min_th, int blur_variant);
 };
 
@@ -76,6 +77,10 @@
   int pyr_strips_fine = 0;
   size_t pyr_lds_a_fine = 0, pyr_lds_b_fine = 0;
   static constexpr int kPyrMaxStrips = 64;
+  static constexpr int kBlurHalo = 3;
+  static constexpr int blur_share(int k, int S, int R) { return (int)((long long)k * R / S); }
+  int blur_fused_levels = 0;
+  std::vector<BlurTileDev> blur_tiles_rest;
   size_t pyr_bytes = 0, blur_bytes = 0;
   size_t slab_entries = 0;
   size_t cand_cap = 0;
```

Result: no change. 47120 frames/s, median of 6 (+0.3%).
